# jyfang6/kirag

Measured on NVIDIA B200. Metric: QPS, exact IP top-100 over 21000000x1024, higher is better.
Workload: dtype bf16 filter + f32 rescoring

## Files before the change

### include/kirag_b200.h

```cpp
#ifndef KIRAG_B200_H
#define KIRAG_B200_H

#include <stdint.h>

#ifdef __cplusplus
extern "C" {
#endif

#define KIRAG_ABI_VERSION 7

#define KIRAG_METRIC_INNER_PRODUCT 0
#define KIRAG_METRIC_L2 1

#define KIRAG_PATH_AUTO 0
#define KIRAG_PATH_EXACT 1
#define KIRAG_PATH_FAST 2

#define KIRAG_DTYPE_F32 0
#define KIRAG_DTYPE_BF16 1
#define KIRAG_DTYPE_F16 2

#define KIRAG_MASK_I64 0
#define KIRAG_MASK_I32 1
#define KIRAG_MASK_U8 2

#define KIRAG_POOL_MEAN 0
#define KIRAG_POOL_CLS 1

typedef struct kirag_index kirag_index_t;

typedef struct kirag_search_stats {
    int64_t nq;
    int64_t n_fast;
    int64_t n_exact;
    int64_t n_cert_fail;
    int64_t n_overflow;
    int32_t levels;
    int32_t path;
    int64_t kernel_launches;
    int64_t n_rescan;
    int64_t n_retry;
} kirag_search_stats_t;


int kirag_abi_version(void);

const char* kirag_last_error(void);

int kirag_device_count(void);

int kirag_profile_enable(int on);
int kirag_profile_read(double* scan_ms, int64_t* scan_launches, double* scan_rows);
int kirag_profile_read_launches(double* ms_out, double* rows_out, int64_t max_n);
int kirag_profile_read_timeline(int* tags_out, double* ms_since_first, int64_t max_n);


int kirag_index_create(int d, int metric, int device, kirag_index_t** out);

int kirag_index_destroy(kirag_index_t* h);

int kirag_index_reserve(kirag_index_t* h, int64_t n_total);

int kirag_index_add(kirag_index_t* h, const float* x, int64_t n, int x_is_device, void* stream);

int64_t kirag_index_ntotal(const kirag_index_t* h);

int kirag_index_dim(const kirag_index_t* h);

int kirag_index_search(kirag_index_t* h, const float* q, int64_t nq, int k,
                       float* D, int64_t* I, int ptrs_are_device, int64_t id_offset, void* stream);

int kirag_index_search_ex(kirag_index_t* h, const float* q, int64_t nq, int k,
                          float* D, int64_t* I, int ptrs_are_device, int64_t id_offset,
                          int path, kirag_search_stats_t* stats, void* stream);

int kirag_index_range_search(kirag_index_t* h, const float* q, int64_t nq, float radius, int q_is_device,
                             int64_t id_offset, int path, int64_t* lims_out, kirag_search_stats_t* stats,
                             void* stream);
int kirag_index_range_fetch(kirag_index_t* h, float* D, int64_t* I, int ptrs_are_device, void* stream);

int kirag_index_search_async(kirag_index_t* h, const float* q, int64_t nq, int k,
                             float* D, int64_t* I, int64_t id_offset, void* stream);

int kirag_index_search_finish(kirag_index_t* h, kirag_search_stats_t* stats, int64_t* n_changed);

int kirag_index_search_flags(const kirag_index_t* h, const int** flags_dev);

int kirag_index_search_rearm(kirag_index_t* h, void* stream);

int kirag_index_state_token(const kirag_index_t* h, uint64_t* token);

int kirag_index_reconstruct(const kirag_index_t* h, int64_t i0, int64_t n, float* out,
                            int out_is_device, void* stream);

int kirag_index_save(const kirag_index_t* h, const char* path);

int kirag_index_load(const char* path, int device, kirag_index_t** out);

int kirag_index_device_ptrs(const kirag_index_t* h, const float** master_f32, const void** shadow_bf16);

int kirag_debug_level_schedule(int64_t n_rows, int64_t nq, int k, int d, int64_t* rows_hi_out, int max_levels,
                               int* cap_out, int* kprime_out);

int kirag_index_debug_scores(kirag_index_t* h, const float* q_host, int64_t nq, float* out_host);

int kirag_merge_topk(const float* D_all, const int64_t* I_all, int G, int64_t nq, int k,
                     float* D_out, int64_t* I_out, int ptrs_are_device, int device, void* stream);

typedef struct kirag_exchange kirag_exchange_t;

int kirag_exchange_create(int device, int rank, int world, int64_t max_nq, int max_k, kirag_exchange_t** out);
int kirag_exchange_destroy(kirag_exchange_t* x);
int kirag_exchange_handle_bytes(void);
int kirag_exchange_export(kirag_exchange_t* x, void* handle_out);
int kirag_exchange_connect(kirag_exchange_t* x, const void* handles_all);
int kirag_exchange_connect_ptrs(kirag_exchange_t* x, void* const* peer_buffers);
void* kirag_exchange_buffer(kirag_exchange_t* x);
int kirag_exchange_merge_topk(kirag_exchange_t* x, const float* D_loc, const int64_t* I_loc, int64_t nq, int k,
                              float* D_out, int64_t* I_out, void* stream);

int kirag_exchange_merge_topk_flags(kirag_exchange_t* x, const float* D_loc, const int64_t* I_loc, const int* flags_loc,
                                    int64_t nq, int k, float* D_out, int64_t* I_out, void* stream);
int kirag_exchange_last_any_flag(kirag_exchange_t* x);

// ... 31 lines not shown
```

### kirag_b200/_lib.py

```python
from __future__ import annotations

import ctypes
import os
from ctypes import POINTER, c_char_p, c_float, c_int, c_int32, c_int64, c_void_p

HERE = os.path.dirname(os.path.abspath(__file__))
LIB_PATH = os.environ.get("KIRAG_B200_LIB") or os.path.join(HERE, "libkirag_b200.so")

ABI_VERSION = 7
METRIC_INNER_PRODUCT = 0
METRIC_L2 = 1
PATH_AUTO, PATH_EXACT, PATH_FAST = 0, 1, 2
DTYPE_F32, DTYPE_BF16, DTYPE_F16 = 0, 1, 2
MASK_I64, MASK_I32, MASK_U8 = 0, 1, 2
POOL_MEAN, POOL_CLS = 0, 1


class SearchStats(ctypes.Structure):
    _fields_ = [
        ("nq", c_int64),
        ("n_fast", c_int64),
        ("n_exact", c_int64),
        ("n_cert_fail", c_int64),
        ("n_overflow", c_int64),
        ("levels", c_int32),
        ("path", c_int32),
        ("kernel_launches", c_int64),
        ("n_rescan", c_int64),
        ("n_retry", c_int64),
    ]

    def as_dict(self):
        return {name: int(getattr(self, name)) for name, _ in self._fields_}


class KiragError(RuntimeError):
    """A C-ABI call returned a non-zero status (CUDA failure, bad handle...)."""


SIGNATURES = {
    "kirag_abi_version": (c_int, []),
    "kirag_last_error": (c_char_p, []),
    "kirag_device_count": (c_int, []),
    "kirag_profile_enable": (c_int, [c_int]),
    "kirag_profile_read": (c_int, [POINTER(ctypes.c_double), POINTER(c_int64), POINTER(ctypes.c_double)]),
    "kirag_profile_read_launches": (c_int, [POINTER(ctypes.c_double), POINTER(ctypes.c_double), c_int64]),
    "kirag_profile_read_timeline": (c_int, [POINTER(c_int), POINTER(ctypes.c_double), c_int64]),
    "kirag_index_create": (c_int, [c_int, c_int, c_int, POINTER(c_void_p)]),
    "kirag_index_destroy": (c_int, [c_void_p]),
    "kirag_index_reserve": (c_int, [c_void_p, c_int64]),
    "kirag_index_add": (c_int, [c_void_p, c_void_p, c_int64, c_int, c_void_p]),
    "kirag_index_ntotal": (c_int64, [c_void_p]),
    "kirag_index_dim": (c_int, [c_void_p]),
    "kirag_index_search": (c_int, [c_void_p, c_void_p, c_int64, c_int, c_void_p, c_void_p, c_int, c_int64, c_void_p]),
    "kirag_index_search_ex": (c_int, [c_void_p, c_void_p, c_int64, c_int, c_void_p, c_void_p, c_int, c_int64, c_int,
                                      POINTER(SearchStats), c_void_p]),
    "kirag_index_range_search": (c_int, [c_void_p, c_void_p, c_int64, c_float, c_int, c_int64, c_int, c_void_p,
                                         POINTER(SearchStats), c_void_p]),
    "kirag_index_range_fetch": (c_int, [c_void_p, c_void_p, c_void_p, c_int, c_void_p]),
    "kirag_index_search_async": (c_int, [c_void_p, c_void_p, c_int64, c_int, c_void_p, c_void_p, c_int64, c_void_p]),
    "kirag_index_search_finish": (c_int, [c_void_p, POINTER(SearchStats), POINTER(c_int64)]),
    "kirag_index_search_flags": (c_int, [c_void_p, POINTER(c_void_p)]),
    "kirag_index_search_rearm": (c_int, [c_void_p, c_void_p]),
    "kirag_index_state_token": (c_int, [c_void_p, POINTER(ctypes.c_uint64)]),
    "kirag_index_reconstruct": (c_int, [c_void_p, c_int64, c_int64, c_void_p, c_int, c_void_p]),
    "kirag_index_save": (c_int, [c_void_p, c_char_p]),
    "kirag_index_load": (c_int, [c_char_p, c_int, POINTER(c_void_p)]),
    "kirag_index_device_ptrs": (c_int, [c_void_p, POINTER(c_void_p), POINTER(c_void_p)]),
    "kirag_debug_level_schedule": (c_int, [c_int64, c_int64, c_int, c_int, POINTER(c_int64), c_int, POINTER(c_int),
                                           POINTER(c_int)]),
    "kirag_index_debug_scores": (c_int, [c_void_p, c_void_p, c_int64, c_void_p]),
    "kirag_merge_topk": (c_int, [c_void_p, c_void_p, c_int, c_int64, c_int, c_void_p, c_void_p, c_int, c_int, c_void_p]),
    "kirag_exchange_create": (c_int, [c_int, c_int, c_int, c_int64, c_int, POINTER(c_void_p)]),
    "kirag_exchange_destroy": (c_int, [c_void_p]),
    "kirag_exchange_handle_bytes": (c_int, []),
    "kirag_exchange_export": (c_int, [c_void_p, c_void_p]),
    "kirag_exchange_connect": (c_int, [c_void_p, c_void_p]),
    "kirag_exchange_connect_ptrs": (c_int, [c_void_p, POINTER(c_void_p)]),
    "kirag_exchange_buffer": (c_void_p, [c_void_p]),
    "kirag_exchange_merge_topk": (c_int, [c_void_p, c_void_p, c_void_p, c_int64, c_int, c_void_p, c_void_p, c_void_p]),
    "kirag_exchange_merge_topk_flags": (c_int, [c_void_p, c_void_p, c_void_p, c_void_p, c_int64, c_int, c_void_p, c_void_p,
                                                c_void_p]),
    "kirag_exchange_last_any_flag": (c_int, [c_void_p]),
    "kirag_topk_ip": (c_int, [c_void_p, c_int64, c_void_p, c_int64, c_int, c_int, c_void_p, c_void_p, c_int, c_int,
                              c_void_p]),
    "kirag_topk_ip_release": (c_int, []),
    "kirag_pool_normalize": (c_int, [c_void_p, c_void_p, c_void_p, c_int64, c_int64, c_int64, c_int64, c_int64, c_int64,
                                     c_int, c_int, c_int, c_int, c_int, c_void_p]),
    "kirag_pool_normalize_fwd_saved": (c_int, [c_void_p, c_void_p, c_void_p, c_void_p, c_int64, c_int64, c_int64,
                                               c_int64, c_int64, c_int64, c_int, c_int, c_int, c_int, c_int, c_void_p]),
    "kirag_pool_normalize_typed": (c_int, [c_void_p, c_void_p, c_void_p, c_void_p, c_void_p, c_int64, c_int64, c_int64,
                                           c_int64, c_int64, c_int64, c_int, c_int, c_int, c_int, c_int, c_void_p]),
    "kirag_pool_normalize_backward": (c_int, [c_void_p, c_void_p, c_void_p, c_void_p, c_void_p, c_int64, c_int64,
                                              c_int64, c_int64, c_int, c_int, c_int, c_int, c_int, c_void_p]),
}

_lib = None


def load() -> ctypes.CDLL:
    global _lib
    if _lib is not None:
        return _lib
    if not os.path.exists(LIB_PATH):
        raise ImportError(
            f"{LIB_PATH} is missing: build it with `python -m kirag_b200._build` "
            "(or `python -c 'import __graft_entry__ as g; g.build()'`). "
            "kirag_b200 has no CPU or pure-Python fallback."
        )
    lib = ctypes.CDLL(LIB_PATH)
    for name, (restype, argtypes) in SIGNATURES.items():
        fn = getattr(lib, name)
# ... 34 lines not shown
```

### kirag_b200/csrc/api.cu

```cuda
#include "common.cuh"
#include "../../include/kirag_b200.h"

#include <cuda.h>

#include <algorithm>
#include <atomic>
#include <cstdarg>
#include <cstdio>
#include <cstdlib>
#include <cstring>
#include <cmath>
#include <mutex>
#include <new>
#include <vector>

namespace kirag {

static thread_local char g_err[768] = "";
static std::atomic<long long> g_launches{0};

void set_error(const char* fmt, ...) {
    va_list ap;
    va_start(ap, fmt);
    vsnprintf(g_err, sizeof(g_err), fmt, ap);
// ... 140 lines not shown
            return cudaGetDriverEntryPoint(name, fn, cudaEnableDefault, &qr) == cudaSuccess &&
                   qr == cudaDriverEntryPointSuccess && *fn != nullptr;
        };
        a.ok = get("cuMemAddressReserve", (void**)&a.AddressReserve) && get("cuMemAddressFree", (void**)&a.AddressFree) &&
               get("cuMemCreate", (void**)&a.Create) && get("cuMemRelease", (void**)&a.Release) &&
               get("cuMemMap", (void**)&a.Map) && get("cuMemUnmap", (void**)&a.Unmap) &&
               get("cuMemSetAccess", (void**)&a.SetAccess) &&
               get("cuMemGetAllocationGranularity", (void**)&a.GetGranularity);
        cudaGetLastError();
        return a;
    }();
    return api;
}

struct VmBuffer {
    CUdeviceptr base = 0;
    size_t reserved = 0, mapped = 0, gran = 0;
    int device = 0;
    struct Chunk { CUmemGenericAllocationHandle h; size_t off, size; };
    std::vector<Chunk> chunks;

    bool active() const { return base != 0; }
    void* ptr() const { return reinterpret_cast<void*>(base); }

    CUmemAllocationProp prop() const {
        CUmemAllocationProp p = {};
        p.type = CU_MEM_ALLOCATION_TYPE_PINNED;
        p.location.type = CU_MEM_LOCATION_TYPE_DEVICE;
        p.location.id = device;
        return p;
    }
    int reserve(int dev, size_t bytes) {
        const VmmApi& a = vmm_api();
        if (!a.ok) return 1;
        device = dev;
        const CUmemAllocationProp p = prop();
        if (a.GetGranularity(&gran, &p, CU_MEM_ALLOC_GRANULARITY_RECOMMENDED) != CUDA_SUCCESS || gran == 0) return 1;
        reserved = (bytes + gran - 1) / gran * gran;
        if (a.AddressReserve(&base, reserved, 0, 0, 0) != CUDA_SUCCESS) { base = 0; reserved = 0; return 1; }
        return 0;
    }
    int ensure(size_t bytes) {
        if (bytes <= mapped) return 0;
        const VmmApi& a = vmm_api();
        const size_t want = (bytes + gran - 1) / gran * gran;
        if (want > reserved) return 1;
        Chunk c;
        c.off = mapped;
        c.size = want - mapped;
        const CUmemAllocationProp p = prop();
        if (a.Create(&c.h, c.size, &p, 0) != CUDA_SUCCESS) return 1;
        if (a.Map(base + c.off, c.size, 0, c.h, 0) != CUDA_SUCCESS) { a.Release(c.h); return 1; }
        CUmemAccessDesc acc = {};
        acc.location = p.location;
        acc.flags = CU_MEM_ACCESS_FLAGS_PROT_READWRITE;
        if (a.SetAccess(base + c.off, c.size, &acc, 1) != CUDA_SUCCESS) {
            a.Unmap(base + c.off, c.size);
            a.Release(c.h);
            return 1;
        }
        chunks.push_back(c);
        mapped = want;
        return 0;
    }
    void release() {
        const VmmApi& a = vmm_api();
        for (auto& c : chunks) { a.Unmap(base + c.off, c.size); a.Release(c.h); }
        chunks.clear();
        if (base) a.AddressFree(base, reserved);
        base = 0;
        reserved = mapped = 0;
    }
};

struct FastParams {
    int kprime;
    int growth_override;
    int cap_override;
    int first_growth_override;
    int few_queries;
};

struct SearchCounters {
    int64_t n_fast = 0, n_exact = 0, n_cert_fail = 0, n_overflow = 0, n_rescan = 0, n_retry = 0, n_changed = 0;
    int levels = 0;
};

struct PendingSearch {
    bool active = false;
    bool ev_recorded = false;
    bool fast_ok = false;
    int mode = 0, path = 0, k = 0;
    int64_t nq = 0, id_offset = 0;
    const float* qd = nullptr;
    float* Dd = nullptr;
    int64_t* Id = nullptr;
    cudaStream_t st = nullptr;
    long long launches0 = 0;
    SearchCounters counters;
    FastParams fp{};
};

struct kirag_index {
    int d = 0;
    int metric = 0;
    int device = 0;
    int num_sms = 148;
    int64_t ntotal = 0;
    int64_t capacity = 0;
    float* master = nullptr;
    uint8_t* shadow = nullptr;
    VmBuffer vm_master, vm_shadow;
    bool use_vmm = false;
    unsigned* maxnorm2_bits = nullptr;
    float maxnorm = 0.f;
    float maxerr = 0.f;
    float maxnorm_x = 0.f;
    float* center = nullptr;
    float center_norm = 0.f;
    bool center_decided = false;
    DevBuf q_dev, D_dev, I_dev, qshadow, qnorm, cand, cnt, tau, tauk, overflow, flags, rescored;
    DevBuf dense, stage_a, stage_b, qmap, qsel, qnorm2, D_tmp, I_tmp, t_dev, center_sums;
    int* host_flags = nullptr;
    size_t host_flags_n = 0;
    PendingSearch pending;
    PendingSearch captured;
    bool has_captured = false;
    cudaEvent_t pending_ev = nullptr;
    DevBuf ritems, ritems2, rcount, rcursor, roff, rtab, rD, rI;
    int64_t range_n = 0;
    bool range_valid = false;
};

static int64_t round_up(int64_t v, int64_t m) { return (v + m - 1) / m * m; }

static int env_int(const char* name, int dflt) {
    const char* v = getenv(name);
    if (!v || !*v) return dflt;
    return atoi(v);
}

constexpr int64_t kCenterMinRows = 4096;
constexpr int64_t kCenterSampleRows = 8192;
static int decide_center(kirag_index* h, int64_t rows_available, cudaStream_t st) {
    if (env_int("KIRAG_NO_CENTER", 0)) return 0;
    const int d = h->d;
    const int64_t rows = rows_available < kCenterSampleRows ? rows_available : kCenterSampleRows;
    DevBuf& sums = h->center_sums;
    if (sums.ensure((size_t)(d + 1) * 4)) return 1;
    std::vector<float> host((size_t)d + 1);
    int rc = 1;
    do {
        if (cudaMemsetAsync(sums.p, 0, (size_t)(d + 1) * 4, st) != cudaSuccess) break;
        if (launch_column_sums(h->master, rows, d, sums.as<float>(), st)) break;
        if (cudaMemcpyAsync(host.data(), sums.p, (size_t)(d + 1) * 4, cudaMemcpyDeviceToHost, st) != cudaSuccess ||
            cudaStreamSynchronize(st) != cudaSuccess) {
            set_error("decide_center: reading the column sums failed: %s", cudaGetErrorString(cudaGetLastError()));
            break;
        }
        double c2 = 0.0;
        for (int c = 0; c < d; ++c) {
            host[(size_t)c] = (float)((double)host[(size_t)c] / (double)rows);
            c2 += (double)host[(size_t)c] * (double)host[(size_t)c];
        }
        const double mean_sq = (double)host[(size_t)d] / (double)rows;
        rc = 0;
        if (!(c2 >= mean_sq / 16.0) || !(mean_sq > 0.0) || !(c2 == c2)) break;
        rc = 1;
        if (cudaMalloc((void**)&h->center, (size_t)d * 4) != cudaSuccess) {
            h->center = nullptr;
            set_error("decide_center: cudaMalloc failed: %s", cudaGetErrorString(cudaGetLastError()));
            break;
        }
        if (cudaMemcpyAsync(h->center, host.data(), (size_t)d * 4, cudaMemcpyHostToDevice, st) != cudaSuccess ||
            cudaStreamSynchronize(st) != cudaSuccess) {
            set_error("decide_center: uploading the centre failed");
            break;
        }
        h->center_norm = (float)sqrt(c2);
        rc = 0;
    } while (0);
    return rc;
}

static int index_grow(kirag_index* h, int64_t need_rows, cudaStream_t st) {
    if (need_rows <= h->capacity) return 0;
    const bool want_shadow = scan_tc_supported(h->d) != 0;
    const size_t row_m = (size_t)h->d * sizeof(float), row_s = (size_t)h->d * 2;
    if (h->capacity == 0 && !h->master && vmm_api().ok) {
        size_t free_b = 0, total_b = 0;
        if (cudaMemGetInfo(&free_b, &total_b) == cudaSuccess && total_b > 0) {
            const size_t max_rows = (size_t)round_up((int64_t)(total_b / row_m) + kTileRows, kTileRows);
            if (h->vm_master.reserve(h->device, max_rows * row_m) == 0 &&
                (!want_shadow || h->vm_shadow.reserve(h->device, max_rows * row_s) == 0)) {
                h->use_vmm = true;
                h->master = static_cast<float*>(h->vm_master.ptr());
                h->shadow = want_shadow ? static_cast<uint8_t*>(h->vm_shadow.ptr()) : nullptr;
            } else {
                h->vm_master.release();
                h->vm_shadow.release();
            }
        }
        cudaGetLastError();
    }
    int64_t cap = round_up(need_rows > h->capacity + h->capacity / 4 ? need_rows : h->capacity + h->capacity / 4, kTileRows);
    const int64_t exact = round_up(need_rows, kTileRows);
    if (h->use_vmm) {
        for (int attempt = 0; attempt < 2; ++attempt) {
            const int64_t c = attempt == 0 ? cap : exact;
            if (h->vm_master.ensure((size_t)c * row_m) == 0 && (!want_shadow || h->vm_shadow.ensure((size_t)c * row_s) == 0)) {
                h->capacity = c;
                return 0;
            }
            if (cap == exact) break;
        }
        size_t free_b = 0, total_b = 0;
        cudaMemGetInfo(&free_b, &total_b);
        set_error("index storage for %lld rows x %d (fp32 master%s) does not fit: %zu MiB free of %zu MiB",
                  (long long)exact, h->d, want_shadow ? " + bf16 shadow" : "", free_b >> 20, total_b >> 20);
        cudaGetLastError();
        return 1;
    }
    auto regrow = [&](void** buf, size_t row_bytes, size_t live_rows, const char* what) -> int {
        void* nb = nullptr;
        int64_t c = cap;
        cudaError_t e = cudaMalloc(&nb, (size_t)c * row_bytes);
        if (e != cudaSuccess && cap != exact) { cudaGetLastError(); c = exact; e = cudaMalloc(&nb, (size_t)c * row_bytes); }
        if (e != cudaSuccess) {
            set_error("cudaMalloc of the %s (%zu bytes for %lld rows) failed: %s", what, (size_t)c * row_bytes, (long long)c,
                      cudaGetErrorString(e));
            cudaGetLastError();
            return 1;
        }
        if (*buf && live_rows > 0) {
            if (cudaMemcpyAsync(nb, *buf, live_rows * row_bytes, cudaMemcpyDeviceToDevice, st) != cudaSuccess ||
                cudaStreamSynchronize(st) != cudaSuccess) {
                cudaFree(nb);
                set_error("device copy while growing the %s failed: %s", what, cudaGetErrorString(cudaGetLastError()));
                return 1;
            }
        }
        if (*buf) cudaFree(*buf);
        *buf = nb;
        cap = c;
        return 0;
    };
    if (regrow((void**)&h->master, row_m, (size_t)h->ntotal, "fp32 master")) return 1;
    if (want_shadow && regrow((void**)&h->shadow, row_s, (size_t)round_up(h->ntotal, kTileRows), "bf16 shadow")) return 1;
    h->capacity = cap;
    return 0;
}

static int exact_search(kirag_index* h, const float* qsub, int64_t nsub, int k, float* D, int64_t* I,
                        int64_t out_row0, const int* qmap_dev, int64_t id_offset, cudaStream_t st) {
    const int64_t n = h->ntotal;
    const int d = h->d;
    const int m = (int)((k < n) ? k : n);
    const int64_t ld = round_up(n, 32);
    if (h->dense.ensure((size_t)kExactNQ * ld * sizeof(float))) return 1;
    const int64_t n_seg = (n + kSelectSeg - 1) / kSelectSeg;
    if (h->stage_a.ensure((size_t)kExactNQ * n_seg * m * sizeof(Cand))) return 1;
    for (int64_t g0 = 0; g0 < nsub; g0 += kExactNQ) {
        const int gq = (int)((nsub - g0 < kExactNQ) ? (nsub - g0) : kExactNQ);
        if (launch_scan_exact(h->master, n, d, qsub + g0 * d, gq, h->dense.as<float>(), ld, h->num_sms, st)) return 1;
        int nseg_i = 0;
        if (launch_select_dense(h->dense.as<float>(), ld, n, gq, m, h->stage_a.as<Cand>(), &nseg_i, st)) return 1;
        Cand* cur = h->stage_a.as<Cand>();
        int64_t cur_stride = (int64_t)nseg_i * m;
        int cur_count = (int)cur_stride;
        bool use_b = true;
        while (cur_count > kSelectSeg) {
            const int ns2 = (cur_count + kSelectSeg - 1) / kSelectSeg;
            DevBuf& dstb = use_b ? h->stage_b : h->stage_a;
            if (dstb.ensure((size_t)kExactNQ * ns2 * m * sizeof(Cand))) return 1;
            Cand* dst = dstb.as<Cand>();
            if (launch_select_pairs(cur, cur_stride, nullptr, cur_count, 0x7fffffff, gq, m, dst,
                                    (int64_t)ns2 * m, ns2, nullptr, nullptr, nullptr, st)) return 1;
            cur = dst;
            cur_stride = (int64_t)ns2 * m;
            cur_count = (int)cur_stride;
// ... 7 lines not shown
    return 0;
}

constexpr int64_t kWideCapMaxQueries = 128;
constexpr int64_t kQChunk = 16384;
constexpr int64_t kFewQueries = 8;
constexpr int kMaxGrowth = 32;


static bool fast_eligible(const kirag_index* h, int k, FastParams* fp) {
    if (!h->shadow || !scan_tc_supported(h->d)) return false;
    if (h->ntotal > 0x7fffff00LL) return false;
    int64_t kp = (int64_t)4 * k;
    if (kp < 32) kp = 32;
    if (kp > 2048) kp = 2048;
    if (kp < k) return false;
    fp->kprime = (int)kp;
    fp->growth_override = env_int("KIRAG_LEVEL_GROWTH", 0);
    fp->cap_override = env_int("KIRAG_CAND_CAP", 0);
    fp->first_growth_override = env_int("KIRAG_LEVEL1_GROWTH", 0);
    if (fp->cap_override > 0 && fp->cap_override < 4 * kp) return false;
    return true;
}

static int pick_cap(const FastParams& fp, int64_t nq) {
    int cap = (nq <= kWideCapMaxQueries) ? kWideCap : kSelectSeg;
    if (fp.cap_override > 0) cap = fp.cap_override;
    if (cap > kWideCap) cap = kWideCap;
    return cap;
}

static std::vector<int64_t> level_bounds(int64_t n_tiles, int cap, const FastParams& fp) {
    std::vector<int64_t> hi;
    int64_t t = (cap / 2) / kTileRows;
    if (t < 1) t = 1;
    if (t > n_tiles) t = n_tiles;
    hi.push_back(t);
    if (t >= n_tiles) return hi;
    int gmax = cap / (4 * fp.kprime);
    if (gmax > kMaxGrowth) gmax = kMaxGrowth;
    if (fp.growth_override > 0) gmax = fp.growth_override;
    if (gmax < 2) gmax = 2;
    int g1 = (cap >= kWideCap && fp.few_queries) ? 16 : 4;
    if (fp.first_growth_override > 0) g1 = fp.first_growth_override;
    if (g1 > gmax) g1 = gmax;
    t = t * g1;
    if (t > n_tiles) t = n_tiles;
    hi.push_back(t);
    if (t >= n_tiles) return hi;
    const double ratio = (double)n_tiles / (double)t;
    int L = (int)ceil(log(ratio) / log((double)gmax) - 1e-9);
    if (L < 1) L = 1;
    const double g = pow(ratio, 1.0 / L);
    const int64_t base = t;
    for (int i = 1; i <= L; ++i) {
        int64_t b = (i == L) ? n_tiles : (int64_t)ceil((double)base * pow(g, (double)i));
        if (b <= hi.back()) b = hi.back() + 1;
        if (b > n_tiles) b = n_tiles;
        hi.push_back(b);
        if (b >= n_tiles) break;
    }
    return hi;
}

static int64_t pick_tile_mult(int64_t n_tiles) {
    if (n_tiles <= 2) return 1;
    int64_t m = (int64_t)(0.6180339887498949 * (double)n_tiles);
    if (m < 1) m = 1;
    auto gcd = [](int64_t a, int64_t b) { while (b) { int64_t t = a % b; a = b; b = t; } return a; };
    while (gcd(m, n_tiles) != 1) ++m;
    return m % n_tiles;
}

struct CertEps { float a, b; };
static CertEps cert_eps(const kirag_index* h) {
    const double yn = (double)h->maxnorm, ey = (double)h->maxerr, xn = (double)h->maxnorm_x, cn = (double)h->center_norm;
    const double acc = (double)h->d * ldexp(1.0, -22);
    CertEps e;
    e.a = (float)((ey + acc * (yn + xn) + ldexp(1.0, -24) * yn + 64.0 * ldexp(1.0, -24) * cn) * 1.002);
    e.b = (float)((yn + 2.0 * ey) * 1.002);
    return e;
}

static int fast_search(kirag_index* h, const float* qd, int64_t nq, int k, float* D, int64_t* I,
                       int64_t id_offset, const FastParams& fp, int check_cert, int* levels_out,
                       cudaStream_t st) {
    const int d = h->d;
    const int64_t n = h->ntotal;
    struct PdlScope {
        explicit PdlScope(bool on) { g_pdl_this_call = on; }
        ~PdlScope() { g_pdl_this_call = true; }
    } pdl_scope(nq <= kPdlMaxQueries);
    ScanTcPlan plan;
    if (scan_tc_pick(nq, d, &plan)) return 1;
    const size_t qs_bytes = scan_tc_qshadow_bytes(nq, d, plan);
    if (h->qshadow.ensure(qs_bytes)) return 1;
    if (h->qnorm.ensure((size_t)nq * 12)) return 1;
    const int cap = pick_cap(fp, nq);
    if (h->cand.ensure((size_t)nq * cap * sizeof(Cand))) return 1;
    if (h->cnt.ensure((size_t)nq * 4)) return 1;
    const int64_t nq_pad = round_up(nq, 256);
    if (h->tau.ensure((size_t)nq_pad * 4)) return 1;
    if (h->overflow.ensure((size_t)nq * 4)) return 1;
    if (h->flags.ensure((size_t)nq * 4)) return 1;
    if (h->rescored.ensure((size_t)nq * fp.kprime * 4)) return 1;
    if (h->tauk.ensure((size_t)nq * 4)) return 1;
    const bool fuse_tail = cap == kWideCap && fp.kprime <= 2048;
    if ((nq % plan.bq) != 0)
        KIRAG_CUDA_OK(cudaMemsetAsync(h->qshadow.p, 0, qs_bytes, st));
    KIRAG_CUDA_OK(launch_chained(init_search_state_kernel, dim3((unsigned)((nq_pad + 255) / 256)), dim3(256), 0, st,
                                 h->tau.as<float>(), h->cnt.as<int>(), h->overflow.as<int>(), nq, nq_pad));
    KIRAG_LAUNCH_OK("init_search_state_kernel");
    prof_mark(0, st);
    float* const qcdot = h->qnorm.as<float>() + 2 * nq;
    if (launch_convert_rows(qd, nq, d, 0, h->qshadow.p, plan.bq / 2, nullptr, h->qnorm.as<float>(),
                            h->qnorm.as<float>() + nq, h->center, qcdot, st)) return 1;
    prof_mark(1, st);

    const int64_t n_tiles = (n + kTileRows - 1) / kTileRows;
    const int64_t mult = pick_tile_mult(n_tiles);
    FastParams fpl = fp;
    fpl.few_queries = nq <= kFewQueries ? 1 : 0;
    const std::vector<int64_t> bounds = level_bounds(n_tiles, cap, fpl);
    int64_t lo = 0;
    int levels = 0;
    for (const int64_t hi : bounds) {
        cudaEvent_t e0 = nullptr, e1 = nullptr;
        if (g_prof.on) {
            KIRAG_CUDA_OK(cudaEventCreate(&e0));
            KIRAG_CUDA_OK(cudaEventCreate(&e1));
            KIRAG_CUDA_OK(cudaEventRecord(e0, st));
        }
        if (launch_scan_tc(h->shadow, n, d, h->qshadow.p, nq, plan, lo, hi, n_tiles, mult,
                           h->tau.as<float>(), h->cand.as<Cand>(), h->cnt.as<int>(), cap, h->num_sms,
                           levels == 0 ? 1 : 0, st)) return 1;
        if (g_prof.on) {
            KIRAG_CUDA_OK(cudaEventRecord(e1, st));
            g_prof.ev.emplace_back(e0, e1);
            int64_t r1 = hi * kTileRows; if (r1 > n) r1 = n;
            g_prof.rows += (double)(r1 - lo * kTileRows);
            g_prof.launch_rows.push_back((double)(r1 - lo * kTileRows));
            g_prof.queries = (double)nq;
        }
        prof_mark(10 + levels, st);
        const bool last = (hi == bounds.back());
        if (last && fuse_tail) break;
        if (launch_compact_topm(h->cand.as<Cand>(), cap, h->cnt.as<int>(), cap, (int)nq, fp.kprime,
                                h->tau.as<float>(), h->overflow.as<int>(), last ? h->tauk.as<float>() : nullptr,
                                k, st)) return 1;
        prof_mark(30 + levels, st);
        ++levels;
        lo = hi;
    }
    const CertEps ce = cert_eps(h);
    if (fuse_tail) {
        ++levels;
        if (launch_tail_fused(h->cand.as<Cand>(), cap, h->cnt.as<int>(), cap, (int)nq, fp.kprime, h->tau.as<float>(),
                              h->overflow.as<int>(), h->master, d, qd, h->rescored.as<float>(), k, D, I, id_offset,
                              h->qnorm.as<float>(), h->qnorm.as<float>() + nq, qcdot, ce.a, ce.b, h->flags.as<int>(),
                              h->num_sms, st)) return 1;
        prof_mark(51, st);
        if (levels_out) *levels_out = levels;
        return 0;
    }
    if (launch_rescore(h->master, d, qd, h->cand.as<Cand>(), h->cnt.as<int>(), cap, fp.kprime,
                       h->rescored.as<float>(), nq, h->tauk.as<float>(), h->qnorm.as<float>(),
                       h->qnorm.as<float>() + nq, ce.a, ce.b, st)) return 1;
    prof_mark(50, st);
    if (launch_final(h->cand.as<Cand>(), cap, h->rescored.as<float>(), h->cnt.as<int>(), 0, fp.kprime,
                     (int)nq, k, D, I, id_offset, h->tau.as<float>(), h->qnorm.as<float>(), h->qnorm.as<float>() + nq,
                     qcdot, ce.a, ce.b, check_cert, h->overflow.as<int>(), h->flags.as<int>(), nullptr, st)) return 1;
    prof_mark(51, st);
    if (levels_out) *levels_out = levels;
    return 0;
}

__global__ void rescan_threshold_kernel(const float* __restrict__ D, const int* __restrict__ qmap,
                                        const float* __restrict__ qnorm, const float* __restrict__ qerr,
                                        const float* __restrict__ qcdot, int k,
                                        float eps_a, float eps_b, int64_t nb,
                                        int64_t nb_pad, float* __restrict__ tau2, int* __restrict__ cnt,
                                        int* __restrict__ overflow) {
    const int64_t i = (int64_t)blockIdx.x * blockDim.x + threadIdx.x;
    if (i >= nb_pad) return;
    if (i >= nb) { tau2[i] = INFINITY; return; }
    const int q = qmap[i];
    const float kth = D[(int64_t)q * k + (k - 1)];
    tau2[i] = (kth > -FLT_MAX) ? kth - (eps_a * qnorm[q] + eps_b * qerr[q]) - qcdot[q] : -INFINITY;
    cnt[i] = 0;
    overflow[i] = 0;
}

static int rescan_search(kirag_index* h, const float* qsel, const float* qnorm_all, const float* qerr_all,
                         const float* qcdot_all, int64_t nb,
                         int k, float* D,
                         int64_t* I, const int* qmap_dev, int64_t id_offset, int cap, std::vector<int>* still_bad,
                         cudaStream_t st) {
    const int d = h->d;
    const int64_t n = h->ntotal;
    ScanTcPlan plan;
    if (scan_tc_pick(nb, d, &plan)) return 1;
    const size_t qs_bytes = scan_tc_qshadow_bytes(nb, d, plan);
    const int64_t nb_pad = round_up(nb, 256);
    if (h->qshadow.ensure(qs_bytes)) return 1;
    if (h->cand.ensure((size_t)nb * cap * sizeof(Cand))) return 1;
    if (h->cnt.ensure((size_t)nb_pad * 4) || h->tau.ensure((size_t)nb_pad * 4) || h->overflow.ensure((size_t)nb_pad * 4)) return 1;
    if (h->flags.ensure((size_t)nb_pad * 4)) return 1;
    if (h->rescored.ensure((size_t)nb * cap * 4)) return 1;
    const CertEps ce = cert_eps(h);
    rescan_threshold_kernel<<<(unsigned)((nb_pad + 255) / 256), 256, 0, st>>>(
        D, qmap_dev, qnorm_all, qerr_all, qcdot_all, k, ce.a, ce.b, nb, nb_pad, h->tau.as<float>(), h->cnt.as<int>(),
        h->overflow.as<int>());
    KIRAG_LAUNCH_OK("rescan_threshold_kernel");
    if ((nb % plan.bq) != 0) KIRAG_CUDA_OK(cudaMemsetAsync(h->qshadow.p, 0, qs_bytes, st));
    if (launch_convert_rows(qsel, nb, d, 0, h->qshadow.p, plan.bq / 2, nullptr, nullptr, nullptr, nullptr, nullptr,
                            st)) return 1;
    const int64_t n_tiles = (n + kTileRows - 1) / kTileRows;
    if (launch_scan_tc(h->shadow, n, d, h->qshadow.p, nb, plan, 0, n_tiles, n_tiles, 1, h->tau.as<float>(),
                       h->cand.as<Cand>(), h->cnt.as<int>(), cap, h->num_sms, 1, st)) return 1;
    if (launch_rescore(h->master, d, qsel, h->cand.as<Cand>(), h->cnt.as<int>(), cap, cap, h->rescored.as<float>(), nb,
                       nullptr, nullptr, nullptr, 0.f, 0.f, st)) return 1;
    std::vector<int> counts((size_t)nb);
    KIRAG_CUDA_OK(cudaMemcpyAsync(counts.data(), h->cnt.p, (size_t)nb * 4, cudaMemcpyDeviceToHost, st));
    if (launch_final(h->cand.as<Cand>(), cap, h->rescored.as<float>(), h->cnt.as<int>(), 0, cap, (int)nb, k, D, I,
                     id_offset, nullptr, nullptr, nullptr, nullptr, 0.f, 0.f, 0, nullptr, nullptr, qmap_dev, st)) return 1;
    KIRAG_CUDA_OK(cudaStreamSynchronize(st));
    for (int64_t i = 0; i < nb; ++i)
        if (counts[(size_t)i] > cap) still_bad->push_back((int)i);
    return 0;
}


static int ensure_host_flags(kirag_index* h, int64_t cq) {
    if (h->host_flags_n >= (size_t)cq) return 0;
    if (h->host_flags) cudaFreeHost(h->host_flags);
    h->host_flags = nullptr;
    h->host_flags_n = 0;
    const size_t want = (size_t)round_up(cq, 4096);
    KIRAG_CUDA_OK(cudaHostAlloc((void**)&h->host_flags, want * sizeof(int), cudaHostAllocDefault));
    h->host_flags_n = want;
    return 0;
}

static int enqueue_chunk(kirag_index* h, const float* qd, int64_t cq, int k, float* Dd, int64_t* Id, int64_t id_offset,
                         bool fast_ok, const FastParams& fp, SearchCounters* c, int* mode, cudaStream_t st) {
    *mode = 0;
    if (h->ntotal == 0) return launch_fill_pad(Dd, Id, cq * k, st);
    if (!fast_ok) {
        if (exact_search(h, qd, cq, k, Dd, Id, 0, nullptr, id_offset, st)) return 1;
        c->n_exact += cq;
        return 0;
    }
    if (ensure_host_flags(h, cq)) return 1;
    if (fast_search(h, qd, cq, k, Dd, Id, id_offset, fp, 1, &c->levels, st)) return 1;
    KIRAG_CUDA_OK(cudaMemcpyAsync(h->host_flags, h->flags.p, (size_t)cq * 4, cudaMemcpyDeviceToHost, st));
    *mode = 1;
    return 0;
}

__global__ void scatter_rows_kernel(const float* __restrict__ Ds, const int64_t* __restrict__ Is, const int* __restrict__ qmap,
                                    int k, float* __restrict__ D, int64_t* __restrict__ I) {
    const int64_t src = blockIdx.x, dst = qmap[src];
    for (int j = threadIdx.x; j < k; j += blockDim.x) {
        D[dst * k + j] = Ds[src * k + j];
        I[dst * k + j] = Is[src * k + j];
    }
}

static int resolve_chunk(kirag_index* h, const float* qd, int64_t cq, int k, float* Dd, int64_t* Id, int64_t id_offset,
                         int path, const FastParams& fp, SearchCounters* c, cudaStream_t st) {
    const int d = h->d;
    const int* flags = h->host_flags;
    std::vector<int> cert, ovf;
    for (int64_t i = 0; i < cq; ++i) {
        if (flags[(size_t)i] == 2) { ovf.push_back((int)i); ++c->n_overflow; }
        else if (flags[(size_t)i]) { cert.push_back((int)i); ++c->n_cert_fail; }
    }
    const int64_t n_bad = (int64_t)(cert.size() + ovf.size());
    if (n_bad == 0 || path != KIRAG_PATH_AUTO) {
        c->n_fast += cq;
        return 0;
    }
    if (h->qnorm2.ensure((size_t)cq * 12)) return 1;
    KIRAG_CUDA_OK(cudaMemcpyAsync(h->qnorm2.p, h->qnorm.p, (size_t)cq * 12, cudaMemcpyDeviceToDevice, st));
    std::vector<int> exact;
    const bool no_rescan = env_int("KIRAG_NO_RESCAN", 0) != 0;
    const bool gentle_already = fp.growth_override > 0 && fp.growth_override <= 4 && fp.first_growth_override > 0;
    if (!ovf.empty() && !gentle_already) {
        const int64_t nb = (int64_t)ovf.size();
        if (h->qmap.ensure((size_t)nb * 4) || h->qsel.ensure((size_t)nb * d * 4)) return 1;
        if (h->D_tmp.ensure((size_t)nb * k * 4) || h->I_tmp.ensure((size_t)nb * k * 8)) return 1;
        KIRAG_CUDA_OK(cudaMemcpyAsync(h->qmap.p, ovf.data(), (size_t)nb * 4, cudaMemcpyHostToDevice, st));
        gather_rows_kernel<<<(unsigned)nb, 256, 0, st>>>(qd, h->qmap.as<int>(), d, h->qsel.as<float>());
        KIRAG_LAUNCH_OK("gather_rows_kernel");
        FastParams gentle = fp;
        gentle.growth_override = 4;
        gentle.first_growth_override = 2;
        if (fast_search(h, h->qsel.as<float>(), nb, k, h->D_tmp.as<float>(), h->I_tmp.as<int64_t>(), id_offset, gentle, 1,
                        nullptr, st)) return 1;
        std::vector<int> f2((size_t)nb);
        KIRAG_CUDA_OK(cudaMemcpyAsync(f2.data(), h->flags.p, (size_t)nb * 4, cudaMemcpyDeviceToHost, st));
        scatter_rows_kernel<<<(unsigned)nb, 128, 0, st>>>(h->D_tmp.as<float>(), h->I_tmp.as<int64_t>(), h->qmap.as<int>(), k,
                                                          Dd, Id);
        KIRAG_LAUNCH_OK("scatter_rows_kernel");
        KIRAG_CUDA_OK(cudaStreamSynchronize(st));
        for (int64_t i = 0; i < nb; ++i) {
            if (f2[(size_t)i] == 0) ++c->n_retry;
            else if (f2[(size_t)i] == 2) exact.push_back(ovf[(size_t)i]);
            else cert.push_back(ovf[(size_t)i]);
        }
    } else {
        exact = ovf;
    }
    if (!cert.empty() && no_rescan) {
        exact.insert(exact.end(), cert.begin(), cert.end());
        cert.clear();
    }
    if (!cert.empty()) {
        const int64_t nb = (int64_t)cert.size();
        if (h->qmap.ensure((size_t)nb * 4)) return 1;
        if (h->qsel.ensure((size_t)nb * d * 4)) return 1;
        KIRAG_CUDA_OK(cudaMemcpyAsync(h->qmap.p, cert.data(), (size_t)nb * 4, cudaMemcpyHostToDevice, st));
        gather_rows_kernel<<<(unsigned)nb, 256, 0, st>>>(qd, h->qmap.as<int>(), d, h->qsel.as<float>());
        KIRAG_LAUNCH_OK("gather_rows_kernel");
        std::vector<int> still_bad;
        if (rescan_search(h, h->qsel.as<float>(), h->qnorm2.as<float>(), h->qnorm2.as<float>() + cq,
                          h->qnorm2.as<float>() + 2 * cq, nb, k, Dd, Id, h->qmap.as<int>(), id_offset, kSelectSeg, &still_bad,
                          st)) return 1;
        for (int i : still_bad) exact.push_back(cert[(size_t)i]);
        c->n_rescan += nb - (int64_t)still_bad.size();
    }
    if (!exact.empty()) {
        const int64_t nb = (int64_t)exact.size();
        if (h->qmap.ensure((size_t)nb * 4)) return 1;
        if (h->qsel.ensure((size_t)nb * d * 4)) return 1;
        KIRAG_CUDA_OK(cudaMemcpyAsync(h->qmap.p, exact.data(), (size_t)nb * 4, cudaMemcpyHostToDevice, st));
        gather_rows_kernel<<<(unsigned)nb, 256, 0, st>>>(qd, h->qmap.as<int>(), d, h->qsel.as<float>());
        KIRAG_LAUNCH_OK("gather_rows_kernel");
        if (exact_search(h, h->qsel.as<float>(), nb, k, Dd, Id, 0, h->qmap.as<int>(), id_offset, st)) return 1;
        c->n_exact += nb;
    }
    KIRAG_CUDA_OK(cudaStreamSynchronize(st));
    c->n_fast += cq - n_bad;
    c->n_changed += n_bad;
    return 0;
}

static void fill_stats(kirag_search_stats_t* stats, int64_t nq, const SearchCounters& c, bool fast_ok, int path,
                       long long launches0) {
    if (!stats) return;
    stats->nq = nq;
    stats->n_fast = c.n_fast;
    stats->n_exact = c.n_exact;
    stats->n_cert_fail = c.n_cert_fail;
    stats->n_overflow = c.n_overflow;
    stats->n_rescan = c.n_rescan;
    stats->n_retry = c.n_retry;
    stats->levels = c.levels;
    stats->path = fast_ok ? path : KIRAG_PATH_EXACT;
    stats->kernel_launches = g_launches.load() - launches0;
}

static void drop_range_result(kirag_index* h) {
    h->range_n = 0;
    h->range_valid = false;
}

static int finish_pending(kirag_index* h, kirag_search_stats_t* stats, int64_t* n_changed) {
    drop_range_result(h);
    if (n_changed) *n_changed = 0;
    PendingSearch& p = h->pending;
    if (!p.active) {
        if (stats) memset(stats, 0, sizeof(*stats));
        return 0;
    }
    p.active = false;
    DeviceGuard guard(h->device);
    if (!guard.ok) return 1;
    if (p.ev_recorded) KIRAG_CUDA_OK(cudaEventSynchronize(h->pending_ev));
    else KIRAG_CUDA_OK(cudaStreamSynchronize(p.st));
    SearchCounters c = p.counters;
    if (p.mode == 1 && resolve_chunk(h, p.qd, p.nq, p.k, p.Dd, p.Id, p.id_offset, p.path, p.fp, &c, p.st)) return 1;
    fill_stats(stats, p.nq, c, p.fast_ok, p.path, p.launches0);
    if (n_changed) *n_changed = c.n_changed;
    return 0;
}

static int search_impl(kirag_index* h, const float* q, int64_t nq, int k, float* D, int64_t* I,
                       int ptrs_are_device, int64_t id_offset, int path, kirag_search_stats_t* stats,
                       cudaStream_t st) {
    KIRAG_CHECK(h != nullptr, "search: null index");
    KIRAG_CHECK(k > 0, "search: k must be positive (got %d)", k);
    KIRAG_CHECK(k <= 2048, "search: k=%d exceeds the supported maximum of 2048", k);
    KIRAG_CHECK(nq >= 0, "search: negative nq");
    KIRAG_CHECK(path >= 0 && path <= 2, "search: unknown path %d", path);
    if (finish_pending(h, nullptr, nullptr)) return 1;
    if (stats) memset(stats, 0, sizeof(*stats));
    if (nq == 0) return 0;
    KIRAG_CHECK(q && D && I, "search: null buffer");
    DeviceGuard guard(h->device);
    if (!guard.ok) return 1;
    const long long launches0 = g_launches.load();
    const int d = h->d;
    SearchCounters c;
    FastParams fp{};
    const bool fast_ok = (path != KIRAG_PATH_EXACT) && h->ntotal > 0 && fast_eligible(h, k, &fp);

    for (int64_t q0 = 0; q0 < nq; q0 += kQChunk) {
        const int64_t cq = (nq - q0 < kQChunk) ? (nq - q0) : kQChunk;
        const float* qd;
        float* Dd;
        int64_t* Id;
        if (ptrs_are_device) {
            qd = q + q0 * d; Dd = D + q0 * k; Id = I + q0 * k;
        } else {
            if (h->q_dev.ensure((size_t)cq * d * 4)) return 1;
            if (h->D_dev.ensure((size_t)cq * k * 4)) return 1;
            if (h->I_dev.ensure((size_t)cq * k * 8)) return 1;
            KIRAG_CUDA_OK(cudaMemcpyAsync(h->q_dev.p, q + q0 * d, (size_t)cq * d * 4, cudaMemcpyHostToDevice, st));
            qd = h->q_dev.as<float>(); Dd = h->D_dev.as<float>(); Id = h->I_dev.as<int64_t>();
        }
        int mode = 0;
        if (enqueue_chunk(h, qd, cq, k, Dd, Id, id_offset, fast_ok, fp, &c, &mode, st)) return 1;
        if (!ptrs_are_device) {
            KIRAG_CUDA_OK(cudaMemcpyAsync(D + q0 * k, Dd, (size_t)cq * k * 4, cudaMemcpyDeviceToHost, st));
            KIRAG_CUDA_OK(cudaMemcpyAsync(I + q0 * k, Id, (size_t)cq * k * 8, cudaMemcpyDeviceToHost, st));
        }
        if (mode == 1 || !ptrs_are_device) KIRAG_CUDA_OK(cudaStreamSynchronize(st));
        if (mode == 1) {
            const int64_t changed0 = c.n_changed;
            if (resolve_chunk(h, qd, cq, k, Dd, Id, id_offset, path, fp, &c, st)) return 1;
            if (!ptrs_are_device && c.n_changed != changed0) {
                KIRAG_CUDA_OK(cudaMemcpyAsync(D + q0 * k, Dd, (size_t)cq * k * 4, cudaMemcpyDeviceToHost, st));
                KIRAG_CUDA_OK(cudaMemcpyAsync(I + q0 * k, Id, (size_t)cq * k * 8, cudaMemcpyDeviceToHost, st));
                KIRAG_CUDA_OK(cudaStreamSynchronize(st));
            }
        }
    }
    fill_stats(stats, nq, c, fast_ok, path, launches0);
    return 0;
}

constexpr size_t kRangeGroupBytes = (size_t)1 << 30;

struct RangeChunk {
    std::vector<int64_t> src_off, count;
    int64_t used = 0;
};

static int grow_keep(DevBuf& b, size_t used, size_t need, cudaStream_t st) {
    if (need <= b.bytes) return 0;
    size_t want = b.bytes + b.bytes / 2;
    if (want < need) want = need;
    want = (want + ((size_t)1 << 20) - 1) & ~(((size_t)1 << 20) - 1);
    void* p = nullptr;
    cudaError_t e = cudaMalloc(&p, want);
    if (e != cudaSuccess) {
        cudaGetLastError();
        set_error("range_search: cudaMalloc(%zu) for the collected entries failed: %s", want, cudaGetErrorString(e));
        return 1;
    }
    if (used) KIRAG_CUDA_OK(cudaMemcpyAsync(p, b.p, used, cudaMemcpyDeviceToDevice, st));
    KIRAG_CUDA_OK(cudaStreamSynchronize(st));
    b.release();
    b.p = p;
    b.bytes = want;
    return 0;
}

static int range_reserve(kirag_index* h, RangeChunk& rc, const std::vector<int>& counts, const std::vector<int>& chunk_q,
                         cudaStream_t st) {
    const size_t nsrc = counts.size();
    std::vector<int64_t> cursor(nsrc, 0);
    int64_t add = 0;
    for (size_t i = 0; i < nsrc; ++i) {
        if (chunk_q[i] < 0) continue;
        cursor[i] = rc.used + add;
        rc.src_off[(size_t)chunk_q[i]] = cursor[i];
        rc.count[(size_t)chunk_q[i]] = counts[i];
        add += counts[i];
    }
    if (grow_keep(h->ritems, (size_t)rc.used * 8, (size_t)(rc.used + add) * 8, st)) return 1;
    rc.used += add;
    if (h->rcursor.ensure(nsrc * 8)) return 1;
    KIRAG_CUDA_OK(cudaMemcpyAsync(h->rcursor.p, cursor.data(), nsrc * 8, cudaMemcpyHostToDevice, st));
    KIRAG_CUDA_OK(cudaStreamSynchronize(st));
    return 0;
}

static int range_scan(kirag_index* h, const ScanTcPlan& plan, int64_t nq, int cap, cudaStream_t st) {
    const int64_t n = h->ntotal;
    const int64_t n_tiles = (n + kTileRows - 1) / kTileRows;
    cudaEvent_t e0 = nullptr, e1 = nullptr;
    if (g_prof.on) {
        KIRAG_CUDA_OK(cudaEventCreate(&e0));
        KIRAG_CUDA_OK(cudaEventCreate(&e1));
        KIRAG_CUDA_OK(cudaEventRecord(e0, st));
    }
    if (launch_scan_tc(h->shadow, n, h->d, h->qshadow.p, nq, plan, 0, n_tiles, n_tiles, 1, h->tau.as<float>(),
                       h->cand.as<Cand>(), h->cnt.as<int>(), cap, h->num_sms, 1, st)) return 1;
    if (g_prof.on) {
        KIRAG_CUDA_OK(cudaEventRecord(e1, st));
        g_prof.ev.emplace_back(e0, e1);
        g_prof.rows += (double)n;
        g_prof.launch_rows.push_back((double)n);
        g_prof.queries = (double)nq;
    }
    return 0;
}

static int range_filter_pass(kirag_index* h, const float* qs, int64_t nb, const int* qmap_dev,
                             const std::vector<int>& chunk_q_of_row, int64_t cq, float radius, int cap, bool first,
                             RangeChunk& rc, std::vector<int>* cnt_out, cudaStream_t st) {
    const int d = h->d;
// ... 133 lines not shown
    }
    if (n_seg) {
        tab[(size_t)4 * n_seg] = total_long;
        if (h->ritems2.ensure((size_t)rc.used * 8) || h->rtab.ensure(tab.size() * 8)) return 1;
        KIRAG_CUDA_OK(cudaMemcpyAsync(h->rtab.p, tab.data(), tab.size() * 8, cudaMemcpyHostToDevice, st));
    }
    if (h->roff.ensure(((size_t)cq * 2 + 1) * 8)) return 1;
    KIRAG_CUDA_OK(cudaMemcpyAsync(h->roff.p, rc.src_off.data(), (size_t)cq * 8, cudaMemcpyHostToDevice, st));
    KIRAG_CUDA_OK(cudaMemcpyAsync(h->roff.as<int64_t>() + cq, lims.data(), ((size_t)cq + 1) * 8, cudaMemcpyHostToDevice, st));
    if (launch_range_emit(h->ritems.as<uint64_t>(), h->ritems2.as<uint64_t>(), cq, h->roff.as<int64_t>(),
                          h->roff.as<int64_t>() + cq, n_seg, longest, total_long, h->rtab.as<int64_t>(), id_offset,
                          h->rD.as<float>() + base, h->rI.as<int64_t>() + base, st)) return 1;
    KIRAG_CUDA_OK(cudaStreamSynchronize(st));
    return 0;
}

static int range_search_impl(kirag_index* h, const float* q, int64_t nq, float radius, int q_is_device,
                             int64_t id_offset, int path, int64_t* lims_out, kirag_search_stats_t* stats,
                             cudaStream_t st) {
    KIRAG_CHECK(nq >= 0, "range_search: negative nq");
    KIRAG_CHECK(h != nullptr, "range_search: null index");
    KIRAG_CHECK(lims_out != nullptr, "range_search: null lims");
    KIRAG_CHECK(path >= 0 && path <= 2, "range_search: unknown path %d", path);
    if (finish_pending(h, nullptr, nullptr)) return 1;
    if (stats) memset(stats, 0, sizeof(*stats));
    for (int64_t i = 0; i <= nq; ++i) lims_out[i] = 0;
    const bool fast_ok = path != KIRAG_PATH_EXACT && h->shadow && scan_tc_supported(h->d) && h->ntotal <= 0x7fffff00LL;
    if (nq == 0 || h->ntotal == 0 || !(radius < INFINITY)) {
        h->range_valid = true;
        if (stats) { stats->nq = nq; stats->path = fast_ok ? path : KIRAG_PATH_EXACT; }
        return 0;
    }
    KIRAG_CHECK(q != nullptr, "range_search: null queries");
    DeviceGuard guard(h->device);
    if (!guard.ok) return 1;
    const long long launches0 = g_launches.load();
    const int d = h->d;
    FastParams fp{};
    fp.cap_override = env_int("KIRAG_CAND_CAP", 0);
    SearchCounters c;
    int64_t base = 0;
    for (int64_t q0 = 0; q0 < nq; q0 += kQChunk) {
        const int64_t cq = (nq - q0 < kQChunk) ? (nq - q0) : kQChunk;
        const float* qd = q + q0 * d;
        if (!q_is_device) {
            if (h->q_dev.ensure((size_t)cq * d * 4)) return 1;
            KIRAG_CUDA_OK(cudaMemcpyAsync(h->q_dev.p, qd, (size_t)cq * d * 4, cudaMemcpyHostToDevice, st));
            qd = h->q_dev.as<float>();
        }
        RangeChunk rc;
        rc.src_off.assign((size_t)cq, 0);
        rc.count.assign((size_t)cq, 0);
        if (fast_ok ? range_filter_chunk(h, qd, cq, radius, pick_cap(fp, cq), rc, &c, st)
                    : range_exact_chunk(h, qd, cq, radius, rc, &c, st)) return 1;
        int64_t chunk_total = 0;
        if (range_emit_chunk(h, rc, cq, id_offset, base, lims_out + q0, &chunk_total, st)) return 1;
        base += chunk_total;
    }
    lims_out[nq] = base;
    h->range_n = base;
    h->range_valid = true;
    fill_stats(stats, nq, c, fast_ok, path, launches0);
    return 0;
}

static int range_fetch_impl(kirag_index* h, float* D, int64_t* I, int ptrs_are_device, cudaStream_t st) {
    KIRAG_CHECK(h != nullptr, "range_fetch: null index");
    KIRAG_CHECK(h->range_valid, "range_fetch: no range-search result is held (the last call on this index was not "
                                "kirag_index_range_search, or its result was fetched already)");
    const int64_t total = h->range_n;
    if (total > 0) {
        KIRAG_CHECK(D && I, "range_fetch: null buffer");
        DeviceGuard guard(h->device);
        if (!guard.ok) return 1;
        const cudaMemcpyKind kind = ptrs_are_device ? cudaMemcpyDeviceToDevice : cudaMemcpyDeviceToHost;
        KIRAG_CUDA_OK(cudaMemcpyAsync(D, h->rD.p, (size_t)total * 4, kind, st));
        KIRAG_CUDA_OK(cudaMemcpyAsync(I, h->rI.p, (size_t)total * 8, kind, st));
        KIRAG_CUDA_OK(cudaStreamSynchronize(st));
    }
    drop_range_result(h);
    return 0;
}

static int finalize_rows(kirag_index* h, int64_t r0, int64_t n, cudaStream_t st) {
    if (h->shadow && !h->center_decided && r0 + n >= kCenterMinRows) {
        if (decide_center(h, r0 + n, st)) return 1;
        h->center_decided = true;
        if (h->center && r0 > 0) {
            KIRAG_CUDA_OK(cudaMemsetAsync(h->maxnorm2_bits, 0, 8, st));
            if (launch_convert_rows(h->master, r0, h->d, 0, h->shadow, kTileRows, h->maxnorm2_bits, nullptr, nullptr, h->center,
                                    nullptr, st)) return 1;
        }
    }
    if (launch_convert_rows(h->master + r0 * (int64_t)h->d, n, h->d, r0, h->shadow, kTileRows, h->maxnorm2_bits, nullptr,
                            nullptr, h->center, nullptr, st)) return 1;
    if (h->shadow && ((r0 + n) % kTileRows) != 0) {
        const int64_t end = r0 + n;
        const int64_t tile = end / kTileRows;
        const int rr = (int)(end - tile * kTileRows);
        uint8_t* tile_base = h->shadow + (size_t)tile * ((size_t)h->d * kTileRows * 2);
        KIRAG_CUDA_OK(cudaMemset2DAsync(tile_base + (size_t)rr * 128, (size_t)kTileRows * 128, 0, (size_t)(kTileRows - rr) * 128,
                                        (size_t)(h->d / kKChunk), st));
    }
    unsigned bits[3] = {0, 0, 0};
    KIRAG_CUDA_OK(cudaMemcpyAsync(bits, h->maxnorm2_bits, 12, cudaMemcpyDeviceToHost, st));
    KIRAG_CUDA_OK(cudaStreamSynchronize(st));
    float m2[3];
    memcpy(m2, bits, 12);
    h->maxnorm = sqrtf(m2[0]);
    h->maxerr = h->shadow ? sqrtf(m2[1]) : 0.f;
    h->maxnorm_x = h->shadow ? sqrtf(m2[2]) : h->maxnorm;
    h->ntotal = r0 + n;
    return 0;
}

extern "C" {

int kirag_abi_version(void) { return KIRAG_ABI_VERSION; }

const char* kirag_last_error(void) { return g_err; }

int kirag_device_count(void) {
    int n = 0;
    if (cudaGetDeviceCount(&n) != cudaSuccess) { cudaGetLastError(); return 0; }
    return n;
}

int kirag_profile_enable(int on) {
    for (auto& pr : g_prof.ev) { cudaEventDestroy(pr.first); cudaEventDestroy(pr.second); }
    g_prof.ev.clear();
    g_prof.launch_rows.clear();
    for (auto& mk : g_prof.marks) cudaEventDestroy(mk.second);
    g_prof.marks.clear();
    g_prof.rows = 0.0;
    g_prof.on = on != 0;
    return 0;
}

int kirag_profile_read_timeline(int* tags_out, double* ms_since_first, int64_t max_n) {
    int64_t i = 0;
    for (auto& mk : g_prof.marks) {
        if (i >= max_n) break;
        KIRAG_CUDA_OK(cudaEventSynchronize(mk.second));
        float t = 0.f;
        KIRAG_CUDA_OK(cudaEventElapsedTime(&t, g_prof.marks[0].second, mk.second));
        if (tags_out) tags_out[i] = mk.first;
        if (ms_since_first) ms_since_first[i] = t;
        ++i;
    }
    return (int)i;
}

int kirag_profile_read_launches(double* ms_out, double* rows_out, int64_t max_n) {
    int64_t i = 0;
    for (auto& pr : g_prof.ev) {
        if (i >= max_n) break;
        KIRAG_CUDA_OK(cudaEventSynchronize(pr.second));
        float t = 0.f;
        KIRAG_CUDA_OK(cudaEventElapsedTime(&t, pr.first, pr.second));
        if (ms_out) ms_out[i] = t;
        if (rows_out) rows_out[i] = g_prof.launch_rows[(size_t)i];
        ++i;
    }
    return 0;
}

int kirag_profile_read(double* scan_ms, int64_t* scan_launches, double* scan_rows) {
    double ms = 0.0;
    for (auto& pr : g_prof.ev) {
        KIRAG_CUDA_OK(cudaEventSynchronize(pr.second));
        float t = 0.f;
        KIRAG_CUDA_OK(cudaEventElapsedTime(&t, pr.first, pr.second));
        ms += t;
    }
    if (scan_ms) *scan_ms = ms;
    if (scan_launches) *scan_launches = (int64_t)g_prof.ev.size();
    if (scan_rows) *scan_rows = g_prof.rows;
    for (auto& pr : g_prof.ev) { cudaEventDestroy(pr.first); cudaEventDestroy(pr.second); }
    g_prof.ev.clear();
    g_prof.launch_rows.clear();
    for (auto& mk : g_prof.marks) cudaEventDestroy(mk.second);
    g_prof.marks.clear();
    g_prof.rows = 0.0;
    return 0;
}

int kirag_index_create(int d, int metric, int device, kirag_index_t** out) {
    KIRAG_CHECK(out != nullptr, "index_create: null out pointer");
    *out = nullptr;
    KIRAG_CHECK(d > 0 && d <= 16384, "index_create: unsupported dimension %d", d);
    KIRAG_CHECK(metric == KIRAG_METRIC_INNER_PRODUCT,
                "index_create: only the inner-product metric is implemented (got %d)", metric);
    int ndev = 0;
    cudaError_t e = cudaGetDeviceCount(&ndev);
    if (e != cudaSuccess || ndev == 0) {
        set_error("index_create: no CUDA device available (%s); this library has no CPU path",
                  e == cudaSuccess ? "device count is 0" : cudaGetErrorString(e));
        cudaGetLastError();
        return 1;
    }
    KIRAG_CHECK(device >= 0 && device < ndev, "index_create: device %d out of range [0,%d)", device, ndev);
    cudaDeviceProp prop;
    KIRAG_CUDA_OK(cudaGetDeviceProperties(&prop, device));
    KIRAG_CHECK(prop.major == 10, "index_create: device %d is sm_%d%d; this library is built for sm_100a only",
                device, prop.major, prop.minor);
    DeviceGuard guard(device);
    if (!guard.ok) return 1;
    kirag_index* h = new (std::nothrow) kirag_index();
    KIRAG_CHECK(h != nullptr, "index_create: out of host memory");
    h->d = d;
    h->metric = metric;
    h->device = device;
    h->num_sms = prop.multiProcessorCount;
    if (cudaMalloc((void**)&h->maxnorm2_bits, 12) != cudaSuccess || cudaMemset(h->maxnorm2_bits, 0, 12) != cudaSuccess) {
        set_error("index_create: cudaMalloc failed: %s", cudaGetErrorString(cudaGetLastError()));
        delete h;
        return 1;
    }
    *out = h;
    return 0;
}

int kirag_index_destroy(kirag_index_t* h) {
    if (!h) return 0;
    DeviceGuard guard(h->device);
    cudaDeviceSynchronize();
    if (h->use_vmm) {
        h->vm_master.release();
        h->vm_shadow.release();
    } else {
        if (h->master) cudaFree(h->master);
        if (h->shadow) cudaFree(h->shadow);
    }
    if (h->maxnorm2_bits) cudaFree(h->maxnorm2_bits);
    if (h->center) cudaFree(h->center);
    DevBuf* bufs[] = {&h->q_dev, &h->D_dev, &h->I_dev, &h->qshadow, &h->qnorm, &h->cand, &h->cnt, &h->tau, &h->tauk,
                      &h->overflow, &h->flags, &h->rescored, &h->dense, &h->stage_a, &h->stage_b, &h->qmap, &h->qsel, &h->qnorm2, &h->t_dev, &h->center_sums,
                      &h->D_tmp, &h->I_tmp, &h->ritems, &h->ritems2, &h->rcount, &h->rcursor, &h->roff, &h->rtab,
                      &h->rD, &h->rI};
    for (DevBuf* b : bufs) b->release();
    if (h->host_flags) cudaFreeHost(h->host_flags);
    if (h->pending_ev) cudaEventDestroy(h->pending_ev);
    delete h;
    return 0;
}

int kirag_index_reserve(kirag_index_t* h, int64_t n_total) {
    KIRAG_CHECK(h != nullptr, "index_reserve: null index");
    KIRAG_CHECK(n_total >= 0, "index_reserve: negative size");
    DeviceGuard guard(h->device);
    if (!guard.ok) return 1;
    return index_grow(h, n_total, 0);
}

int kirag_index_add(kirag_index_t* h, const float* x, int64_t n, int x_is_device, void* stream) {
    KIRAG_CHECK(h != nullptr, "index_add: null index");
    KIRAG_CHECK(n >= 0, "index_add: negative n");
    if (n == 0) return 0;
    KIRAG_CHECK(x != nullptr, "index_add: null data");
    DeviceGuard guard(h->device);
    if (!guard.ok) return 1;
    cudaStream_t st = (cudaStream_t)stream;
    if (finish_pending(h, nullptr, nullptr)) return 1;
    KIRAG_CHECK(h->ntotal + n <= 0x7fffff00LL, "index_add: more than 2^31 rows per device are not supported");
    if (index_grow(h, h->ntotal + n, st)) return 1;
    float* dst = h->master + h->ntotal * (int64_t)h->d;
    KIRAG_CUDA_OK(cudaMemcpyAsync(dst, x, (size_t)n * h->d * sizeof(float),
                                  x_is_device ? cudaMemcpyDeviceToDevice : cudaMemcpyHostToDevice, st));
    return finalize_rows(h, h->ntotal, n, st);
}

int64_t kirag_index_ntotal(const kirag_index_t* h) { return h ? h->ntotal : -1; }
int kirag_index_dim(const kirag_index_t* h) { return h ? h->d : -1; }

int kirag_index_search(kirag_index_t* h, const float* q, int64_t nq, int k, float* D, int64_t* I,
                       int ptrs_are_device, int64_t id_offset, void* stream) {
    int path = env_int("KIRAG_PATH", KIRAG_PATH_AUTO);
    return search_impl(h, q, nq, k, D, I, ptrs_are_device, id_offset, path, nullptr, (cudaStream_t)stream);
}

int kirag_index_search_ex(kirag_index_t* h, const float* q, int64_t nq, int k, float* D, int64_t* I,
                          int ptrs_are_device, int64_t id_offset, int path, kirag_search_stats_t* stats,
                          void* stream) {
    return search_impl(h, q, nq, k, D, I, ptrs_are_device, id_offset, path, stats, (cudaStream_t)stream);
}

int kirag_index_range_search(kirag_index_t* h, const float* q, int64_t nq, float radius, int q_is_device,
                             int64_t id_offset, int path, int64_t* lims_out, kirag_search_stats_t* stats,
                             void* stream) {
    const int rc = range_search_impl(h, q, nq, radius, q_is_device, id_offset, path, lims_out, stats,
                                     (cudaStream_t)stream);
    if (rc && h) drop_range_result(h);
    return rc;
}

int kirag_index_range_fetch(kirag_index_t* h, float* D, int64_t* I, int ptrs_are_device, void* stream) {
    return range_fetch_impl(h, D, I, ptrs_are_device, (cudaStream_t)stream);
}

int kirag_index_search_async(kirag_index_t* h, const float* q, int64_t nq, int k, float* D, int64_t* I,
                             int64_t id_offset, void* stream) {
    KIRAG_CHECK(h != nullptr, "search_async: null index");
    KIRAG_CHECK(k > 0 && k <= 2048, "search_async: k=%d not in [1, 2048]", k);
    KIRAG_CHECK(nq >= 0 && nq <= kQChunk, "search_async: nq=%lld not in [0, %lld] (split larger batches)", (long long)nq,
                (long long)kQChunk);
    if (finish_pending(h, nullptr, nullptr)) return 1;
    if (nq == 0) return 0;
    KIRAG_CHECK(q && D && I, "search_async: null buffer");
    DeviceGuard guard(h->device);
    if (!guard.ok) return 1;
    cudaStream_t st = (cudaStream_t)stream;
    PendingSearch& p = h->pending;
    p = PendingSearch();
    p.launches0 = g_launches.load();
    p.fast_ok = h->ntotal > 0 && fast_eligible(h, k, &p.fp);
    p.path = KIRAG_PATH_AUTO;
    if (enqueue_chunk(h, q, nq, k, D, I, id_offset, p.fast_ok, p.fp, &p.counters, &p.mode, st)) return 1;
    cudaStreamCaptureStatus cap = cudaStreamCaptureStatusNone;
    cudaStreamIsCapturing(st, &cap);
    if (cap == cudaStreamCaptureStatusNone) {
        if (!h->pending_ev) KIRAG_CUDA_OK(cudaEventCreateWithFlags(&h->pending_ev, cudaEventDisableTiming));
        KIRAG_CUDA_OK(cudaEventRecord(h->pending_ev, st));
        p.ev_recorded = true;
    }
    p.nq = nq; p.k = k; p.id_offset = id_offset;
    p.qd = q; p.Dd = D; p.Id = I; p.st = st;
    p.active = true;
    if (cap != cudaStreamCaptureStatusNone) {
        h->captured = p;
        h->has_captured = true;
    }
    return 0;
}

int kirag_index_search_rearm(kirag_index_t* h, void* stream) {
    KIRAG_CHECK(h != nullptr, "search_rearm: null index");
    KIRAG_CHECK(h->has_captured, "search_rearm: no asynchronous search has been captured on this index");
    if (finish_pending(h, nullptr, nullptr)) return 1;
    h->pending = h->captured;
    h->pending.st = (cudaStream_t)stream;
    h->pending.ev_recorded = false;
    h->pending.launches0 = g_launches.load();
    h->pending.active = true;
    return 0;
}

int kirag_index_state_token(const kirag_index_t* h, uint64_t* token) {
    KIRAG_CHECK(h != nullptr && token != nullptr, "state_token: null argument");
    uint64_t x = 1469598103934665603ULL;
    auto mix = [&x](uint64_t v) {
        for (int i = 0; i < 8; ++i) { x ^= (v >> (8 * i)) & 0xffu; x *= 1099511628211ULL; }
    };
    mix((uint64_t)h->ntotal);
    mix((uint64_t)(uintptr_t)h->master);
    mix((uint64_t)(uintptr_t)h->shadow);
    mix((uint64_t)(uintptr_t)h->center);
    uint32_t f[4];
    memcpy(&f[0], &h->maxnorm, 4); memcpy(&f[1], &h->maxerr, 4); memcpy(&f[2], &h->maxnorm_x, 4); memcpy(&f[3], &h->center_norm, 4);
    mix(((uint64_t)f[0] << 32) | f[1]);
    mix(((uint64_t)f[2] << 32) | f[3]);
    const DevBuf* bufs[] = {&h->qshadow, &h->qnorm, &h->cand, &h->cnt, &h->tau, &h->tauk, &h->overflow, &h->flags, &h->rescored};
    for (const DevBuf* b : bufs) { mix((uint64_t)(uintptr_t)b->p); mix((uint64_t)b->bytes); }
    mix((uint64_t)(uintptr_t)h->host_flags);
    *token = x;
    return 0;
}

int kirag_index_search_finish(kirag_index_t* h, kirag_search_stats_t* stats, int64_t* n_changed) {
    KIRAG_CHECK(h != nullptr, "search_finish: null index");
    return finish_pending(h, stats, n_changed);
}

int kirag_index_search_flags(const kirag_index_t* h, const int** flags_dev) {
    KIRAG_CHECK(h != nullptr && flags_dev != nullptr, "search_flags: null argument");
    *flags_dev = (h->pending.active && h->pending.mode == 1) ? h->flags.as<int>() : nullptr;
    return 0;
}

int kirag_index_reconstruct(const kirag_index_t* h, int64_t i0, int64_t n, float* out, int out_is_device,
                            void* stream) {
    KIRAG_CHECK(h != nullptr && out != nullptr, "index_reconstruct: null argument");
    KIRAG_CHECK(i0 >= 0 && n >= 0 && i0 + n <= h->ntotal, "index_reconstruct: rows [%lld,%lld) out of range (ntotal=%lld)",
                (long long)i0, (long long)(i0 + n), (long long)h->ntotal);
    if (n == 0) return 0;
    DeviceGuard guard(h->device);
    if (!guard.ok) return 1;
    cudaStream_t st = (cudaStream_t)stream;
    KIRAG_CUDA_OK(cudaMemcpyAsync(out, h->master + i0 * (int64_t)h->d, (size_t)n * h->d * 4,
                                  out_is_device ? cudaMemcpyDeviceToDevice : cudaMemcpyDeviceToHost, st));
    if (!out_is_device) KIRAG_CUDA_OK(cudaStreamSynchronize(st));
    return 0;
}

int kirag_index_debug_scores(kirag_index_t* h, const float* q_host, int64_t nq, float* out_host) {
    KIRAG_CHECK(h && q_host && out_host, "debug_scores: null argument");
    KIRAG_CHECK(h->shadow && scan_tc_supported(h->d), "debug_scores: index has no bf16 shadow (d=%d)", h->d);
    KIRAG_CHECK(nq > 0 && h->ntotal > 0, "debug_scores: empty input");
    DeviceGuard guard(h->device);
    if (!guard.ok) return 1;
    cudaStream_t st = 0;
    const int d = h->d;
    ScanTcPlan plan;
    if (scan_tc_pick(nq, d, &plan)) return 1;
    const char* force = getenv("KIRAG_DEBUG_BQ");
    if (force && *force) {
        static const struct { const char* name; int bq, resident; } kVariants[] = {
            {"64r", 64, 1}, {"64s", 64, 0}, {"128r", 128, 1}, {"128s", 128, 0}, {"256s", 256, 0}};
        bool found = false;
        for (const auto& v : kVariants)
            if (strcmp(force, v.name) == 0) { plan.bq = v.bq; plan.resident = v.resident; found = true; }
        KIRAG_CHECK(found, "debug_scores: KIRAG_DEBUG_BQ=%s is not one of 64r, 64s, 128r, 128s, 256s", force);
    }
    const size_t qs_bytes = scan_tc_qshadow_bytes(nq, d, plan);
    const int64_t nq_pad = round_up(nq, 256);
    DevBuf qd, qs, tau, cnt, dump, cdot;
    std::vector<float> cdot_host;
    int rc = 1;
    do {
        if (cdot.ensure((size_t)nq_pad * 4)) break;
        if (qd.ensure((size_t)nq * d * 4) || qs.ensure(qs_bytes) || tau.ensure((size_t)nq_pad * 4) ||
            cnt.ensure((size_t)nq_pad * 4) || dump.ensure((size_t)h->ntotal * nq * 4)) break;
        if (cudaMemcpyAsync(qd.p, q_host, (size_t)nq * d * 4, cudaMemcpyHostToDevice, st) != cudaSuccess) break;
        if (cudaMemsetAsync(qs.p, 0, qs_bytes, st) != cudaSuccess) break;
        if (cudaMemsetAsync(cnt.p, 0, (size_t)nq_pad * 4, st) != cudaSuccess) break;
        if (cudaMemsetAsync(dump.p, 0, (size_t)h->ntotal * nq * 4, st) != cudaSuccess) break;
        if (fill_f32(tau.as<float>(), INFINITY, nq_pad, st)) break;
        if (launch_convert_rows(qd.as<float>(), nq, d, 0, qs.p, plan.bq / 2, nullptr, nullptr, nullptr, h->center,
                                h->center ? cdot.as<float>() : nullptr, st)) break;
        if (launch_scan_tc_dump(h->shadow, h->ntotal, d, qs.p, nq, plan, tau.as<float>(), cnt.as<int>(),
                                dump.as<float>(), nq, h->num_sms, st)) break;
        if (h->center) {
            cdot_host.resize((size_t)nq);
            if (cudaMemcpyAsync(cdot_host.data(), cdot.p, (size_t)nq * 4, cudaMemcpyDeviceToHost, st) != cudaSuccess) break;
        }
        if (cudaMemcpyAsync(out_host, dump.p, (size_t)h->ntotal * nq * 4, cudaMemcpyDeviceToHost, st) != cudaSuccess ||
            cudaStreamSynchronize(st) != cudaSuccess) {
            set_error("debug_scores: copy/sync failed: %s", cudaGetErrorString(cudaGetLastError()));
            break;
        }
        if (h->center)
            for (int64_t r = 0; r < h->ntotal; ++r)
                for (int64_t qi = 0; qi < nq; ++qi) out_host[r * nq + qi] += cdot_host[(size_t)qi];
        rc = 0;
    } while (0);
    qd.release(); qs.release(); tau.release(); cnt.release(); dump.release(); cdot.release();
    return rc;
}

int kirag_debug_level_schedule(int64_t n_rows, int64_t nq, int k, int d, int64_t* rows_hi_out, int max_levels,
                               int* cap_out, int* kprime_out) {
    if (!(n_rows > 0 && nq > 0 && k > 0 && rows_hi_out && max_levels > 0)) {
        set_error("debug_level_schedule: bad argument");
        return -2;
    }
    int64_t kp = (int64_t)4 * k;
    if (kp < 32) kp = 32;
    if (kp > 2048) kp = 2048;
    if (kp < k || !scan_tc_supported(d) || n_rows > 0x7fffff00LL) return -1;
    FastParams fp{};
    fp.kprime = (int)kp;
    fp.growth_override = env_int("KIRAG_LEVEL_GROWTH", 0);
    fp.cap_override = env_int("KIRAG_CAND_CAP", 0);
    fp.first_growth_override = env_int("KIRAG_LEVEL1_GROWTH", 0);
    if (fp.cap_override > 0 && fp.cap_override < 4 * kp) return -1;
    const int cap = pick_cap(fp, nq);
    fp.few_queries = nq <= kFewQueries ? 1 : 0;
    const int64_t n_tiles = (n_rows + kTileRows - 1) / kTileRows;
    const std::vector<int64_t> b = level_bounds(n_tiles, cap, fp);
    if ((int)b.size() > max_levels) {
        set_error("debug_level_schedule: %zu levels do not fit in %d slots", b.size(), max_levels);
        return -2;
    }
    for (size_t i = 0; i < b.size(); ++i) {
        const int64_t r = b[i] * kTileRows;
        rows_hi_out[i] = r < n_rows ? r : n_rows;
    }
    if (cap_out) *cap_out = cap;
    if (kprime_out) *kprime_out = (int)kp;
    return (int)b.size();
}

int kirag_index_device_ptrs(const kirag_index_t* h, const float** master_f32, const void** shadow_bf16) {
    KIRAG_CHECK(h != nullptr, "index_device_ptrs: null index");
    if (master_f32) *master_f32 = h->master;
    if (shadow_bf16) *shadow_bf16 = h->shadow;
    return 0;
}

static const size_t kIoChunkRows = 65536;

int kirag_index_save(const kirag_index_t* h, const char* path) {
    KIRAG_CHECK(h != nullptr && path != nullptr, "index_save: null argument");
    DeviceGuard guard(h->device);
    if (!guard.ok) return 1;
    FILE* f = fopen(path, "wb");
    KIRAG_CHECK(f != nullptr, "index_save: cannot open %s for writing", path);
    bool ok = true;
    const uint32_t fourcc = (uint32_t)'I' | ((uint32_t)'x' << 8) | ((uint32_t)'F' << 16) | ((uint32_t)'I' << 24);
    const int32_t d = h->d;
    const int64_t ntotal = h->ntotal;
    const int64_t dummy = (int64_t)1 << 20;
    const uint8_t trained = 1;
    const int32_t metric = 0;
    const uint64_t words = (uint64_t)ntotal * (uint64_t)d;
    ok = ok && fwrite(&fourcc, 4, 1, f) == 1 && fwrite(&d, 4, 1, f) == 1 && fwrite(&ntotal, 8, 1, f) == 1 &&
         fwrite(&dummy, 8, 1, f) == 1 && fwrite(&dummy, 8, 1, f) == 1 && fwrite(&trained, 1, 1, f) == 1 &&
         fwrite(&metric, 4, 1, f) == 1 && fwrite(&words, 8, 1, f) == 1;
    float* stage[2] = {nullptr, nullptr};
    cudaEvent_t copied[2] = {nullptr, nullptr};
    cudaStream_t st = nullptr;
    const size_t chunk_bytes = kIoChunkRows * (size_t)d * 4;
    if (ok && ntotal > 0) {
        bool alloc_ok = cudaStreamCreateWithFlags(&st, cudaStreamNonBlocking) == cudaSuccess;
        for (int i = 0; i < 2; ++i)
            alloc_ok = alloc_ok && cudaMallocHost((void**)&stage[i], chunk_bytes) == cudaSuccess &&
                       cudaEventCreateWithFlags(&copied[i], cudaEventDisableTiming) == cudaSuccess;
        if (!alloc_ok) {
            set_error("index_save: pinned staging buffers: %s", cudaGetErrorString(cudaGetLastError()));
            ok = false;
        }
    }
    const int64_t n_pieces = (ntotal + (int64_t)kIoChunkRows - 1) / (int64_t)kIoChunkRows;
    auto piece_rows = [&](int64_t i) {
        const int64_t r = i * (int64_t)kIoChunkRows;
        return (ntotal - r < (int64_t)kIoChunkRows) ? (ntotal - r) : (int64_t)kIoChunkRows;
    };
    auto enqueue = [&](int64_t i) {
        const int b = (int)(i & 1);
// ... 102 lines not shown
    KIRAG_CHECK(G > 0 && k > 0 && nq >= 0, "merge_topk: bad shape G=%d nq=%lld k=%d", G, (long long)nq, k);
    if (nq == 0) return 0;
    KIRAG_CHECK(D_all && I_all && D_out && I_out, "merge_topk: null buffer");
    DeviceGuard guard(device);
    if (!guard.ok) return 1;
    cudaStream_t st = (cudaStream_t)stream;
    if (ptrs_are_device) return launch_merge(D_all, I_all, G, nq, k, D_out, I_out, st);
    const size_t nin = (size_t)G * nq * k, nout = (size_t)nq * k;
    float* dD = nullptr; int64_t* dI = nullptr; float* oD = nullptr; int64_t* oI = nullptr;
    int rc = 1;
    do {
        if (cudaMalloc((void**)&dD, nin * 4) != cudaSuccess || cudaMalloc((void**)&dI, nin * 8) != cudaSuccess ||
            cudaMalloc((void**)&oD, nout * 4) != cudaSuccess || cudaMalloc((void**)&oI, nout * 8) != cudaSuccess) {
            set_error("merge_topk: cudaMalloc failed: %s", cudaGetErrorString(cudaGetLastError()));
            break;
        }
        if (cudaMemcpyAsync(dD, D_all, nin * 4, cudaMemcpyHostToDevice, st) != cudaSuccess ||
            cudaMemcpyAsync(dI, I_all, nin * 8, cudaMemcpyHostToDevice, st) != cudaSuccess) {
            set_error("merge_topk: H2D copy failed");
            break;
        }
        if (launch_merge(dD, dI, G, nq, k, oD, oI, st)) break;
        if (cudaMemcpyAsync(D_out, oD, nout * 4, cudaMemcpyDeviceToHost, st) != cudaSuccess ||
            cudaMemcpyAsync(I_out, oI, nout * 8, cudaMemcpyDeviceToHost, st) != cudaSuccess ||
            cudaStreamSynchronize(st) != cudaSuccess) {
            set_error("merge_topk: D2H copy failed: %s", cudaGetErrorString(cudaGetLastError()));
            break;
        }
        rc = 0;
    } while (0);
    if (dD) cudaFree(dD); if (dI) cudaFree(dI); if (oD) cudaFree(oD); if (oI) cudaFree(oI);
    return rc;
}

struct ScratchIndex { int device; int d; kirag_index_t* h; };
static std::vector<ScratchIndex> g_scratch;
static std::mutex g_scratch_mu;

int kirag_topk_ip(const float* q, int64_t nq, const float* t, int64_t nt, int d, int k, float* D, int64_t* I,
                  int ptrs_are_device, int device, void* stream) {
    KIRAG_CHECK(nt >= 0 && nq >= 0, "topk_ip: negative size");
    std::lock_guard<std::mutex> lock(g_scratch_mu);
    kirag_index_t* h = nullptr;
    for (auto& e : g_scratch)
        if (e.device == device && e.d == d) h = e.h;
    if (!h) {
        if (kirag_index_create(d, KIRAG_METRIC_INNER_PRODUCT, device, &h)) return 1;
        g_scratch.push_back({device, d, h});
    }
    DeviceGuard guard(device);
    if (!guard.ok) return 1;
    cudaStream_t st = (cudaStream_t)stream;
    if (finish_pending(h, nullptr, nullptr)) return 1;
    if (nq > 0 && nq <= 2 * kExactNQ && nt > 0 && nt <= kSelectSeg) {
        KIRAG_CHECK(q && t && D && I, "topk_ip: null buffer");
        KIRAG_CHECK(k > 0 && k <= 2048, "topk_ip: k=%d not in [1, 2048]", k);
        const float* qd = q;
        const float* td = t;
        float* Dd = D;
        int64_t* Id = I;
        if (!ptrs_are_device) {
            if (h->t_dev.ensure((size_t)nt * d * 4) || h->q_dev.ensure((size_t)nq * d * 4) ||
                h->D_dev.ensure((size_t)nq * k * 4) || h->I_dev.ensure((size_t)nq * k * 8)) return 1;
            KIRAG_CUDA_OK(cudaMemcpyAsync(h->t_dev.p, t, (size_t)nt * d * 4, cudaMemcpyHostToDevice, st));
            KIRAG_CUDA_OK(cudaMemcpyAsync(h->q_dev.p, q, (size_t)nq * d * 4, cudaMemcpyHostToDevice, st));
            qd = h->q_dev.as<float>(); td = h->t_dev.as<float>(); Dd = h->D_dev.as<float>(); Id = h->I_dev.as<int64_t>();
        }
        float* const own_master = h->master;
        const int64_t own_n = h->ntotal;
        h->master = const_cast<float*>(td);
        h->ntotal = nt;
        const int rc_small = exact_search(h, qd, nq, k, Dd, Id, 0, nullptr, 0, st);
        h->master = own_master;
        h->ntotal = own_n;
        if (rc_small) return 1;
        if (!ptrs_are_device) {
            KIRAG_CUDA_OK(cudaMemcpyAsync(D, Dd, (size_t)nq * k * 4, cudaMemcpyDeviceToHost, st));
            KIRAG_CUDA_OK(cudaMemcpyAsync(I, Id, (size_t)nq * k * 8, cudaMemcpyDeviceToHost, st));
            KIRAG_CUDA_OK(cudaStreamSynchronize(st));
        }
        return 0;
    }
    h->ntotal = 0;
    h->maxnorm = h->maxerr = h->maxnorm_x = h->center_norm = 0.f;
    h->center_decided = false;
    if (h->center) { cudaFree(h->center); h->center = nullptr; }
    KIRAG_CUDA_OK(cudaMemsetAsync(h->maxnorm2_bits, 0, 12, st));
    int rc = 0;
    if (nt > 0 && ptrs_are_device && (reinterpret_cast<uintptr_t>(t) & 15) == 0) {
        if (index_grow(h, nt, st)) return 1;
        float* const own_master = h->master;
        h->master = const_cast<float*>(t);
        rc = finalize_rows(h, 0, nt, st);
        if (!rc) rc = kirag_index_search(h, q, nq, k, D, I, ptrs_are_device, 0, stream);
        h->master = own_master;
        return rc;
    }
    if (nt > 0) rc = kirag_index_add(h, t, nt, ptrs_are_device, stream);
    if (!rc) rc = kirag_index_search(h, q, nq, k, D, I, ptrs_are_device, 0, stream);
    return rc;
}

int kirag_topk_ip_release(void) {
    std::lock_guard<std::mutex> lock(g_scratch_mu);
    for (auto& e : g_scratch) kirag_index_destroy(e.h);
    g_scratch.clear();
    return 0;
}

int kirag_pool_normalize(const void* hidden, const void* mask, float* out, int64_t B, int64_t S, int64_t H,
                         int64_t sb, int64_t ss, int64_t mb, int hidden_dtype, int mask_dtype, int mode,
                         int normalize, int device, void* stream) {
    KIRAG_CHECK(hidden && out, "pool_normalize: null buffer");
    DeviceGuard guard(device);
    if (!guard.ok) return 1;
    return launch_pool_normalize(hidden, mask, out, nullptr, nullptr, B, S, H, sb, ss, mb, hidden_dtype, mask_dtype, mode,
                                 normalize, (cudaStream_t)stream);
}

int kirag_pool_normalize_fwd_saved(const void* hidden, const void* mask, float* out, float* pooled_norm,
                                   int64_t B, int64_t S, int64_t H, int64_t sb, int64_t ss, int64_t mb,
                                   int hidden_dtype, int mask_dtype, int mode, int normalize, int device,
                                   void* stream) {
    KIRAG_CHECK(hidden && out && pooled_norm, "pool_normalize_fwd_saved: null buffer");
    DeviceGuard guard(device);
    if (!guard.ok) return 1;
    return launch_pool_normalize(hidden, mask, out, nullptr, pooled_norm, B, S, H, sb, ss, mb, hidden_dtype, mask_dtype,
                                 mode, normalize, (cudaStream_t)stream);
}

int kirag_pool_normalize_typed(const void* hidden, const void* mask, float* out, void* out_typed, float* pooled_norm,
                               int64_t B, int64_t S, int64_t H, int64_t sb, int64_t ss, int64_t mb,
                               int hidden_dtype, int mask_dtype, int mode, int normalize, int device,
                               void* stream) {
    KIRAG_CHECK(hidden && out && out_typed, "pool_normalize_typed: null buffer");
    DeviceGuard guard(device);
    if (!guard.ok) return 1;
    return launch_pool_normalize(hidden, mask, out, out_typed, pooled_norm, B, S, H, sb, ss, mb, hidden_dtype, mask_dtype,
                                 mode, normalize, (cudaStream_t)stream);
}

int kirag_pool_normalize_backward(const float* grad_out, const float* out, const float* pooled_norm,
                                  const void* mask, void* grad_hidden, int64_t B, int64_t S, int64_t H,
                                  int64_t mb, int hidden_dtype, int mask_dtype, int mode, int normalize,
                                  int device, void* stream) {
    KIRAG_CHECK(grad_out && out && pooled_norm && grad_hidden, "pool_normalize_backward: null buffer");
    DeviceGuard guard(device);
    if (!guard.ok) return 1;
    return launch_pool_normalize_backward(grad_out, out, pooled_norm, mask, grad_hidden, B, S, H, mb, hidden_dtype,
                                          mask_dtype, mode, normalize, (cudaStream_t)stream);
}

}
```

### kirag_b200/csrc/common.cuh

```cuda
#pragma once

#include <cuda_runtime.h>
#include <cuda_bf16.h>
#include <cuda_fp16.h>
#include <stdint.h>
#include <float.h>

namespace kirag {

void set_error(const char* fmt, ...);
void count_launch(int n = 1);

#define KIRAG_CUDA_OK(expr)                                                              \
    do {                                                                                  \
        cudaError_t _e = (expr);                                                          \
        if (_e != cudaSuccess) {                                                          \
            kirag::set_error("%s failed: %s (%s:%d)", #expr, cudaGetErrorString(_e),      \
                             __FILE__, __LINE__);                                         \
            return 1;                                                                     \
        }                                                                                 \
    } while (0)

#define KIRAG_CHECK(cond, ...)                                                            \
    do {                                                                                  \
        if (!(cond)) {                                                                    \
            kirag::set_error(__VA_ARGS__);                                                \
            return 1;                                                                     \
        }                                                                                 \
    } while (0)

#define KIRAG_LAUNCH_OK(name)                                                             \
    do {                                                                                  \
        cudaError_t _e = cudaGetLastError();                                              \
        if (_e != cudaSuccess) {                                                          \
            kirag::set_error("launch of %s failed: %s (%s:%d)", name,                     \
                             cudaGetErrorString(_e), __FILE__, __LINE__);                 \
            return 1;                                                                     \
        }                                                                                 \
        kirag::count_launch();                                                            \
    } while (0)

int ensure_dynamic_smem_impl(const void* kernel, size_t bytes);
template <typename K>
inline int ensure_dynamic_smem(K kernel, size_t bytes) {
    return ensure_dynamic_smem_impl(reinterpret_cast<const void*>(kernel), bytes);
}

#ifdef __CUDACC__
__device__ __forceinline__ void pdl_launch_dependents() { asm volatile("griddepcontrol.launch_dependents;" ::: "memory"); }
__device__ __forceinline__ void pdl_wait() { asm volatile("griddepcontrol.wait;" ::: "memory"); }
#endif
bool pdl_enabled();

template <typename... KArgs, typename... Args>
inline cudaError_t launch_chained(void (*kernel)(KArgs...), dim3 grid, dim3 block, size_t smem, cudaStream_t st,
                                  Args... args) {
    cudaLaunchConfig_t cfg = {};
    cfg.gridDim = grid;
    cfg.blockDim = block;
    cfg.dynamicSmemBytes = smem;
    cfg.stream = st;
    cudaLaunchAttribute attr[1];
    attr[0].id = cudaLaunchAttributeProgrammaticStreamSerialization;
    attr[0].val.programmaticStreamSerializationAllowed = 1;
    cfg.attrs = attr;
    cfg.numAttrs = pdl_enabled() ? 1 : 0;
    return cudaLaunchKernelEx(&cfg, kernel, static_cast<KArgs>(args)...);
}

constexpr int kTileRows = 128;
constexpr int kKChunk = 64;
constexpr int kChunkBytes = 16;

__host__ __device__ __forceinline__ size_t shadow_offset(int64_t r, int c, int d, int rows_per_tile) {
    const int64_t tile = r / rows_per_tile;
    const int rr = (int)(r - tile * rows_per_tile);
    const int kc = c >> 6;
    const int cc = c & 63;
    const int g = cc >> 3;
    const size_t tile_bytes = (size_t)rows_per_tile * d * 2;
    const size_t block_bytes = (size_t)rows_per_tile * 128;
    return (size_t)tile * tile_bytes + (size_t)kc * block_bytes + (size_t)rr * 128 +
           (size_t)((g ^ (rr & 7)) << 4) + (size_t)(cc & 7) * 2;
}

__host__ __device__ __forceinline__ uint32_t score_key(float f) {
    if (!(f == f)) return 0u;
    f += 0.0f;
#ifdef __CUDA_ARCH__
    uint32_t u = __float_as_uint(f);
#else
    union { float f; uint32_t u; } cv; cv.f = f; uint32_t u = cv.u;
#endif
    return (u & 0x80000000u) ? ~u : (u | 0x80000000u);
}
__host__ __device__ __forceinline__ float key_score(uint32_t k) {
    uint32_t u = (k & 0x80000000u) ? (k & 0x7fffffffu) : ~k;
#ifdef __CUDA_ARCH__
    return __uint_as_float(u);
#else
    union { float f; uint32_t u; } cv; cv.u = u; return cv.f;
#endif
}
__host__ __device__ __forceinline__ uint64_t pack_item(float score, int32_t id) {
    return ((uint64_t)score_key(score) << 32) | (uint64_t)(0xffffffffu - (uint32_t)id);
}
__host__ __device__ __forceinline__ int32_t item_id(uint64_t it) {
    return (int32_t)(0xffffffffu - (uint32_t)(it & 0xffffffffu));
}
__host__ __device__ __forceinline__ uint32_t item_key(uint64_t it) { return (uint32_t)(it >> 32); }

struct __align__(8) Cand {
    float s;
    int32_t id;
};

#ifdef __CUDACC__
__device__ __forceinline__ float canonical_partial(const float* __restrict__ x,
                                                   const float* __restrict__ q, int d, int lane,
                                                   bool vec4) {
    float acc = 0.0f;
    if (vec4) {
#pragma unroll 8
        for (int c = lane * 4; c < d; c += 128) {
            const float4 xv = *reinterpret_cast<const float4*>(x + c);
            const float4 qv = *reinterpret_cast<const float4*>(q + c);
            acc = __fmaf_rn(xv.x, qv.x, acc);
            acc = __fmaf_rn(xv.y, qv.y, acc);
            acc = __fmaf_rn(xv.z, qv.z, acc);
            acc = __fmaf_rn(xv.w, qv.w, acc);
        }
    } else {
        for (int c = lane * 4; c < d; c += 128) {
#pragma unroll
            for (int j = 0; j < 4; ++j)
                if (c + j < d) acc = __fmaf_rn(x[c + j], q[c + j], acc);
        }
    }
    return acc;
}
__device__ __forceinline__ float warp_butterfly_sum(float v) {
    v = __fadd_rn(v, __shfl_xor_sync(0xffffffffu, v, 16));
    v = __fadd_rn(v, __shfl_xor_sync(0xffffffffu, v, 8));
    v = __fadd_rn(v, __shfl_xor_sync(0xffffffffu, v, 4));
    v = __fadd_rn(v, __shfl_xor_sync(0xffffffffu, v, 2));
    v = __fadd_rn(v, __shfl_xor_sync(0xffffffffu, v, 1));
    return v;
}

__device__ __forceinline__ void bitonic_sort_desc(uint64_t* s, int P) {
    for (int size = 2; size <= P; size <<= 1) {
        for (int stride = size >> 1; stride > 0; stride >>= 1) {
            for (int t = threadIdx.x; t < (P >> 1); t += blockDim.x) {
                const int pos = 2 * t - (t & (stride - 1));
                const int par = pos + stride;
                const bool desc = ((pos & size) == 0);
                const uint64_t a = s[pos], b = s[par];
                if ((a < b) == desc) { s[pos] = b; s[par] = a; }
            }
            __syncthreads();
        }
    }
}
#endif

int launch_convert_rows(const float* src, int64_t n_rows, int d, int64_t dst_row0, void* shadow,
                        int rows_per_tile, unsigned* maxnorm2_bits, float* row_norms, float* row_errs,
                        const float* center, float* row_cdot, cudaStream_t st);
int launch_column_sums(const float* src, int64_t n_rows, int d, float* sums, cudaStream_t st);
constexpr int kExactNQ = 8;
int launch_scan_exact(const float* master, int64_t n, int d, const float* q, int nq_valid,
                      float* scores, int64_t ld, int num_sms, cudaStream_t st);
int launch_rescore(const float* master, int d, const float* q, const Cand* cand, const int* cnt,
                   int cand_stride, int m, float* out_scores, int64_t nq, const float* tauk, const float* qnorm,
                   const float* qerr, float eps_a, float eps_b, cudaStream_t st);
constexpr int kSelectSeg = 8192;
constexpr int kWideCap = 32768;
int launch_select_dense(const float* scores, int64_t ld, int64_t n, int nq, int m, Cand* out,
                        int* n_seg_out, cudaStream_t st);
int launch_select_pairs(const Cand* in, int64_t in_stride, const int* cnt, int fixed_count, int cap,
                        int nq, int m, Cand* out, int64_t out_stride, int n_seg, float* tau,
                        int* cnt_out, int* overflow, cudaStream_t st);
int launch_compact_topm(Cand* buf, int64_t stride, int* cnt, int cap, int nq, int m, float* tau, int* overflow,
                        float* tauk, int kth_k, cudaStream_t st);
int launch_tail_fused(Cand* buf, int64_t stride, int* cnt, int cap, int nq, int m, float* tau, int* overflow,
                      const float* master, int d, const float* q, float* rescored, int k, float* D, int64_t* I,
                      int64_t id_offset, const float* qnorm, const float* qerr, const float* qcdot, float eps_a, float eps_b,
                      int* flags, int num_sms, cudaStream_t st);
int launch_final(const Cand* cand, int64_t cand_stride, const float* rescored, const int* cnt,
                 int fixed_count, int m_in, int nq, int k, float* D, int64_t* I, int64_t id_offset,
                 const float* tau, const float* qnorm, const float* qerr, const float* qcdot, float eps_a, float eps_b,
                 int check_cert, const int* overflow, int* flags, const int* qmap, cudaStream_t st);
int launch_merge(const float* D_all, const int64_t* I_all, int G, int64_t nq, int k, float* D_out,
                 int64_t* I_out, cudaStream_t st);
int launch_fill_pad(float* D, int64_t* I, int64_t n, cudaStream_t st);
struct ScanTcPlan {
    int bq;
    int resident;
};
int scan_tc_supported(int d);
int scan_tc_pick(int64_t nq, int d, ScanTcPlan* plan);
size_t scan_tc_qshadow_bytes(int64_t nq, int d, const ScanTcPlan& plan);
int launch_scan_tc(const void* shadow, int64_t n_rows, int d, const void* qshadow, int64_t nq,
                   const ScanTcPlan& plan, int64_t tile_lo, int64_t tile_hi, int64_t n_tiles,
                   int64_t tile_mult, const float* tau, Cand* cand, int* cnt, int cap, int num_sms,
                   int q_dep, cudaStream_t st);
int launch_scan_tc_dump(const void* shadow, int64_t n_rows, int d, const void* qshadow, int64_t nq,
                        const ScanTcPlan& plan, const float* tau_inf, int* cnt_scratch, float* dump,
                        int64_t dump_ld, int num_sms, cudaStream_t st);
constexpr int kRangeRun = 8192;
int launch_range_threshold(const int* qmap, const float* qnorm, const float* qerr, const float* qcdot, float radius,
                           float eps_a, float eps_b, int64_t nb, int64_t nb_pad, float* tau, int* cnt, cudaStream_t st);
int launch_range_count_cand(const Cand* cand, int cap, const float* rescored, int m, const int* cnt, int64_t nq,
                            float radius, int* counts, cudaStream_t st);
int launch_range_collect_cand(const Cand* cand, int cap, const float* rescored, int m, const int* cnt, int64_t nq,
                              float radius, unsigned long long* cursor, uint64_t* items, cudaStream_t st);
int launch_range_count_dense(const float* scores, int64_t ld, int64_t n, int nq, float radius, int* counts,
                             cudaStream_t st);
int launch_range_collect_dense(const float* scores, int64_t ld, int64_t n, int nq, float radius,
                               unsigned long long* cursor, uint64_t* items, cudaStream_t st);
int launch_range_emit(uint64_t* items, uint64_t* items2, int64_t nq, const int64_t* src_off, const int64_t* lims,
                      int n_seg, int64_t longest, int64_t total_long, const int64_t* tab, int64_t id_offset, float* D,
                      int64_t* I, cudaStream_t st);
int launch_pool_normalize(const void* hidden, const void* mask, float* out, void* out_lp, float* pooled_norm,
                          int64_t B, int64_t S, int64_t H, int64_t sb, int64_t ss, int64_t mb,
                          int hidden_dtype, int mask_dtype, int mode, int normalize,
                          cudaStream_t st);
int launch_pool_normalize_backward(const float* grad_out, const float* out, const float* pooled_norm,
                                   const void* mask, void* grad_hidden, int64_t B, int64_t S,
                                   int64_t H, int64_t mb, int hidden_dtype, int mask_dtype, int mode,
                                   int normalize, cudaStream_t st);

}
```

### kirag_b200/csrc/convert.cu

```cuda
#include "common.cuh"

namespace kirag {

__global__ void __launch_bounds__(256)
convert_rows_kernel(const float* __restrict__ src, int64_t n_rows, int d, int64_t dst_row0,
                    uint8_t* __restrict__ shadow, int rows_per_tile,
                    unsigned* __restrict__ maxnorm2_bits, float* __restrict__ row_norms,
                    float* __restrict__ row_errs, const float* __restrict__ center, float* __restrict__ row_cdot) {
    pdl_wait();
    pdl_launch_dependents();
    const int lane = threadIdx.x & 31;
    const int64_t warp = ((int64_t)blockIdx.x * blockDim.x + threadIdx.x) >> 5;
    const int64_t n_warps = ((int64_t)gridDim.x * blockDim.x) >> 5;
    const int n_gran = d >> 3;
    for (int64_t r = warp; r < n_rows; r += n_warps) {
        const float* row = src + r * (int64_t)d;
        float ss = 0.0f;
        float xs = 0.0f;
        float es = 0.0f;
        float cd = 0.0f;
        for (int g = lane; g < n_gran; g += 32) {
            float4 a = *reinterpret_cast<const float4*>(row + g * 8);
            float4 b = *reinterpret_cast<const float4*>(row + g * 8 + 4);
            if (center) {
                const float4 ca = __ldg(reinterpret_cast<const float4*>(center + g * 8));
                const float4 cb = __ldg(reinterpret_cast<const float4*>(center + g * 8 + 4));
                if (row_cdot) {
                    cd = fmaf(a.x, ca.x, cd); cd = fmaf(a.y, ca.y, cd); cd = fmaf(a.z, ca.z, cd); cd = fmaf(a.w, ca.w, cd);
                    cd = fmaf(b.x, cb.x, cd); cd = fmaf(b.y, cb.y, cd); cd = fmaf(b.z, cb.z, cd); cd = fmaf(b.w, cb.w, cd);
                } else {
                    xs = fmaf(a.x, a.x, xs); xs = fmaf(a.y, a.y, xs); xs = fmaf(a.z, a.z, xs); xs = fmaf(a.w, a.w, xs);
                    xs = fmaf(b.x, b.x, xs); xs = fmaf(b.y, b.y, xs); xs = fmaf(b.z, b.z, xs); xs = fmaf(b.w, b.w, xs);
                    a.x = __fsub_rn(a.x, ca.x); a.y = __fsub_rn(a.y, ca.y); a.z = __fsub_rn(a.z, ca.z); a.w = __fsub_rn(a.w, ca.w);
                    b.x = __fsub_rn(b.x, cb.x); b.y = __fsub_rn(b.y, cb.y); b.z = __fsub_rn(b.z, cb.z); b.w = __fsub_rn(b.w, cb.w);
                }
            }
            ss = fmaf(a.x, a.x, ss); ss = fmaf(a.y, a.y, ss);
            ss = fmaf(a.z, a.z, ss); ss = fmaf(a.w, a.w, ss);
            ss = fmaf(b.x, b.x, ss); ss = fmaf(b.y, b.y, ss);
            ss = fmaf(b.z, b.z, ss); ss = fmaf(b.w, b.w, ss);
            __nv_bfloat162 p0 = __floats2bfloat162_rn(a.x, a.y);
            __nv_bfloat162 p1 = __floats2bfloat162_rn(a.z, a.w);
            __nv_bfloat162 p2 = __floats2bfloat162_rn(b.x, b.y);
            __nv_bfloat162 p3 = __floats2bfloat162_rn(b.z, b.w);
            {
                const float2 r0 = __bfloat1622float2(p0), r1 = __bfloat1622float2(p1);
                const float2 r2 = __bfloat1622float2(p2), r3 = __bfloat1622float2(p3);
                float e;
                e = a.x - r0.x; es = fmaf(e, e, es); e = a.y - r0.y; es = fmaf(e, e, es);
                e = a.z - r1.x; es = fmaf(e, e, es); e = a.w - r1.y; es = fmaf(e, e, es);
                e = b.x - r2.x; es = fmaf(e, e, es); e = b.y - r2.y; es = fmaf(e, e, es);
                e = b.z - r3.x; es = fmaf(e, e, es); e = b.w - r3.y; es = fmaf(e, e, es);
            }
            uint4 o;
            o.x = *reinterpret_cast<uint32_t*>(&p0);
            o.y = *reinterpret_cast<uint32_t*>(&p1);
            o.z = *reinterpret_cast<uint32_t*>(&p2);
            o.w = *reinterpret_cast<uint32_t*>(&p3);
            const size_t off = shadow_offset(dst_row0 + r, g * 8, d, rows_per_tile);
            *reinterpret_cast<uint4*>(shadow + off) = o;
        }
        ss = warp_butterfly_sum(ss);
        es = warp_butterfly_sum(es);
        if (center && !row_cdot) xs = warp_butterfly_sum(xs); else xs = ss;
        if (row_cdot) cd = warp_butterfly_sum(cd);
        if (lane == 0) {
            if (row_norms) row_norms[r] = sqrtf(ss);
            if (row_errs) row_errs[r] = (es == es) ? sqrtf(es) : INFINITY;
            if (row_cdot) row_cdot[r] = center ? cd : 0.0f;
            if (maxnorm2_bits) {
                unsigned bits = (ss == ss) ? __float_as_uint(ss) : 0x7f800000u;
                atomicMax(maxnorm2_bits, bits);
                unsigned ebits = (es == es) ? __float_as_uint(es) : 0x7f800000u;
                atomicMax(maxnorm2_bits + 1, ebits);
                unsigned xbits = (xs == xs) ? __float_as_uint(xs) : 0x7f800000u;
                atomicMax(maxnorm2_bits + 2, xbits);
            }
        }
    }
}

__global__ void __launch_bounds__(256)
column_sums_kernel(const float* __restrict__ src, int64_t n_rows, int d, int rows_per_block, float* __restrict__ sums) {
    const int64_t r0 = (int64_t)blockIdx.x * rows_per_block;
    int64_t r1 = r0 + rows_per_block;
    if (r1 > n_rows) r1 = n_rows;
    float sq = 0.0f;
    for (int c = threadIdx.x; c < d; c += blockDim.x) {
        float acc = 0.0f;
        int64_t r = r0;
        for (; r + 4 <= r1; r += 4) {
            const float v0 = src[r * (int64_t)d + c], v1 = src[(r + 1) * (int64_t)d + c];
            const float v2 = src[(r + 2) * (int64_t)d + c], v3 = src[(r + 3) * (int64_t)d + c];
            acc += (v0 + v1) + (v2 + v3);
            sq = fmaf(v0, v0, fmaf(v1, v1, fmaf(v2, v2, fmaf(v3, v3, sq))));
        }
        for (; r < r1; ++r) {
            const float v = src[r * (int64_t)d + c];
            acc += v;
            sq = fmaf(v, v, sq);
        }
        atomicAdd(sums + c, acc);
    }
    sq = warp_butterfly_sum(sq);
    if ((threadIdx.x & 31) == 0) atomicAdd(sums + d, sq);
}

__global__ void __launch_bounds__(256)
row_norms_kernel(const float* __restrict__ src, int64_t n_rows, int d,
                 unsigned* __restrict__ maxnorm2_bits, float* __restrict__ row_norms) {
    const int lane = threadIdx.x & 31;
    const int64_t warp = ((int64_t)blockIdx.x * blockDim.x + threadIdx.x) >> 5;
    const int64_t n_warps = ((int64_t)gridDim.x * blockDim.x) >> 5;
    for (int64_t r = warp; r < n_rows; r += n_warps) {
        const float* row = src + r * (int64_t)d;
        float ss = 0.0f;
        for (int c = lane; c < d; c += 32) ss = fmaf(row[c], row[c], ss);
        ss = warp_butterfly_sum(ss);
        if (lane == 0) {
            if (row_norms) row_norms[r] = sqrtf(ss);
            if (maxnorm2_bits) {
                unsigned bits = (ss == ss) ? __float_as_uint(ss) : 0x7f800000u;
                atomicMax(maxnorm2_bits, bits);
            }
        }
    }
}

int launch_column_sums(const float* src, int64_t n_rows, int d, float* sums, cudaStream_t st) {
    if (n_rows <= 0) return 0;
    const int rows_per_block = 16;
    column_sums_kernel<<<(unsigned)((n_rows + rows_per_block - 1) / rows_per_block), 256, 0, st>>>(src, n_rows, d,
                                                                                                    rows_per_block, sums);
    KIRAG_LAUNCH_OK("column_sums_kernel");
    return 0;
}

int launch_convert_rows(const float* src, int64_t n_rows, int d, int64_t dst_row0, void* shadow,
                        int rows_per_tile, unsigned* maxnorm2_bits, float* row_norms, float* row_errs,
                        const float* center, float* row_cdot, cudaStream_t st) {
    if (n_rows <= 0) return 0;
    const int threads = 256;
    const int64_t warps_needed = n_rows;
    int64_t blocks = (warps_needed * 32 + threads - 1) / threads;
    if (blocks > 148 * 16) blocks = 148 * 16;
    if (shadow) {
        KIRAG_CHECK(d % 64 == 0, "convert: d=%d is not a multiple of 64", d);
        KIRAG_CUDA_OK(launch_chained(convert_rows_kernel, dim3((unsigned)blocks), dim3(threads), 0, st, src, n_rows, d,
                                     dst_row0, (uint8_t*)shadow, rows_per_tile, maxnorm2_bits, row_norms, row_errs, center,
                                     row_cdot));
        KIRAG_LAUNCH_OK("convert_rows_kernel");
    } else {
        row_norms_kernel<<<(unsigned)blocks, threads, 0, st>>>(src, n_rows, d, maxnorm2_bits,
                                                              row_norms);
        KIRAG_LAUNCH_OK("row_norms_kernel");
    }
    return 0;
}

}
```

### kirag_b200/csrc/rescore.cu

```cuda
#include "common.cuh"

namespace kirag {

__global__ void __launch_bounds__(256)
rescore_kernel(const float* __restrict__ master, int d, const float* __restrict__ q,
               const Cand* __restrict__ cand, const int* __restrict__ cnt, int cand_stride, int m,
               float* __restrict__ out, int64_t nq, bool vec4, const float* __restrict__ tauk,
               const float* __restrict__ qnorm, const float* __restrict__ qerr, float eps_a, float eps_b) {
    pdl_wait();
    pdl_launch_dependents();
    const int lane = threadIdx.x & 31;
    const int64_t warp = ((int64_t)blockIdx.x * blockDim.x + threadIdx.x) >> 5;
    if (warp >= nq * m) return;
    const int64_t qi = warp / m;
    const int j = (int)(warp - qi * m);
    int count = cnt ? cnt[qi] : m;
    if (count > m) count = m;
    float result = __int_as_float(0x7fc00000);
    if (j < count) {
        const Cand cd = cand[qi * (int64_t)cand_stride + j];
        const int32_t row = cd.id;
        bool needed = true;
        if (tauk) needed = cd.s >= __ldcg(tauk + qi) - 2.0f * (eps_a * __ldcg(qnorm + qi) + eps_b * __ldcg(qerr + qi));
        if (row >= 0 && needed) {
            const float* x = master + (int64_t)row * d;
            const float part = canonical_partial(x, q + qi * (int64_t)d, d, lane, vec4);
            result = warp_butterfly_sum(part);
        }
    }
    if (lane == 0) out[qi * (int64_t)m + j] = result;
}

int launch_rescore(const float* master, int d, const float* q, const Cand* cand, const int* cnt,
                   int cand_stride, int m, float* out_scores, int64_t nq, const float* tauk, const float* qnorm,
                   const float* qerr, float eps_a, float eps_b, cudaStream_t st) {
    if (nq <= 0 || m <= 0) return 0;
    const int threads = 256;
    const int64_t warps = nq * m;
    const int64_t blocks = (warps + (threads / 32) - 1) / (threads / 32);
    KIRAG_CHECK(blocks < 0x7fffffffLL, "rescore: too many candidates (%lld warps)", (long long)warps);
    const bool vec4 = (d % 4 == 0) && ((reinterpret_cast<uintptr_t>(master) & 15) == 0) &&
                      ((reinterpret_cast<uintptr_t>(q) & 15) == 0);
    KIRAG_CUDA_OK(launch_chained(rescore_kernel, dim3((unsigned)blocks), dim3(threads), 0, st, master, d, q, cand, cnt,
                                 cand_stride, m, out_scores, nq, vec4, tauk, qnorm, qerr, eps_a, eps_b));
    KIRAG_LAUNCH_OK("rescore_kernel");
    return 0;
}

}
```

### kirag_b200/csrc/scan_tc.cu

```cuda
#include "common.cuh"
#include <cstdio>

namespace kirag {

constexpr int kMaxStages = 12;
constexpr int kBlockBytes = kTileRows * 128;
constexpr int kSmemLimit = 227 * 1024;

__device__ __forceinline__ uint32_t smem_u32(const void* p) {
    return (uint32_t)__cvta_generic_to_shared(p);
}
__device__ __forceinline__ void mbar_init(uint64_t* bar, uint32_t count) {
    asm volatile("mbarrier.init.shared::cta.b64 [%0], %1;" ::"r"(smem_u32(bar)), "r"(count));
}
__device__ __forceinline__ void mbar_expect_tx(uint64_t* bar, uint32_t bytes) {
    asm volatile("mbarrier.arrive.expect_tx.shared::cta.b64 _, [%0], %1;" ::"r"(smem_u32(bar)), "r"(bytes)
                 : "memory");
}
__device__ __forceinline__ bool mbar_try_wait(uint64_t* bar, uint32_t parity) {
    uint32_t ok;
    asm volatile(
        "{\n\t.reg .pred p;\n\t"
        "mbarrier.try_wait.parity.shared::cta.b64 p, [%1], %2;\n\t"
        "selp.u32 %0, 1, 0, p;\n\t}"
        : "=r"(ok)
        : "r"(smem_u32(bar)), "r"(parity)
        : "memory");
    return ok != 0;
}
__device__ __forceinline__ void mbar_wait(uint64_t* bar, uint32_t parity, int tag) {
    if (mbar_try_wait(bar, parity)) return;
    const long long t0 = clock64();
    while (!mbar_try_wait(bar, parity)) {
        if (clock64() - t0 > 8000000000LL) {
            printf("kirag scan_tc: mbarrier wait timed out (tag %d, block %d, thread %d, parity %u)\n", tag,
                   blockIdx.x, threadIdx.x, parity);
            __trap();
        }
    }
}
__device__ __forceinline__ void mbar_wait_warp(uint64_t* bar, uint32_t parity, int tag, int lane) {
    if (lane == 0) mbar_wait(bar, parity, tag);
    __syncwarp();
}
__device__ __forceinline__ bool elect_one() {
    uint32_t pred;
    asm volatile(
        "{\n\t.reg .pred P;\n\t"
        "elect.sync _|P, 0xffffffff;\n\t"
        "selp.u32 %0, 1, 0, P;\n\t}"
        : "=r"(pred));
    return pred != 0;
}
__device__ __forceinline__ void fence_barrier_init() {
    asm volatile("fence.mbarrier_init.release.cluster;" ::: "memory");
}
__device__ __forceinline__ uint64_t policy_evict_first() {
    uint64_t p;
    asm volatile("createpolicy.fractional.L2::evict_first.b64 %0, 1.0;" : "=l"(p));
    return p;
}
__device__ __forceinline__ uint64_t policy_evict_last() {
    uint64_t p;
    asm volatile("createpolicy.fractional.L2::evict_last.b64 %0, 1.0;" : "=l"(p));
    return p;
}
__device__ __forceinline__ void bulk_g2s(void* dst_smem, const void* src_gmem, uint32_t bytes, uint64_t* bar,
                                         uint64_t policy) {
    asm volatile(
        "cp.async.bulk.shared::cluster.global.mbarrier::complete_tx::bytes.L2::cache_hint [%0], [%1], %2, [%3], %4;"
        ::"r"(smem_u32(dst_smem)), "l"(src_gmem), "r"(bytes), "r"(smem_u32(bar)), "l"(policy)
        : "memory");
}
__device__ __forceinline__ void tc_fence_before() { asm volatile("tcgen05.fence::before_thread_sync;" ::: "memory"); }
__device__ __forceinline__ void tc_fence_after() { asm volatile("tcgen05.fence::after_thread_sync;" ::: "memory"); }
__device__ __forceinline__ uint32_t cluster_ctarank() {
    uint32_t r;
    asm volatile("mov.u32 %0, %%cluster_ctarank;" : "=r"(r));
    return r;
}
__device__ __forceinline__ void cluster_sync_all() {
    asm volatile("barrier.cluster.arrive.release.aligned;" ::: "memory");
    asm volatile("barrier.cluster.wait.acquire.aligned;" ::: "memory");
}
__device__ __forceinline__ uint32_t map_to_rank(const void* p, uint32_t rank) {
    uint32_t r;
    asm volatile("mapa.shared::cluster.u32 %0, %1, %2;" : "=r"(r) : "r"(smem_u32(p)), "r"(rank));
    return r;
}
__device__ __forceinline__ void mbar_arrive_cluster(uint32_t cluster_addr) {
    asm volatile("mbarrier.arrive.shared::cluster.b64 _, [%0];" ::"r"(cluster_addr) : "memory");
}
__device__ __forceinline__ void tmem_alloc2(uint32_t* holder_smem, uint32_t ncols) {
    asm volatile("tcgen05.alloc.cta_group::2.sync.aligned.shared::cta.b32 [%0], %1;" ::"r"(smem_u32(holder_smem)),
                 "r"(ncols)
                 : "memory");
    asm volatile("tcgen05.relinquish_alloc_permit.cta_group::2.sync.aligned;" ::: "memory");
}
__device__ __forceinline__ void tmem_dealloc2(uint32_t taddr, uint32_t ncols) {
    asm volatile("tcgen05.dealloc.cta_group::2.sync.aligned.b32 %0, %1;" ::"r"(taddr), "r"(ncols) : "memory");
}
__device__ __forceinline__ void umma_bf16_2cta(uint32_t tmem_d, uint64_t desc_a, uint64_t desc_b, uint32_t idesc,
                                               uint32_t accumulate) {
    asm volatile(
        "{\n\t.reg .pred p;\n\t"
        "setp.ne.b32 p, %4, 0;\n\t"
        "tcgen05.mma.cta_group::2.kind::f16 [%0], %1, %2, %3, p;\n\t}"
        ::"r"(tmem_d), "l"(desc_a), "l"(desc_b), "r"(idesc), "r"(accumulate)
        : "memory");
}
__device__ __forceinline__ void umma_commit_2cta(uint64_t* bar, uint16_t mask) {
    asm volatile(
        "tcgen05.commit.cta_group::2.mbarrier::arrive::one.shared::cluster.multicast::cluster.b64 [%0], %1;"
        ::"r"(smem_u32(bar)), "h"(mask)
        : "memory");
}
__device__ __forceinline__ void tmem_ld32(uint32_t taddr, uint32_t (&v)[32]) {
    asm volatile(
        "tcgen05.ld.sync.aligned.32x32b.x32.b32 "
        "{%0, %1, %2, %3, %4, %5, %6, %7, %8, %9, %10, %11, %12, %13, %14, %15, "
        "%16, %17, %18, %19, %20, %21, %22, %23, %24, %25, %26, %27, %28, %29, %30, %31}, [%32];"
        : "=r"(v[0]), "=r"(v[1]), "=r"(v[2]), "=r"(v[3]), "=r"(v[4]), "=r"(v[5]), "=r"(v[6]), "=r"(v[7]),
          "=r"(v[8]), "=r"(v[9]), "=r"(v[10]), "=r"(v[11]), "=r"(v[12]), "=r"(v[13]), "=r"(v[14]), "=r"(v[15]),
          "=r"(v[16]), "=r"(v[17]), "=r"(v[18]), "=r"(v[19]), "=r"(v[20]), "=r"(v[21]), "=r"(v[22]), "=r"(v[23]),
          "=r"(v[24]), "=r"(v[25]), "=r"(v[26]), "=r"(v[27]), "=r"(v[28]), "=r"(v[29]), "=r"(v[30]), "=r"(v[31])
        : "r"(taddr)
        : "memory");
}
__device__ __forceinline__ uint32_t tmem_ld1(uint32_t taddr) {
    uint32_t r;
    asm volatile("tcgen05.ld.sync.aligned.32x32b.x1.b32 {%0}, [%1];" : "=r"(r) : "r"(taddr) : "memory");
    return r;
}
__device__ __forceinline__ void tmem_ld_wait() { asm volatile("tcgen05.wait::ld.sync.aligned;" ::: "memory"); }

__device__ __forceinline__ uint64_t make_sw128_desc(uint32_t smem_addr) {
    uint64_t d = 0;
    d |= (uint64_t)((smem_addr & 0x3ffffu) >> 4);
    d |= (uint64_t)1 << 16;
    d |= (uint64_t)(1024 >> 4) << 32;
    d |= (uint64_t)1 << 46;
    d |= (uint64_t)2 << 61;
    return d;
}
__host__ __device__ constexpr uint32_t make_idesc_bf16(int M, int N) {
    return (1u << 4) | (1u << 7) | (1u << 10) | ((uint32_t)(N >> 3) << 17) | ((uint32_t)(M >> 4) << 24);
}

struct ScanArgs {
    const uint8_t* shadow;
    const uint8_t* qshadow;
    int64_t n_rows;
    int d;
    int64_t nq;
    int64_t tile_lo, tile_hi, n_tiles, tile_mult;
    const float* tau;
    Cand* cand;
    int* cnt;
    int cap;
    int n_stages;
    int q_dep;
    float* dump;
    int64_t dump_ld;
};

__device__ __forceinline__ uint32_t pass_mask(const ScanArgs& a, const uint32_t (&v)[32], int64_t q0, int64_t row,
                                              bool row_ok, float mytau) {
    uint32_t pass = 0;
#pragma unroll
    for (int c = 0; c < 32; ++c) {
        const float t = __shfl_sync(0xffffffffu, mytau, c);
        pass |= (__uint_as_float(v[c]) >= t ? 1u : 0u) << c;
    }
    if (!row_ok) pass = 0;
    if (a.dump && row_ok) {
#pragma unroll
        for (int c = 0; c < 32; ++c)
            if (q0 + c < a.nq) a.dump[row * a.dump_ld + q0 + c] = __uint_as_float(v[c]);
    }
    return pass;
}

constexpr int kStash = 4;
struct Stash {
    uint32_t sv[kStash];
    int sc[kStash];
    int slot[kStash];
    int n;
    int64_t q0;
    int32_t row;
};
__device__ __forceinline__ void stash_clear(Stash& st) {
    st.n = 0;
    st.q0 = 0;
    st.row = 0;
#pragma unroll
    for (int j = 0; j < kStash; ++j) { st.sv[j] = 0; st.sc[j] = 0; st.slot[j] = -1; }
}
__device__ __forceinline__ void stash_reserve(const ScanArgs& a, Stash& st) {
#pragma unroll
    for (int j = 0; j < kStash; ++j) {
        st.slot[j] = -1;
        if (st.n > j && st.q0 + st.sc[j] < a.nq) st.slot[j] = atomicAdd(a.cnt + st.q0 + st.sc[j], 1);
    }
}
__device__ __forceinline__ void stash_store(const ScanArgs& a, const Stash& st) {
#pragma unroll
    for (int j = 0; j < kStash; ++j) {
        if (st.n > j && st.slot[j] >= 0 && st.slot[j] < a.cap) {
            Cand cd;
            cd.s = __uint_as_float(st.sv[j]);
            cd.id = st.row;
            a.cand[(st.q0 + st.sc[j]) * (int64_t)a.cap + st.slot[j]] = cd;
        }
    }
}

__device__ __forceinline__ uint32_t warp_transpose_bits(uint32_t x, int lane) {
#pragma unroll
    for (int s = 0; s < 5; ++s) {
        const int j = 16 >> s;
        const uint32_t m = (s == 0) ? 0x0000ffffu : (s == 1) ? 0x00ff00ffu : (s == 2) ? 0x0f0f0f0fu
                         : (s == 3) ? 0x33333333u : 0x55555555u;
        const uint32_t t = __shfl_xor_sync(0xffffffffu, x, j);
        x = (lane & j) ? ((x & ~m) | ((t & ~m) >> j)) : ((x & m) | ((t & m) << j));
    }
    return x;
}

__device__ __forceinline__ uint32_t select32(const uint32_t (&v)[32], int c) {
    uint32_t a[16];
#pragma unroll
    for (int i = 0; i < 16; ++i) a[i] = (c & 16) ? v[16 + i] : v[i];
#pragma unroll
    for (int i = 0; i < 8; ++i) a[i] = (c & 8) ? a[8 + i] : a[i];
#pragma unroll
    for (int i = 0; i < 4; ++i) a[i] = (c & 4) ? a[4 + i] : a[i];
#pragma unroll
    for (int i = 0; i < 2; ++i) a[i] = (c & 2) ? a[2 + i] : a[i];
    return (c & 1) ? a[1] : a[0];
}

__device__ __forceinline__ void handle_survivors(const ScanArgs& a, const uint32_t (&v)[32], uint32_t pass,
                                                 int64_t q0g, int col_g, int32_t row, int lane, Stash& st) {
    if (__all_sync(0xffffffffu, pass == 0xffffffffu)) {
        int mybase = a.cap;
        if (q0g + lane < a.nq) mybase = atomicAdd(a.cnt + q0g + lane, 32);
#pragma unroll
        for (int c = 0; c < 32; ++c) {
            const int slot = __shfl_sync(0xffffffffu, mybase, c) + lane;
            if (slot < a.cap) {
                Cand cd;
                cd.s = __uint_as_float(v[c]);
                cd.id = row;
                a.cand[(q0g + c) * (int64_t)a.cap + slot] = cd;
            }
        }
        return;
    }
    const bool dense = __any_sync(0xffffffffu, st.n + __popc(pass) > kStash);
    if (!dense) {
        for (uint32_t u = pass; u; u &= u - 1) {
            const int c = __ffs(u) - 1;
            const uint32_t val = select32(v, c);
#pragma unroll
            for (int j = 0; j < kStash; ++j)
                if (st.n == j) { st.sv[j] = val; st.sc[j] = col_g + c; }
            ++st.n;
        }
        return;
    }
    uint32_t loc[32];
#pragma unroll
    for (int c = 0; c < 32; ++c) loc[c] = v[c];
    uint32_t mybal = warp_transpose_bits(pass, lane);
    if (q0g + lane >= a.nq) mybal = 0;
    int mybase = 0;
    if (mybal != 0) mybase = atomicAdd(a.cnt + q0g + lane, __popc(mybal));
    const unsigned lt = (1u << lane) - 1u;
    const int iters = __reduce_max_sync(0xffffffffu, __popc(pass));
    uint32_t u = pass;
    for (int i = 0; i < iters; ++i) {
        const bool has = u != 0;
        const int c = has ? (__ffs(u) - 1) : 0;
        u &= u - 1;
        const unsigned bal = __shfl_sync(0xffffffffu, mybal, c);
        const int base = __shfl_sync(0xffffffffu, mybase, c);
        if (has) {
            const int slot = base + __popc(bal & lt);
            if (slot < a.cap && ((bal >> lane) & 1u)) {
                Cand cd;
                cd.s = __uint_as_float(loc[c]);
                cd.id = row;
                a.cand[(q0g + c) * (int64_t)a.cap + slot] = cd;
            }
        }
    }
}

template <int NG, typename Release>
__device__ __forceinline__ void filter_item(const ScanArgs& a, uint32_t taddr, int64_t q0, int64_t row, bool row_ok,
                                            int lane, Stash& st, const float (&mytau)[NG], Release release) {
    stash_clear(st);
    st.q0 = q0;
    st.row = (int32_t)row;
#pragma unroll 1
    for (int g = 0; g < NG; ++g) {
        uint32_t v[32];
        tmem_ld32(taddr + g * 32, v);
        tmem_ld_wait();
        const uint32_t pass = pass_mask(a, v, q0 + g * 32, row, row_ok, mytau[g]);
        if (__any_sync(0xffffffffu, pass != 0))
            handle_survivors(a, v, pass, q0 + g * 32, g * 32, (int32_t)row, lane, st);
    }
    release();
}

template <int BQ> struct EpiCfg {
    static constexpr int kWarps = (BQ >= 128) ? 8 : 4;
    static constexpr int kThreads = 64 + 32 * kWarps;
    static constexpr int kGroups = BQ / 32 / (kWarps / 4);
};

template <int PQ, bool RES> struct PairCfg {
    static constexpr int kHalfQ = PQ / 2;
    static constexpr int kQHalfBytes = kHalfQ * 128;
    static constexpr int kStageBytes = kBlockBytes + (RES ? 0 : kQHalfBytes);
};

template <int PQ, bool RES>
__global__ void __cluster_dims__(2, 1, 1) __launch_bounds__(EpiCfg<PQ>::kThreads, 1)
scan_tc_pair_kernel(const ScanArgs a) {
    constexpr int kHalfQ = PairCfg<PQ, RES>::kHalfQ;
    constexpr int kQHalfBytes = PairCfg<PQ, RES>::kQHalfBytes;
    constexpr int kStageBytes = PairCfg<PQ, RES>::kStageBytes;
    constexpr uint16_t kPairMask = 0x3;
    extern __shared__ uint8_t smem_raw[];
    uint8_t* smem = reinterpret_cast<uint8_t*>((reinterpret_cast<uintptr_t>(smem_raw) + 1023) & ~(uintptr_t)1023);
    const int KC = a.d >> 6;
    const int NS = a.n_stages;
    uint8_t* stage_base = smem;
    uint8_t* q_res = smem + (size_t)NS * kStageBytes;
    uint8_t* tail = q_res + (RES ? (size_t)KC * kQHalfBytes : 0);
    uint64_t* full_bar = reinterpret_cast<uint64_t*>(tail);
    uint64_t* empty_bar = full_bar + kMaxStages;
    uint64_t* tmem_full = empty_bar + kMaxStages;
    uint64_t* tmem_empty = tmem_full + 2;
    uint64_t* q_bar = tmem_empty + 2;
    uint32_t* tmem_holder = reinterpret_cast<uint32_t*>(q_bar + 1);

    const int warp = threadIdx.x >> 5;
    const int lane = threadIdx.x & 31;
    const uint32_t rank = cluster_ctarank();
    const int64_t pair = blockIdx.x / 2;
    const int64_t n_pairs = gridDim.x / 2;
    constexpr uint32_t kTmemCols = 2 * PQ;
    const int n_qt = (int)((a.nq + PQ - 1) / PQ);
    const int64_t W = ((a.tile_hi - a.tile_lo + 1) / 2) * n_qt;
    const int64_t w_lo = W * pair / n_pairs;
    const int64_t w_hi = W * (pair + 1) / n_pairs;

    if (threadIdx.x == 0) {
        for (int s = 0; s < NS; ++s) { mbar_init(&full_bar[s], rank == 0 ? 2 : 1); mbar_init(&empty_bar[s], 1); }
        for (int s = 0; s < 2; ++s) { mbar_init(&tmem_full[s], 1); mbar_init(&tmem_empty[s], 2 * EpiCfg<PQ>::kWarps); }
        mbar_init(q_bar, rank == 0 ? 2 : 1);
        fence_barrier_init();
    }
    if (warp == 1) tmem_alloc2(tmem_holder, kTmemCols);
    tc_fence_before();
    cluster_sync_all();
    tc_fence_after();
    const uint32_t tmem_base = *tmem_holder;

    if (warp == 0) {
        {
            const uint64_t pol_x = (n_qt == 1) ? policy_evict_first() : policy_evict_last();
            const uint64_t pol_x_last = policy_evict_first();
            const uint64_t pol_q = policy_evict_last();
            if (a.q_dep) pdl_wait();
            if (RES && elect_one()) {
                mbar_expect_tx(q_bar, (uint32_t)(KC * kQHalfBytes));
                bulk_g2s(q_res, a.qshadow + (size_t)rank * ((size_t)a.d * kHalfQ * 2), (uint32_t)(KC * kQHalfBytes),
                         q_bar, pol_q);
            }
            __syncwarp();
            int s = 0;
            uint32_t ph = 0;
            for (int64_t w = w_lo; w < w_hi; ++w) {
                const int64_t p = w / n_qt;
                const int qt = (int)(w - p * n_qt);
                int64_t ti = a.tile_lo + 2 * p + rank;
                if (ti >= a.tile_hi) ti = a.tile_hi - 1;
                const int64_t tile = (ti * a.tile_mult) % a.n_tiles;
                const uint8_t* xsrc = a.shadow + (size_t)tile * ((size_t)a.d * kTileRows * 2);
                const uint8_t* qsrc = a.qshadow + (size_t)(2 * qt + rank) * ((size_t)a.d * kHalfQ * 2);
                const uint64_t pol_xw = (n_qt > 1 && qt == n_qt - 1) ? pol_x_last : pol_x;
                for (int kc = 0; kc < KC; ++kc) {
                    mbar_wait_warp(&empty_bar[s], ph ^ 1u, 100 + s, lane);
                    uint8_t* dst = stage_base + (size_t)s * kStageBytes;
                    if (elect_one()) {
                        mbar_expect_tx(&full_bar[s], (uint32_t)kStageBytes);
                        bulk_g2s(dst, xsrc + (size_t)kc * kBlockBytes, kBlockBytes, &full_bar[s], pol_xw);
                        if (!RES)
                            bulk_g2s(dst + kBlockBytes, qsrc + (size_t)kc * kQHalfBytes, kQHalfBytes, &full_bar[s], pol_q);
                    }
                    __syncwarp();
                    if (++s == NS) { s = 0; ph ^= 1u; }
                }
            }
        }
    } else if (warp == 1) {
        {
            int s = 0;
            uint32_t ph = 0;
            if (rank == 1) {
                if (RES) {
                    mbar_wait_warp(q_bar, 0, 650, lane);
                    if (elect_one()) mbar_arrive_cluster(map_to_rank(q_bar, 0));
                    __syncwarp();
                }
                for (int64_t w = w_lo; w < w_hi; ++w) {
                    for (int kc = 0; kc < KC; ++kc) {
                        mbar_wait_warp(&full_bar[s], ph, 600 + s, lane);
                        if (elect_one()) mbar_arrive_cluster(map_to_rank(&full_bar[s], 0));
                        __syncwarp();
                        if (++s == NS) { s = 0; ph ^= 1u; }
                    }
                }
            } else {
                constexpr uint32_t idesc = make_idesc_bf16(2 * kTileRows, PQ);
                if (RES) mbar_wait_warp(q_bar, 0, 200, lane);
                uint32_t it = 0;
                for (int64_t w = w_lo; w < w_hi; ++w, ++it) {
                    const uint32_t as = it & 1u;
                    const uint32_t aph = (it >> 1) & 1u;
                    mbar_wait_warp(&tmem_empty[as], aph ^ 1u, 300 + as, lane);
                    tc_fence_after();
                    const uint32_t d_tmem = tmem_base + as * PQ;
                    for (int kc = 0; kc < KC; ++kc) {
                        mbar_wait_warp(&full_bar[s], ph, 400 + s, lane);
                        tc_fence_after();
                        const uint32_t xa = smem_u32(stage_base + (size_t)s * kStageBytes);
                        const uint64_t da = make_sw128_desc(xa);
                        const uint64_t db = make_sw128_desc(RES ? smem_u32(q_res + (size_t)kc * kQHalfBytes) : xa + kBlockBytes);
                        if (elect_one()) {
#pragma unroll
                            for (int k4 = 0; k4 < 4; ++k4)
                                umma_bf16_2cta(d_tmem, da + (uint64_t)(k4 * 2), db + (uint64_t)(k4 * 2), idesc,
                                               (kc | k4) ? 1u : 0u);
                            umma_commit_2cta(&empty_bar[s], kPairMask);
                            if (kc == KC - 1) umma_commit_2cta(&tmem_full[as], kPairMask);
                        }
                        __syncwarp();
                        if (++s == NS) { s = 0; ph ^= 1u; }
                    }
                }
            }
        }
    } else {
        const int quad = warp & 3;
        const uint32_t lane_base = (uint32_t)(quad * 32) << 16;
        uint32_t leader_empty[2];
        leader_empty[0] = map_to_rank(&tmem_empty[0], 0);
        leader_empty[1] = map_to_rank(&tmem_empty[1], 0);
        constexpr int NG = EpiCfg<PQ>::kGroups;
        const int col0 = ((warp - 2) >> 2) * (NG * 32);
        uint32_t it = 0;
        Stash pend, cur;
        stash_clear(pend);
        pdl_wait();
        float mytau[NG], nxtau[NG];
        {
            const int qt0 = RES ? 0 : (int)(w_lo % n_qt);
#pragma unroll
            for (int g = 0; g < NG; ++g)
                mytau[g] = (w_lo < w_hi) ? __ldcg(a.tau + (int64_t)qt0 * PQ + col0 + g * 32 + lane) : 0.f;
        }
        for (int64_t w = w_lo; w < w_hi; ++w, ++it) {
            const int64_t p = w / n_qt;
            const int qt = (int)(w - p * n_qt);
            const int64_t ti = a.tile_lo + 2 * p + rank;
            const bool tile_ok = ti < a.tile_hi;
            const int64_t tile = ((tile_ok ? ti : a.tile_hi - 1) * a.tile_mult) % a.n_tiles;
            const int64_t row = tile * kTileRows + quad * 32 + lane;
            const bool row_ok = tile_ok && row < a.n_rows;
            const uint32_t as = it & 1u;
            const uint32_t aph = (it >> 1) & 1u;
            const int qt_next = (qt + 1 == n_qt) ? 0 : qt + 1;
            const bool fetch = !RES && n_qt > 1 && w + 1 < w_hi;
#pragma unroll
            for (int g = 0; g < NG; ++g)
                nxtau[g] = fetch ? __ldcg(a.tau + (int64_t)qt_next * PQ + col0 + g * 32 + lane) : mytau[g];
            mbar_wait(&tmem_full[as], aph, 500 + as);
            tc_fence_after();
            const uint32_t ebar = leader_empty[as];
            filter_item<NG>(a, tmem_base + lane_base + as * PQ + col0, (int64_t)qt * PQ + col0, row, row_ok,
                            lane, cur, mytau, [=]() {
                                tc_fence_before();
                                __syncwarp();
                                if (lane == 0) mbar_arrive_cluster(ebar);
                            });
#pragma unroll
            for (int g = 0; g < NG; ++g) mytau[g] = nxtau[g];
            stash_store(a, pend);
            stash_reserve(a, cur);
            pend = cur;
        }
        stash_store(a, pend);
    }
    pdl_launch_dependents();
    tc_fence_before();
    cluster_sync_all();
    if (warp == 1) {
        tc_fence_after();
        tmem_dealloc2(tmem_base, kTmemCols);
    }
}

int scan_tc_supported(int d) { return (d % 64 == 0 && d >= 64 && d <= 4096) ? 1 : 0; }

template <int PQ, bool RES>
static size_t pair_fixed_bytes(int d) {
    return 1024 + (2 * kMaxStages + 5) * 8 + 16 + (RES ? (size_t)(d / 64) * PairCfg<PQ, RES>::kQHalfBytes : 0);
}
template <int PQ, bool RES>
static int pair_stages(int d) {
    int ns = kMaxStages;
    while (ns > 0 && pair_fixed_bytes<PQ, RES>(d) + (size_t)ns * PairCfg<PQ, RES>::kStageBytes > (size_t)kSmemLimit) --ns;
    return ns;
}

int scan_tc_pick(int64_t nq, int d, ScanTcPlan* plan) {
    KIRAG_CHECK(scan_tc_supported(d), "scan_tc: dimension %d is not supported (need a multiple of 64, <= 4096)", d);
    if (nq <= 64) { plan->bq = 64; plan->resident = pair_stages<64, true>(d) >= 6; }
    else if (nq <= 128) { plan->bq = 128; plan->resident = pair_stages<128, true>(d) >= 4; }
    else { plan->bq = 256; plan->resident = 0; }
    return 0;
}

size_t scan_tc_qshadow_bytes(int64_t nq, int d, const ScanTcPlan& plan) {
    const int64_t tiles = (nq + plan.bq - 1) / plan.bq;
    return (size_t)tiles * plan.bq * d * 2;
}

template <int PQ, bool RES>
static int launch_scan_pair(const ScanArgs& args_in, int num_sms, cudaStream_t st) {
    ScanArgs args = args_in;
    const int ns = pair_stages<PQ, RES>(args.d);
    KIRAG_CHECK(ns >= 2, "scan_tc pair: no room for a shared-memory pipeline");
    KIRAG_CHECK(!RES || args.nq <= PQ, "scan_tc pair: the resident variant takes a single query tile");
    args.n_stages = ns;
    const size_t smem = pair_fixed_bytes<PQ, RES>(args.d) + (size_t)ns * PairCfg<PQ, RES>::kStageBytes;
    if (ensure_dynamic_smem(scan_tc_pair_kernel<PQ, RES>, kSmemLimit)) return 1;
    int64_t pairs = ((args.tile_hi - args.tile_lo + 1) / 2) * ((args.nq + PQ - 1) / PQ);
    if (pairs > num_sms / 2) pairs = num_sms / 2;
    if (pairs <= 0) return 0;
    KIRAG_CUDA_OK(launch_chained(scan_tc_pair_kernel<PQ, RES>, dim3((unsigned)(2 * pairs)), dim3(EpiCfg<PQ>::kThreads), smem, st, args));
    KIRAG_LAUNCH_OK("scan_tc_pair_kernel");
    return 0;
}

static int launch_scan_args(const ScanArgs& args, const ScanTcPlan& plan, int num_sms, cudaStream_t st) {
    if (plan.bq == 64 && plan.resident) return launch_scan_pair<64, true>(args, num_sms, st);
    if (plan.bq == 64 && !plan.resident) return launch_scan_pair<64, false>(args, num_sms, st);
    if (plan.bq == 128 && plan.resident) return launch_scan_pair<128, true>(args, num_sms, st);
    if (plan.bq == 128 && !plan.resident) return launch_scan_pair<128, false>(args, num_sms, st);
    if (plan.bq == 256 && !plan.resident) return launch_scan_pair<256, false>(args, num_sms, st);
    set_error("scan_tc: no kernel for plan (bq=%d resident=%d)", plan.bq, plan.resident);
    return 1;
}

int launch_scan_tc(const void* shadow, int64_t n_rows, int d, const void* qshadow, int64_t nq,
                   const ScanTcPlan& plan, int64_t tile_lo, int64_t tile_hi, int64_t n_tiles,
                   int64_t tile_mult, const float* tau, Cand* cand, int* cnt, int cap, int num_sms,
                   int q_dep, cudaStream_t st) {
    ScanArgs args{};
    args.q_dep = q_dep;
    args.shadow = (const uint8_t*)shadow;
    args.qshadow = (const uint8_t*)qshadow;
    args.n_rows = n_rows;
    args.d = d;
    args.nq = nq;
    args.tile_lo = tile_lo;
    args.tile_hi = tile_hi;
    args.n_tiles = n_tiles;
    args.tile_mult = tile_mult;
    args.tau = tau;
    args.cand = cand;
    args.cnt = cnt;
    args.cap = cap;
    args.dump = nullptr;
    args.dump_ld = 0;
    return launch_scan_args(args, plan, num_sms, st);
}

int launch_scan_tc_dump(const void* shadow, int64_t n_rows, int d, const void* qshadow, int64_t nq,
                        const ScanTcPlan& plan, const float* tau_inf, int* cnt_scratch, float* dump,
                        int64_t dump_ld, int num_sms, cudaStream_t st) {
    ScanArgs args{};
    args.shadow = (const uint8_t*)shadow;
    args.qshadow = (const uint8_t*)qshadow;
    args.n_rows = n_rows;
    args.d = d;
    args.nq = nq;
    args.n_tiles = (n_rows + kTileRows - 1) / kTileRows;
    args.tile_lo = 0;
    args.tile_hi = args.n_tiles;
    args.tile_mult = 1;
    args.tau = tau_inf;
    args.cand = nullptr;
    args.cnt = cnt_scratch;
    args.cap = 0;
    args.dump = dump;
    args.dump_ld = dump_ld;
    args.q_dep = 1;
    return launch_scan_args(args, plan, num_sms, st);
}

}
```

Before: 31620.

## Add int8 tensor-core prefilter tier with bf16 rescore before f32 certification

Adds an int8 shadow copy of the database with per-row metadata, plus int8 query quantization. Large batches scan with an int8 UMMA kernel using a rigorous error-bound slack, then rescore the top-2048 candidates in bf16 before the existing compaction and certification. Queries that fail certification fall back to the full bf16 fast path. This halves the bytes streamed per row and raises tensor-core throughput, in exchange for extra memory, an extra rescore stage and possible fallback work when the bounds are loose.

```diff
diff --git a/include/kirag_b200.h b/include/kirag_b200.h
--- a/include/kirag_b200.h
+++ b/include/kirag_b200.h
@@ -7,7 +7,7 @@
 extern "C" {
 #endif
 
-#define KIRAG_ABI_VERSION 7
+#define KIRAG_ABI_VERSION 8
 
 #define KIRAG_METRIC_INNER_PRODUCT 0
 #define KIRAG_METRIC_L2 1
@@ -40,6 +40,7 @@
     int64_t kernel_launches;
     int64_t n_rescan;
     int64_t n_retry;
+    int64_t n_i8;
 } kirag_search_stats_t;
 
 
diff --git a/kirag_b200/_lib.py b/kirag_b200/_lib.py
--- a/kirag_b200/_lib.py
+++ b/kirag_b200/_lib.py
@@ -7,7 +7,7 @@
 HERE = os.path.dirname(os.path.abspath(__file__))
 LIB_PATH = os.environ.get("KIRAG_B200_LIB") or os.path.join(HERE, "libkirag_b200.so")
 
-ABI_VERSION = 7
+ABI_VERSION = 8
 METRIC_INNER_PRODUCT = 0
 METRIC_L2 = 1
 PATH_AUTO, PATH_EXACT, PATH_FAST = 0, 1, 2
@@ -28,6 +28,7 @@
         ("kernel_launches", c_int64),
         ("n_rescan", c_int64),
         ("n_retry", c_int64),
+        ("n_i8", c_int64),
     ]
 
     def as_dict(self):
diff --git a/kirag_b200/csrc/api.cu b/kirag_b200/csrc/api.cu
--- a/kirag_b200/csrc/api.cu
+++ b/kirag_b200/csrc/api.cu
@@ -246,7 +246,7 @@
 };
 
 struct SearchCounters {
-    int64_t n_fast = 0, n_exact = 0, n_cert_fail = 0, n_overflow = 0, n_rescan = 0, n_retry = 0, n_changed = 0;
+    int64_t n_i8 = 0, n_fast = 0, n_exact = 0, n_cert_fail = 0, n_overflow = 0, n_rescan = 0, n_retry = 0, n_changed = 0;
     int levels = 0;
 };
 
@@ -254,6 +254,7 @@
     bool active = false;
     bool ev_recorded = false;
     bool fast_ok = false;
+    bool i8 = false;
     int mode = 0, path = 0, k = 0;
     int64_t nq = 0, id_offset = 0;
     const float* qd = nullptr;
@@ -274,7 +275,12 @@
     int64_t capacity = 0;
     float* master = nullptr;
     uint8_t* shadow = nullptr;
-    VmBuffer vm_master, vm_shadow;
+    uint8_t* shadow8 = nullptr;
+    float* meta8 = nullptr;
+    int64_t s8_cap = 0, s8_rows = 0;
+    unsigned* min8_bits = nullptr;
+    float emin8 = 0.f, ymin8 = 0.f;
+    VmBuffer vm_master, vm_shadow, vm_shadow8, vm_meta8;
     bool use_vmm = false;
     unsigned* maxnorm2_bits = nullptr;
     float maxnorm = 0.f;
@@ -285,6 +291,7 @@
     bool center_decided = false;
     DevBuf q_dev, D_dev, I_dev, qshadow, qnorm, cand, cnt, tau, tauk, overflow, flags, rescored;
     DevBuf dense, stage_a, stage_b, qmap, qsel, qnorm2, D_tmp, I_tmp, t_dev, center_sums;
+    DevBuf qshadow8, qmeta8, tau8, qfb, qmapfb, Dfb, Ifb;
     int* host_flags = nullptr;
     size_t host_flags_n = 0;
     PendingSearch pending;
@@ -360,6 +367,14 @@
                 h->use_vmm = true;
                 h->master = static_cast<float*>(h->vm_master.ptr());
                 h->shadow = want_shadow ? static_cast<uint8_t*>(h->vm_shadow.ptr()) : nullptr;
+                if (scan_tc_i8_supported(h->d) && h->vm_shadow8.reserve(h->device, max_rows * (size_t)h->d) == 0 &&
+                    h->vm_meta8.reserve(h->device, max_rows * 12) == 0) {
+                    h->shadow8 = static_cast<uint8_t*>(h->vm_shadow8.ptr());
+                    h->meta8 = static_cast<float*>(h->vm_meta8.ptr());
+                } else {
+                    h->vm_shadow8.release();
+                    h->vm_meta8.release();
+                }
             } else {
                 h->vm_master.release();
                 h->vm_shadow.release();
@@ -533,8 +548,26 @@
     return e;
 }
 
+constexpr int kI8KPrime = 2048;
+constexpr int64_t kI8MinQueries = 1024;
+constexpr int64_t kI8MinRows = (int64_t)1 << 22;
+static bool i8_eligible(const kirag_index* h, int64_t nq, const FastParams& fp) {
+    if (!(h->shadow8 && h->s8_rows == h->ntotal && nq >= kI8MinQueries && h->ntotal >= kI8MinRows &&
+          fp.kprime <= kI8KPrime)) return false;
+    FastParams fpl = fp;
+    fpl.few_queries = 0;
+    const std::vector<int64_t> b = level_bounds((h->ntotal + kTileRows - 1) / kTileRows, pick_cap(fp, nq), fpl);
+    for (size_t i = 2; i < b.size(); ++i)
+        if (b[i] > b[i - 1] * (kWideCap / (2 * kI8KPrime))) return false;
+    return true;
+}
+static float i8_slack(const kirag_index* h) {
+    const double yn = (double)h->maxnorm, xn = (double)h->maxnorm_x, cn = (double)h->center_norm;
+    return (float)(((double)h->d * ldexp(1.0, -22) * xn + ldexp(1.0, -24) * yn + 64.0 * ldexp(1.0, -24) * cn) * 1.002);
+}
+
 static int fast_search(kirag_index* h, const float* qd, int64_t nq, int k, float* D, int64_t* I,
-                       int64_t id_offset, const FastParams& fp, int check_cert, int* levels_out,
+                       int64_t id_offset, const FastParams& fp, int check_cert, int* levels_out, bool i8,
                        cudaStream_t st) {
     const int d = h->d;
     const int64_t n = h->ntotal;
@@ -547,7 +580,9 @@
     const size_t qs_bytes = scan_tc_qshadow_bytes(nq, d, plan);
     if (h->qshadow.ensure(qs_bytes)) return 1;
     if (h->qnorm.ensure((size_t)nq * 12)) return 1;
-    const int cap = pick_cap(fp, nq);
+    const int cap_sched = pick_cap(fp, nq);
+    const int cap = i8 ? kWideCap : cap_sched;
+    const int m_scan = i8 ? kI8KPrime : fp.kprime;
     if (h->cand.ensure((size_t)nq * cap * sizeof(Cand))) return 1;
     if (h->cnt.ensure((size_t)nq * 4)) return 1;
     const int64_t nq_pad = round_up(nq, 256);
@@ -556,9 +591,23 @@
     if (h->flags.ensure((size_t)nq * 4)) return 1;
     if (h->rescored.ensure((size_t)nq * fp.kprime * 4)) return 1;
     if (h->tauk.ensure((size_t)nq * 4)) return 1;
-    const bool fuse_tail = cap == kWideCap && fp.kprime <= 2048;
+    const bool fuse_tail = !i8 && cap == kWideCap && fp.kprime <= 2048;
     if ((nq % plan.bq) != 0)
         KIRAG_CUDA_OK(cudaMemsetAsync(h->qshadow.p, 0, qs_bytes, st));
+    ScanTcPlan plan8 = plan;
+    plan8.i8 = 1;
+    ScanI8Args a8{};
+    if (i8) {
+        const size_t qs8_bytes = scan_tc_qshadow_bytes(nq, d, plan8);
+        const size_t meta_bytes = (size_t)(nq_pad * 3 + (nq_pad / 256) * 2) * 4;
+        if (h->qshadow8.ensure(qs8_bytes) || h->qmeta8.ensure(meta_bytes) || h->tau8.ensure((size_t)nq * 4)) return 1;
+        if ((nq % plan8.bq) != 0) KIRAG_CUDA_OK(cudaMemsetAsync(h->qshadow8.p, 0, qs8_bytes, st));
+        KIRAG_CUDA_OK(cudaMemsetAsync(h->qmeta8.p, 0, meta_bytes, st));
+        a8.rowmeta = h->meta8;
+        a8.qscale = h->qmeta8.as<float>();
+        a8.tile_ab = h->qmeta8.as<float>() + nq_pad * 3;
+        a8.slack = i8_slack(h);
+    }
     KIRAG_CUDA_OK(launch_chained(init_search_state_kernel, dim3((unsigned)((nq_pad + 255) / 256)), dim3(256), 0, st,
                                  h->tau.as<float>(), h->cnt.as<int>(), h->overflow.as<int>(), nq, nq_pad));
     KIRAG_LAUNCH_OK("init_search_state_kernel");
@@ -566,13 +615,15 @@
     float* const qcdot = h->qnorm.as<float>() + 2 * nq;
     if (launch_convert_rows(qd, nq, d, 0, h->qshadow.p, plan.bq / 2, nullptr, h->qnorm.as<float>(),
                             h->qnorm.as<float>() + nq, h->center, qcdot, st)) return 1;
+    if (i8 && launch_convert_rows_s8(qd, nq, d, 0, h->qshadow8.p, plan8.bq / 2, nullptr, h->qmeta8.as<float>(),
+                                     h->qmeta8.as<float>() + nq_pad * 3, nullptr, st)) return 1;
     prof_mark(1, st);
 
     const int64_t n_tiles = (n + kTileRows - 1) / kTileRows;
     const int64_t mult = pick_tile_mult(n_tiles);
     FastParams fpl = fp;
     fpl.few_queries = nq <= kFewQueries ? 1 : 0;
-    const std::vector<int64_t> bounds = level_bounds(n_tiles, cap, fpl);
+    const std::vector<int64_t> bounds = level_bounds(n_tiles, cap_sched, fpl);
     int64_t lo = 0;
     int levels = 0;
     for (const int64_t hi : bounds) {
@@ -582,9 +633,9 @@
             KIRAG_CUDA_OK(cudaEventCreate(&e1));
             KIRAG_CUDA_OK(cudaEventRecord(e0, st));
         }
-        if (launch_scan_tc(h->shadow, n, d, h->qshadow.p, nq, plan, lo, hi, n_tiles, mult,
-                           h->tau.as<float>(), h->cand.as<Cand>(), h->cnt.as<int>(), cap, h->num_sms,
-                           levels == 0 ? 1 : 0, st)) return 1;
+        if (launch_scan_tc(i8 ? h->shadow8 : h->shadow, n, d, i8 ? h->qshadow8.p : h->qshadow.p, nq, i8 ? plan8 : plan, lo,
+                           hi, n_tiles, mult, h->tau.as<float>(), h->cand.as<Cand>(), h->cnt.as<int>(), cap, h->num_sms,
+                           levels == 0 ? 1 : 0, st, i8 ? &a8 : nullptr)) return 1;
         if (g_prof.on) {
             KIRAG_CUDA_OK(cudaEventRecord(e1, st));
             g_prof.ev.emplace_back(e0, e1);
@@ -596,14 +647,24 @@
         prof_mark(10 + levels, st);
         const bool last = (hi == bounds.back());
         if (last && fuse_tail) break;
-        if (launch_compact_topm(h->cand.as<Cand>(), cap, h->cnt.as<int>(), cap, (int)nq, fp.kprime,
-                                h->tau.as<float>(), h->overflow.as<int>(), last ? h->tauk.as<float>() : nullptr,
+        if (launch_compact_topm(h->cand.as<Cand>(), cap, h->cnt.as<int>(), cap, (int)nq, m_scan,
+                                h->tau.as<float>(), h->overflow.as<int>(), (last && !i8) ? h->tauk.as<float>() : nullptr,
                                 k, st)) return 1;
         prof_mark(30 + levels, st);
         ++levels;
         lo = hi;
     }
     const CertEps ce = cert_eps(h);
+    if (i8) {
+        if (launch_bf16_rescore(h->shadow, d, qd, h->cand.as<Cand>(), h->cnt.as<int>(), cap, kI8KPrime, nq,
+                                h->tau.as<float>(), h->tau8.as<float>(), st)) return 1;
+        if (launch_compact_topm(h->cand.as<Cand>(), cap, h->cnt.as<int>(), cap, (int)nq, fp.kprime, h->tau.as<float>(),
+                                h->overflow.as<int>(), h->tauk.as<float>(), k, st)) return 1;
+        if (launch_tier2_threshold(h->tau.as<float>(), h->tau8.as<float>(), h->qnorm.as<float>(), h->qnorm.as<float>() + nq,
+                                   ce.a, ce.b, h->qmeta8.as<float>(), h->qmeta8.as<float>() + nq_pad * 3, h->emin8,
+                                   h->ymin8, nq, st)) return 1;
+        prof_mark(40, st);
+    }
     if (fuse_tail) {
         ++levels;
         if (launch_tail_fused(h->cand.as<Cand>(), cap, h->cnt.as<int>(), cap, (int)nq, fp.kprime, h->tau.as<float>(),
@@ -694,8 +755,9 @@
 }
 
 static int enqueue_chunk(kirag_index* h, const float* qd, int64_t cq, int k, float* Dd, int64_t* Id, int64_t id_offset,
-                         bool fast_ok, const FastParams& fp, SearchCounters* c, int* mode, cudaStream_t st) {
+                         bool fast_ok, const FastParams& fp, SearchCounters* c, int* mode, bool* i8, cudaStream_t st) {
     *mode = 0;
+    *i8 = false;
     if (h->ntotal == 0) return launch_fill_pad(Dd, Id, cq * k, st);
     if (!fast_ok) {
         if (exact_search(h, qd, cq, k, Dd, Id, 0, nullptr, id_offset, st)) return 1;
@@ -703,7 +765,8 @@
         return 0;
     }
     if (ensure_host_flags(h, cq)) return 1;
-    if (fast_search(h, qd, cq, k, Dd, Id, id_offset, fp, 1, &c->levels, st)) return 1;
+    *i8 = i8_eligible(h, cq, fp);
+    if (fast_search(h, qd, cq, k, Dd, Id, id_offset, fp, 1, &c->levels, *i8, st)) return 1;
     KIRAG_CUDA_OK(cudaMemcpyAsync(h->host_flags, h->flags.p, (size_t)cq * 4, cudaMemcpyDeviceToHost, st));
     *mode = 1;
     return 0;
@@ -748,7 +811,7 @@
         gentle.growth_override = 4;
         gentle.first_growth_override = 2;
         if (fast_search(h, h->qsel.as<float>(), nb, k, h->D_tmp.as<float>(), h->I_tmp.as<int64_t>(), id_offset, gentle, 1,
-                        nullptr, st)) return 1;
+                        nullptr, false, st)) return 1;
         std::vector<int> f2((size_t)nb);
         KIRAG_CUDA_OK(cudaMemcpyAsync(f2.data(), h->flags.p, (size_t)nb * 4, cudaMemcpyDeviceToHost, st));
         scatter_rows_kernel<<<(unsigned)nb, 128, 0, st>>>(h->D_tmp.as<float>(), h->I_tmp.as<int64_t>(), h->qmap.as<int>(), k,
@@ -797,6 +860,35 @@
     return 0;
 }
 
+static int resolve_i8_chunk(kirag_index* h, const float* qd, int64_t cq, int k, float* Dd, int64_t* Id, int64_t id_offset,
+                            int path, const FastParams& fp, SearchCounters* c, cudaStream_t st) {
+    const int d = h->d;
+    std::vector<int> fb;
+    for (int64_t i = 0; i < cq; ++i)
+        if (h->host_flags[(size_t)i]) fb.push_back((int)i);
+    const int64_t nb = (int64_t)fb.size();
+    c->n_i8 += cq - nb;
+    c->n_fast += cq - nb;
+    if (nb == 0) return 0;
+    if (h->qmapfb.ensure((size_t)nb * 4) || h->qfb.ensure((size_t)nb * d * 4)) return 1;
+    if (h->Dfb.ensure((size_t)nb * k * 4) || h->Ifb.ensure((size_t)nb * k * 8)) return 1;
+    KIRAG_CUDA_OK(cudaMemcpyAsync(h->qmapfb.p, fb.data(), (size_t)nb * 4, cudaMemcpyHostToDevice, st));
+    gather_rows_kernel<<<(unsigned)nb, 256, 0, st>>>(qd, h->qmapfb.as<int>(), d, h->qfb.as<float>());
+    KIRAG_LAUNCH_OK("gather_rows_kernel");
+    if (fast_search(h, h->qfb.as<float>(), nb, k, h->Dfb.as<float>(), h->Ifb.as<int64_t>(), id_offset, fp, 1, nullptr, false,
+                    st)) return 1;
+    KIRAG_CUDA_OK(cudaMemcpyAsync(h->host_flags, h->flags.p, (size_t)nb * 4, cudaMemcpyDeviceToHost, st));
+    KIRAG_CUDA_OK(cudaStreamSynchronize(st));
+    const int64_t changed0 = c->n_changed;
+    if (resolve_chunk(h, h->qfb.as<float>(), nb, k, h->Dfb.as<float>(), h->Ifb.as<int64_t>(), id_offset, path, fp, c, st))
+        return 1;
+    scatter_rows_kernel<<<(unsigned)nb, 128, 0, st>>>(h->Dfb.as<float>(), h->Ifb.as<int64_t>(), h->qmapfb.as<int>(), k, Dd, Id);
+    KIRAG_LAUNCH_OK("scatter_rows_kernel");
+    KIRAG_CUDA_OK(cudaStreamSynchronize(st));
+    c->n_changed = changed0 + nb;
+    return 0;
+}
+
 static void fill_stats(kirag_search_stats_t* stats, int64_t nq, const SearchCounters& c, bool fast_ok, int path,
                        long long launches0) {
     if (!stats) return;
@@ -807,6 +899,7 @@
     stats->n_overflow = c.n_overflow;
     stats->n_rescan = c.n_rescan;
     stats->n_retry = c.n_retry;
+    stats->n_i8 = c.n_i8;
     stats->levels = c.levels;
     stats->path = fast_ok ? path : KIRAG_PATH_EXACT;
     stats->kernel_launches = g_launches.load() - launches0;
@@ -831,7 +924,8 @@
     if (p.ev_recorded) KIRAG_CUDA_OK(cudaEventSynchronize(h->pending_ev));
     else KIRAG_CUDA_OK(cudaStreamSynchronize(p.st));
     SearchCounters c = p.counters;
-    if (p.mode == 1 && resolve_chunk(h, p.qd, p.nq, p.k, p.Dd, p.Id, p.id_offset, p.path, p.fp, &c, p.st)) return 1;
+    if (p.mode == 1 && (p.i8 ? resolve_i8_chunk(h, p.qd, p.nq, p.k, p.Dd, p.Id, p.id_offset, p.path, p.fp, &c, p.st)
+                              : resolve_chunk(h, p.qd, p.nq, p.k, p.Dd, p.Id, p.id_offset, p.path, p.fp, &c, p.st))) return 1;
     fill_stats(stats, p.nq, c, p.fast_ok, p.path, p.launches0);
     if (n_changed) *n_changed = c.n_changed;
     return 0;
@@ -872,7 +966,8 @@
             qd = h->q_dev.as<float>(); Dd = h->D_dev.as<float>(); Id = h->I_dev.as<int64_t>();
         }
         int mode = 0;
-        if (enqueue_chunk(h, qd, cq, k, Dd, Id, id_offset, fast_ok, fp, &c, &mode, st)) return 1;
+        bool i8 = false;
+        if (enqueue_chunk(h, qd, cq, k, Dd, Id, id_offset, fast_ok, fp, &c, &mode, &i8, st)) return 1;
         if (!ptrs_are_device) {
             KIRAG_CUDA_OK(cudaMemcpyAsync(D + q0 * k, Dd, (size_t)cq * k * 4, cudaMemcpyDeviceToHost, st));
             KIRAG_CUDA_OK(cudaMemcpyAsync(I + q0 * k, Id, (size_t)cq * k * 8, cudaMemcpyDeviceToHost, st));
@@ -880,7 +975,8 @@
         if (mode == 1 || !ptrs_are_device) KIRAG_CUDA_OK(cudaStreamSynchronize(st));
         if (mode == 1) {
             const int64_t changed0 = c.n_changed;
-            if (resolve_chunk(h, qd, cq, k, Dd, Id, id_offset, path, fp, &c, st)) return 1;
+            if (i8 ? resolve_i8_chunk(h, qd, cq, k, Dd, Id, id_offset, path, fp, &c, st)
+                   : resolve_chunk(h, qd, cq, k, Dd, Id, id_offset, path, fp, &c, st)) return 1;
             if (!ptrs_are_device && c.n_changed != changed0) {
                 KIRAG_CUDA_OK(cudaMemcpyAsync(D + q0 * k, Dd, (size_t)cq * k * 4, cudaMemcpyDeviceToHost, st));
                 KIRAG_CUDA_OK(cudaMemcpyAsync(I + q0 * k, Id, (size_t)cq * k * 8, cudaMemcpyDeviceToHost, st));
@@ -1180,6 +1276,36 @@
     return 0;
 }
 
+static int s8_storage(kirag_index* h, cudaStream_t st) {
+    const int64_t cap = h->capacity;
+    if (h->s8_cap >= cap && h->shadow8) return 0;
+    if (!h->min8_bits && cudaMalloc((void**)&h->min8_bits, 8) != cudaSuccess) { h->min8_bits = nullptr; cudaGetLastError(); return 1; }
+    if (h->use_vmm) {
+        if (h->shadow8 && h->vm_shadow8.ensure((size_t)cap * h->d) == 0 && h->vm_meta8.ensure((size_t)cap * 12) == 0) {
+            h->s8_cap = cap;
+            return 0;
+        }
+        h->s8_rows = 0;
+        return 1;
+    }
+    cudaStreamSynchronize(st);
+    if (h->shadow8) cudaFree(h->shadow8);
+    if (h->meta8) cudaFree(h->meta8);
+    h->shadow8 = nullptr;
+    h->meta8 = nullptr;
+    h->s8_cap = h->s8_rows = 0;
+    if (cudaMalloc((void**)&h->shadow8, (size_t)cap * h->d) != cudaSuccess ||
+        cudaMalloc((void**)&h->meta8, (size_t)cap * 12) != cudaSuccess) {
+        if (h->shadow8) cudaFree(h->shadow8);
+        h->shadow8 = nullptr;
+        h->meta8 = nullptr;
+        cudaGetLastError();
+        return 1;
+    }
+    h->s8_cap = cap;
+    return 0;
+}
+
 static int finalize_rows(kirag_index* h, int64_t r0, int64_t n, cudaStream_t st) {
     if (h->shadow && !h->center_decided && r0 + n >= kCenterMinRows) {
         if (decide_center(h, r0 + n, st)) return 1;
@@ -1192,6 +1318,18 @@
     }
     if (launch_convert_rows(h->master + r0 * (int64_t)h->d, n, h->d, r0, h->shadow, kTileRows, h->maxnorm2_bits, nullptr,
                             nullptr, h->center, nullptr, st)) return 1;
+    if (scan_tc_i8_supported(h->d) && r0 + n >= kI8MinRows && s8_storage(h, st) == 0 && h->s8_rows < r0 + n) {
+        const int64_t s0 = h->s8_rows;
+        if (s0 == 0) KIRAG_CUDA_OK(cudaMemsetAsync(h->min8_bits, 0xff, 8, st));
+        if (launch_convert_rows_s8(h->master + s0 * (int64_t)h->d, r0 + n - s0, h->d, s0, h->shadow8, kTileRows, h->center,
+                                   h->meta8, nullptr, h->min8_bits, st)) return 1;
+        unsigned mb[2];
+        KIRAG_CUDA_OK(cudaMemcpyAsync(mb, h->min8_bits, 8, cudaMemcpyDeviceToHost, st));
+        KIRAG_CUDA_OK(cudaStreamSynchronize(st));
+        memcpy(&h->emin8, &mb[0], 4);
+        memcpy(&h->ymin8, &mb[1], 4);
+        h->s8_rows = r0 + n;
+    }
     if (h->shadow && ((r0 + n) % kTileRows) != 0) {
         const int64_t end = r0 + n;
         const int64_t tile = end / kTileRows;
@@ -1326,16 +1464,21 @@
     if (h->use_vmm) {
         h->vm_master.release();
         h->vm_shadow.release();
+        h->vm_shadow8.release();
+        h->vm_meta8.release();
     } else {
         if (h->master) cudaFree(h->master);
         if (h->shadow) cudaFree(h->shadow);
+        if (h->shadow8) cudaFree(h->shadow8);
+        if (h->meta8) cudaFree(h->meta8);
     }
     if (h->maxnorm2_bits) cudaFree(h->maxnorm2_bits);
+    if (h->min8_bits) cudaFree(h->min8_bits);
     if (h->center) cudaFree(h->center);
     DevBuf* bufs[] = {&h->q_dev, &h->D_dev, &h->I_dev, &h->qshadow, &h->qnorm, &h->cand, &h->cnt, &h->tau, &h->tauk,
                       &h->overflow, &h->flags, &h->rescored, &h->dense, &h->stage_a, &h->stage_b, &h->qmap, &h->qsel, &h->qnorm2, &h->t_dev, &h->center_sums,
                       &h->D_tmp, &h->I_tmp, &h->ritems, &h->ritems2, &h->rcount, &h->rcursor, &h->roff, &h->rtab,
-                      &h->rD, &h->rI};
+                      &h->rD, &h->rI, &h->qshadow8, &h->qmeta8, &h->tau8, &h->qfb, &h->qmapfb, &h->Dfb, &h->Ifb};
     for (DevBuf* b : bufs) b->release();
     if (h->host_flags) cudaFreeHost(h->host_flags);
     if (h->pending_ev) cudaEventDestroy(h->pending_ev);
@@ -1413,7 +1556,7 @@
     p.launches0 = g_launches.load();
     p.fast_ok = h->ntotal > 0 && fast_eligible(h, k, &p.fp);
     p.path = KIRAG_PATH_AUTO;
-    if (enqueue_chunk(h, q, nq, k, D, I, id_offset, p.fast_ok, p.fp, &p.counters, &p.mode, st)) return 1;
+    if (enqueue_chunk(h, q, nq, k, D, I, id_offset, p.fast_ok, p.fp, &p.counters, &p.mode, &p.i8, st)) return 1;
     cudaStreamCaptureStatus cap = cudaStreamCaptureStatusNone;
     cudaStreamIsCapturing(st, &cap);
     if (cap == cudaStreamCaptureStatusNone) {
@@ -1452,12 +1595,21 @@
     mix((uint64_t)h->ntotal);
     mix((uint64_t)(uintptr_t)h->master);
     mix((uint64_t)(uintptr_t)h->shadow);
+    mix((uint64_t)(uintptr_t)h->shadow8);
+    mix((uint64_t)(uintptr_t)h->meta8);
+    mix((uint64_t)h->s8_rows);
+    {
+        uint32_t m8[2];
+        memcpy(&m8[0], &h->emin8, 4); memcpy(&m8[1], &h->ymin8, 4);
+        mix(((uint64_t)m8[0] << 32) | m8[1]);
+    }
     mix((uint64_t)(uintptr_t)h->center);
     uint32_t f[4];
     memcpy(&f[0], &h->maxnorm, 4); memcpy(&f[1], &h->maxerr, 4); memcpy(&f[2], &h->maxnorm_x, 4); memcpy(&f[3], &h->center_norm, 4);
     mix(((uint64_t)f[0] << 32) | f[1]);
     mix(((uint64_t)f[2] << 32) | f[3]);
-    const DevBuf* bufs[] = {&h->qshadow, &h->qnorm, &h->cand, &h->cnt, &h->tau, &h->tauk, &h->overflow, &h->flags, &h->rescored};
+    const DevBuf* bufs[] = {&h->qshadow, &h->qnorm, &h->cand, &h->cnt, &h->tau, &h->tauk, &h->overflow, &h->flags, &h->rescored,
+                            &h->qshadow8, &h->qmeta8, &h->tau8};
     for (const DevBuf* b : bufs) { mix((uint64_t)(uintptr_t)b->p); mix((uint64_t)b->bytes); }
     mix((uint64_t)(uintptr_t)h->host_flags);
     *token = x;
@@ -1502,20 +1654,35 @@
     if (scan_tc_pick(nq, d, &plan)) return 1;
     const char* force = getenv("KIRAG_DEBUG_BQ");
     if (force && *force) {
-        static const struct { const char* name; int bq, resident; } kVariants[] = {
-            {"64r", 64, 1}, {"64s", 64, 0}, {"128r", 128, 1}, {"128s", 128, 0}, {"256s", 256, 0}};
+        static const struct { const char* name; int bq, resident, i8; } kVariants[] = {
+            {"64r", 64, 1, 0}, {"64s", 64, 0, 0}, {"128r", 128, 1, 0}, {"128s", 128, 0, 0}, {"256s", 256, 0, 0},
+            {"256i", 256, 0, 1}};
         bool found = false;
         for (const auto& v : kVariants)
-            if (strcmp(force, v.name) == 0) { plan.bq = v.bq; plan.resident = v.resident; found = true; }
-        KIRAG_CHECK(found, "debug_scores: KIRAG_DEBUG_BQ=%s is not one of 64r, 64s, 128r, 128s, 256s", force);
-    }
-    const size_t qs_bytes = scan_tc_qshadow_bytes(nq, d, plan);
+            if (strcmp(force, v.name) == 0) { plan.bq = v.bq; plan.resident = v.resident; plan.i8 = v.i8; found = true; }
+        KIRAG_CHECK(found, "debug_scores: KIRAG_DEBUG_BQ=%s is not one of 64r, 64s, 128r, 128s, 256s, 256i", force);
+        KIRAG_CHECK(!plan.i8 || scan_tc_i8_supported(d), "debug_scores: no int8 scan at d=%d (needs d %% 128 == 0)", d);
+    }
+    ScanTcPlan plan16 = plan;
+    plan16.i8 = 0;
+    const size_t qs_bytes = scan_tc_qshadow_bytes(nq, d, plan16);
+    const size_t qs8_bytes = scan_tc_qshadow_bytes(nq, d, plan);
     const int64_t nq_pad = round_up(nq, 256);
-    DevBuf qd, qs, tau, cnt, dump, cdot;
+    const size_t meta_bytes = (size_t)(nq_pad * 3 + (nq_pad / 256) * 2) * 4;
+    const size_t xs8_bytes = plan.i8 ? (size_t)round_up(h->ntotal, kTileRows) * d : 0;
+    DevBuf qd, qs, tau, cnt, dump, cdot, qmeta, qs8, xs8, xmeta8;
     std::vector<float> cdot_host;
     int rc = 1;
     do {
-        if (cdot.ensure((size_t)nq_pad * 4)) break;
+        if (cdot.ensure((size_t)nq_pad * 4) || qmeta.ensure(meta_bytes) || qs8.ensure(qs8_bytes)) break;
+        if (cudaMemsetAsync(qmeta.p, 0, meta_bytes, st) != cudaSuccess) break;
+        if (cudaMemsetAsync(qs8.p, 0, qs8_bytes, st) != cudaSuccess) break;
+        if (plan.i8) {
+            if (xs8.ensure(xs8_bytes) || xmeta8.ensure((size_t)round_up(h->ntotal, kTileRows) * 12)) break;
+            if (cudaMemsetAsync(xs8.p, 0, xs8_bytes, st) != cudaSuccess) break;
+            if (launch_convert_rows_s8(h->master, h->ntotal, d, 0, xs8.p, kTileRows, h->center, xmeta8.as<float>(), nullptr,
+                                       nullptr, st)) break;
+        }
         if (qd.ensure((size_t)nq * d * 4) || qs.ensure(qs_bytes) || tau.ensure((size_t)nq_pad * 4) ||
             cnt.ensure((size_t)nq_pad * 4) || dump.ensure((size_t)h->ntotal * nq * 4)) break;
         if (cudaMemcpyAsync(qd.p, q_host, (size_t)nq * d * 4, cudaMemcpyHostToDevice, st) != cudaSuccess) break;
@@ -1525,8 +1692,11 @@
         if (fill_f32(tau.as<float>(), INFINITY, nq_pad, st)) break;
         if (launch_convert_rows(qd.as<float>(), nq, d, 0, qs.p, plan.bq / 2, nullptr, nullptr, nullptr, h->center,
                                 h->center ? cdot.as<float>() : nullptr, st)) break;
-        if (launch_scan_tc_dump(h->shadow, h->ntotal, d, qs.p, nq, plan, tau.as<float>(), cnt.as<int>(),
-                                dump.as<float>(), nq, h->num_sms, st)) break;
+        ScanI8Args a8{xmeta8.as<float>(), qmeta.as<float>(), qmeta.as<float>() + nq_pad * 3, i8_slack(h)};
+        if (plan.i8 && launch_convert_rows_s8(qd.as<float>(), nq, d, 0, qs8.p, plan.bq / 2, nullptr, qmeta.as<float>(),
+                                              qmeta.as<float>() + nq_pad * 3, nullptr, st)) break;
+        if (launch_scan_tc_dump(plan.i8 ? xs8.p : h->shadow, h->ntotal, d, plan.i8 ? qs8.p : qs.p, nq, plan, tau.as<float>(),
+                                cnt.as<int>(), dump.as<float>(), nq, h->num_sms, st, plan.i8 ? &a8 : nullptr)) break;
         if (h->center) {
             cdot_host.resize((size_t)nq);
             if (cudaMemcpyAsync(cdot_host.data(), cdot.p, (size_t)nq * 4, cudaMemcpyDeviceToHost, st) != cudaSuccess) break;
@@ -1541,7 +1711,7 @@
                 for (int64_t qi = 0; qi < nq; ++qi) out_host[r * nq + qi] += cdot_host[(size_t)qi];
         rc = 0;
     } while (0);
-    qd.release(); qs.release(); tau.release(); cnt.release(); dump.release(); cdot.release();
+    qd.release(); qs.release(); tau.release(); cnt.release(); dump.release(); cdot.release(); qmeta.release(); qs8.release(); xs8.release(); xmeta8.release();
     return rc;
 }
 
@@ -1810,6 +1980,7 @@
         return 0;
     }
     h->ntotal = 0;
+    h->s8_rows = 0;
     h->maxnorm = h->maxerr = h->maxnorm_x = h->center_norm = 0.f;
     h->center_decided = false;
     if (h->center) { cudaFree(h->center); h->center = nullptr; }
diff --git a/kirag_b200/csrc/common.cuh b/kirag_b200/csrc/common.cuh
--- a/kirag_b200/csrc/common.cuh
+++ b/kirag_b200/csrc/common.cuh
@@ -72,16 +72,17 @@
 constexpr int kKChunk = 64;
 constexpr int kChunkBytes = 16;
 
-__host__ __device__ __forceinline__ size_t shadow_offset(int64_t r, int c, int d, int rows_per_tile) {
+__host__ __device__ __forceinline__ size_t shadow_offset(int64_t r, int c, int d, int rows_per_tile, int elem_bytes = 2) {
     const int64_t tile = r / rows_per_tile;
     const int rr = (int)(r - tile * rows_per_tile);
-    const int kc = c >> 6;
-    const int cc = c & 63;
-    const int g = cc >> 3;
-    const size_t tile_bytes = (size_t)rows_per_tile * d * 2;
+    const int per_row = 128 / elem_bytes;
+    const int kc = c / per_row;
+    const int cb = (c - kc * per_row) * elem_bytes;
+    const int g = cb >> 4;
+    const size_t tile_bytes = (size_t)rows_per_tile * d * elem_bytes;
     const size_t block_bytes = (size_t)rows_per_tile * 128;
     return (size_t)tile * tile_bytes + (size_t)kc * block_bytes + (size_t)rr * 128 +
-           (size_t)((g ^ (rr & 7)) << 4) + (size_t)(cc & 7) * 2;
+           (size_t)((g ^ (rr & 7)) << 4) + (size_t)(cb & 15);
 }
 
 __host__ __device__ __forceinline__ uint32_t score_key(float f) {
@@ -167,6 +168,9 @@
 int launch_convert_rows(const float* src, int64_t n_rows, int d, int64_t dst_row0, void* shadow,
                         int rows_per_tile, unsigned* maxnorm2_bits, float* row_norms, float* row_errs,
                         const float* center, float* row_cdot, cudaStream_t st);
+int launch_convert_rows_s8(const float* src, int64_t n_rows, int d, int64_t dst_row0, void* shadow8,
+                           int rows_per_tile, const float* center, float* meta, float* tile_ab, unsigned* min_bits,
+                           cudaStream_t st);
 int launch_column_sums(const float* src, int64_t n_rows, int d, float* sums, cudaStream_t st);
 constexpr int kExactNQ = 8;
 int launch_scan_exact(const float* master, int64_t n, int d, const float* q, int nq_valid,
@@ -174,6 +178,10 @@
 int launch_rescore(const float* master, int d, const float* q, const Cand* cand, const int* cnt,
                    int cand_stride, int m, float* out_scores, int64_t nq, const float* tauk, const float* qnorm,
                    const float* qerr, float eps_a, float eps_b, cudaStream_t st);
+int launch_bf16_rescore(const void* shadow, int d, const float* q, Cand* cand, const int* cnt, int cand_stride, int m,
+                        int64_t nq, float* tau, float* tau8, cudaStream_t st);
+int launch_tier2_threshold(float* tau, const float* tau8, const float* qnorm, const float* qerr, float eps_a, float eps_b,
+                           const float* qmeta, const float* tile_ab, float emin, float ymin, int64_t nq, cudaStream_t st);
 constexpr int kSelectSeg = 8192;
 constexpr int kWideCap = 32768;
 int launch_select_dense(const float* scores, int64_t ld, int64_t n, int nq, int m, Cand* out,
@@ -197,17 +205,25 @@
 struct ScanTcPlan {
     int bq;
     int resident;
+    int i8;
+};
+struct ScanI8Args {
+    const float* rowmeta;
+    const float* qscale;
+    const float* tile_ab;
+    float slack;
 };
 int scan_tc_supported(int d);
+int scan_tc_i8_supported(int d);
 int scan_tc_pick(int64_t nq, int d, ScanTcPlan* plan);
 size_t scan_tc_qshadow_bytes(int64_t nq, int d, const ScanTcPlan& plan);
 int launch_scan_tc(const void* shadow, int64_t n_rows, int d, const void* qshadow, int64_t nq,
                    const ScanTcPlan& plan, int64_t tile_lo, int64_t tile_hi, int64_t n_tiles,
                    int64_t tile_mult, const float* tau, Cand* cand, int* cnt, int cap, int num_sms,
-                   int q_dep, cudaStream_t st);
+                   int q_dep, cudaStream_t st, const ScanI8Args* i8 = nullptr);
 int launch_scan_tc_dump(const void* shadow, int64_t n_rows, int d, const void* qshadow, int64_t nq,
                         const ScanTcPlan& plan, const float* tau_inf, int* cnt_scratch, float* dump,
-                        int64_t dump_ld, int num_sms, cudaStream_t st);
+                        int64_t dump_ld, int num_sms, cudaStream_t st, const ScanI8Args* i8 = nullptr);
 constexpr int kRangeRun = 8192;
 int launch_range_threshold(const int* qmap, const float* qnorm, const float* qerr, const float* qcdot, float radius,
                            float eps_a, float eps_b, int64_t nb, int64_t nb_pad, float* tau, int* cnt, cudaStream_t st);
diff --git a/kirag_b200/csrc/convert.cu b/kirag_b200/csrc/convert.cu
--- a/kirag_b200/csrc/convert.cu
+++ b/kirag_b200/csrc/convert.cu
@@ -81,6 +81,84 @@
 }
 
 __global__ void __launch_bounds__(256)
+convert_rows_s8_kernel(const float* __restrict__ src, int64_t n_rows, int d, int64_t dst_row0,
+                       uint8_t* __restrict__ shadow8, int rows_per_tile, const float* __restrict__ center,
+                       float* __restrict__ meta, unsigned* __restrict__ tile_ab, unsigned* __restrict__ min_bits) {
+    pdl_wait();
+    pdl_launch_dependents();
+    const int lane = threadIdx.x & 31;
+    const int64_t warp = ((int64_t)blockIdx.x * blockDim.x + threadIdx.x) >> 5;
+    const int64_t n_warps = ((int64_t)gridDim.x * blockDim.x) >> 5;
+    const int n_gran = d >> 4;
+    for (int64_t r = warp; r < n_rows; r += n_warps) {
+        const float* row = src + r * (int64_t)d;
+        float mx = 0.0f;
+        bool finite = true;
+        for (int c = lane * 4; c < d; c += 128) {
+            float4 a = *reinterpret_cast<const float4*>(row + c);
+            if (center) {
+                const float4 ca = __ldg(reinterpret_cast<const float4*>(center + c));
+                a.x = __fsub_rn(a.x, ca.x); a.y = __fsub_rn(a.y, ca.y); a.z = __fsub_rn(a.z, ca.z); a.w = __fsub_rn(a.w, ca.w);
+            }
+            finite = finite && isfinite(a.x) && isfinite(a.y) && isfinite(a.z) && isfinite(a.w);
+            mx = fmaxf(mx, fmaxf(fmaxf(fabsf(a.x), fabsf(a.y)), fmaxf(fabsf(a.z), fabsf(a.w))));
+        }
+#pragma unroll
+        for (int o = 16; o > 0; o >>= 1) mx = fmaxf(mx, __shfl_xor_sync(0xffffffffu, mx, o));
+        finite = __all_sync(0xffffffffu, finite);
+        const float s = finite ? mx / 127.0f : 0.0f;
+        const float inv = (s > 0.0f) ? 127.0f / mx : 0.0f;
+        double es = 0.0, ys = 0.0;
+        for (int g = lane; g < n_gran; g += 32) {
+            uint32_t packed[4];
+#pragma unroll
+            for (int j = 0; j < 4; ++j) {
+                float4 a = *reinterpret_cast<const float4*>(row + g * 16 + j * 4);
+                if (center) {
+                    const float4 ca = __ldg(reinterpret_cast<const float4*>(center + g * 16 + j * 4));
+                    a.x = __fsub_rn(a.x, ca.x); a.y = __fsub_rn(a.y, ca.y); a.z = __fsub_rn(a.z, ca.z); a.w = __fsub_rn(a.w, ca.w);
+                }
+                const float y[4] = {a.x, a.y, a.z, a.w};
+                uint32_t w = 0;
+#pragma unroll
+                for (int e = 0; e < 4; ++e) {
+                    const float qf = fminf(fmaxf(rintf(y[e] * inv), -127.0f), 127.0f);
+                    const double err = (double)y[e] - (double)s * (double)qf;
+                    es = fma(err, err, es);
+                    ys = fma((double)y[e], (double)y[e], ys);
+                    w |= ((uint32_t)(int)qf & 0xffu) << (8 * e);
+                }
+                packed[j] = w;
+            }
+            const size_t off = shadow_offset(dst_row0 + r, g * 16, d, rows_per_tile, 1);
+            *reinterpret_cast<uint4*>(shadow8 + off) = make_uint4(packed[0], packed[1], packed[2], packed[3]);
+        }
+#pragma unroll
+        for (int o = 16; o > 0; o >>= 1) {
+            es += __shfl_xor_sync(0xffffffffu, es, o);
+            ys += __shfl_xor_sync(0xffffffffu, ys, o);
+        }
+        if (lane == 0) {
+            const float E = finite ? __double2float_ru(sqrt(es) * (1.0 + 0x1p-40)) : INFINITY;
+            const float Y = finite ? __double2float_ru(sqrt(ys) * (1.0 + 0x1p-40)) : INFINITY;
+            float* m = meta + (dst_row0 + r) * 3;
+            m[0] = s;
+            m[1] = E;
+            m[2] = Y;
+            if (min_bits) {
+                atomicMin(min_bits, __float_as_uint(E));
+                atomicMin(min_bits + 1, __float_as_uint(Y));
+            }
+            if (tile_ab) {
+                const int64_t t = (dst_row0 + r) / 256;
+                atomicMax(tile_ab + 2 * t, __float_as_uint(__fadd_ru(Y, E)));
+                atomicMax(tile_ab + 2 * t + 1, __float_as_uint(E));
+            }
+        }
+    }
+}
+
+__global__ void __launch_bounds__(256)
 column_sums_kernel(const float* __restrict__ src, int64_t n_rows, int d, int rows_per_block, float* __restrict__ sums) {
     const int64_t r0 = (int64_t)blockIdx.x * rows_per_block;
     int64_t r1 = r0 + rows_per_block;
@@ -133,6 +211,19 @@
     column_sums_kernel<<<(unsigned)((n_rows + rows_per_block - 1) / rows_per_block), 256, 0, st>>>(src, n_rows, d,
                                                                                                     rows_per_block, sums);
     KIRAG_LAUNCH_OK("column_sums_kernel");
+    return 0;
+}
+
+int launch_convert_rows_s8(const float* src, int64_t n_rows, int d, int64_t dst_row0, void* shadow8,
+                           int rows_per_tile, const float* center, float* meta, float* tile_ab, unsigned* min_bits,
+                           cudaStream_t st) {
+    if (n_rows <= 0) return 0;
+    KIRAG_CHECK(d % 128 == 0, "convert_s8: d=%d is not a multiple of 128", d);
+    int64_t blocks = (n_rows * 32 + 255) / 256;
+    if (blocks > 148 * 16) blocks = 148 * 16;
+    KIRAG_CUDA_OK(launch_chained(convert_rows_s8_kernel, dim3((unsigned)blocks), dim3(256), 0, st, src, n_rows, d, dst_row0,
+                                 (uint8_t*)shadow8, rows_per_tile, center, meta, (unsigned*)tile_ab, min_bits));
+    KIRAG_LAUNCH_OK("convert_rows_s8_kernel");
     return 0;
 }
 
diff --git a/kirag_b200/csrc/rescore.cu b/kirag_b200/csrc/rescore.cu
--- a/kirag_b200/csrc/rescore.cu
+++ b/kirag_b200/csrc/rescore.cu
@@ -31,6 +31,81 @@
     if (lane == 0) out[qi * (int64_t)m + j] = result;
 }
 
+__global__ void __launch_bounds__(256)
+bf16_rescore_kernel(const uint8_t* __restrict__ shadow, int d, const float* __restrict__ q, Cand* __restrict__ cand,
+                    const int* __restrict__ cnt, int cand_stride, int m, int64_t nq, float* __restrict__ tau,
+                    float* __restrict__ tau8) {
+    pdl_wait();
+    pdl_launch_dependents();
+    const int lane = threadIdx.x & 31;
+    const int64_t warp = ((int64_t)blockIdx.x * blockDim.x + threadIdx.x) >> 5;
+    if (warp >= nq * m) return;
+    const int64_t qi = warp / m;
+    const int j = (int)(warp - qi * m);
+    if (j == 0 && lane == 0) {
+        tau8[qi] = tau[qi];
+        tau[qi] = -INFINITY;
+    }
+    int count = cnt[qi];
+    if (count > m) count = m;
+    if (j >= count) return;
+    Cand* cd = cand + qi * (int64_t)cand_stride + j;
+    const int32_t row = cd->id;
+    const float* qr = q + qi * (int64_t)d;
+    float acc = 0.0f;
+    for (int c = lane * 8; c < d; c += 256) {
+        const uint4 raw = *reinterpret_cast<const uint4*>(shadow + shadow_offset(row, c, d, kTileRows));
+        const float4 qa = *reinterpret_cast<const float4*>(qr + c);
+        const float4 qb = *reinterpret_cast<const float4*>(qr + c + 4);
+        const float qv[8] = {qa.x, qa.y, qa.z, qa.w, qb.x, qb.y, qb.z, qb.w};
+        const uint32_t w[4] = {raw.x, raw.y, raw.z, raw.w};
+#pragma unroll
+        for (int e = 0; e < 8; ++e) {
+            const float y = __uint_as_float((e & 1) ? (w[e >> 1] & 0xffff0000u) : (w[e >> 1] << 16));
+            acc = fmaf(__bfloat162float(__float2bfloat16_rn(qv[e])), y, acc);
+        }
+    }
+    acc = warp_butterfly_sum(acc);
+    if (lane == 0) cd->s = acc;
+}
+
+__global__ void tier2_threshold_kernel(float* __restrict__ tau, const float* __restrict__ tau8, const float* __restrict__ qnorm,
+                                       const float* __restrict__ qerr, float eps_a, float eps_b,
+                                       const float* __restrict__ qmeta, const float* __restrict__ tile_ab, float emin,
+                                       float ymin, int64_t nq) {
+    pdl_wait();
+    pdl_launch_dependents();
+    const int64_t i = (int64_t)blockIdx.x * blockDim.x + threadIdx.x;
+    if (i >= nq) return;
+    const float eq = qmeta[3 * i + 1], aq = __fadd_ru(qmeta[3 * i + 2], eq);
+    const float at = tile_ab[2 * (i / 256)], bt = tile_ab[2 * (i / 256) + 1];
+    float delta = __fadd_rd(__fmul_rd(emin, __fsub_rd(at, aq)), __fmul_rd(ymin, __fsub_rd(bt, eq))) * (1.0f - 0x1p-10f);
+    if (!(delta >= 0.0f)) delta = 0.0f;
+    const float t8 = tau8[i] - delta - (eps_a * qnorm[i] + eps_b * qerr[i]);
+    if (t8 > tau[i] || !(t8 == t8)) tau[i] = (t8 == t8) ? t8 : INFINITY;
+}
+
+int launch_bf16_rescore(const void* shadow, int d, const float* q, Cand* cand, const int* cnt, int cand_stride, int m,
+                        int64_t nq, float* tau, float* tau8, cudaStream_t st) {
+    if (nq <= 0 || m <= 0) return 0;
+    KIRAG_CHECK(d % 64 == 0 && (reinterpret_cast<uintptr_t>(q) & 15) == 0, "bf16_rescore: d=%d or query alignment", d);
+    const int64_t blocks = (nq * m + 7) / 8;
+    KIRAG_CHECK(blocks < 0x7fffffffLL, "bf16_rescore: too many candidates");
+    KIRAG_CUDA_OK(launch_chained(bf16_rescore_kernel, dim3((unsigned)blocks), dim3(256), 0, st, (const uint8_t*)shadow, d, q,
+                                 cand, cnt, cand_stride, m, nq, tau, tau8));
+    KIRAG_LAUNCH_OK("bf16_rescore_kernel");
+    return 0;
+}
+
+int launch_tier2_threshold(float* tau, const float* tau8, const float* qnorm, const float* qerr, float eps_a, float eps_b,
+                           const float* qmeta, const float* tile_ab, float emin, float ymin, int64_t nq, cudaStream_t st) {
+    if (nq <= 0) return 0;
+    KIRAG_CUDA_OK(launch_chained(tier2_threshold_kernel, dim3((unsigned)((nq + 255) / 256)), dim3(256), 0, st, tau, tau8,
+                                 qnorm, qerr, eps_a, eps_b, qmeta, tile_ab, emin, ymin, nq));
+    KIRAG_LAUNCH_OK("tier2_threshold_kernel");
+    return 0;
+}
+
 int launch_rescore(const float* master, int d, const float* q, const Cand* cand, const int* cnt,
                    int cand_stride, int m, float* out_scores, int64_t nq, const float* tauk, const float* qnorm,
                    const float* qerr, float eps_a, float eps_b, cudaStream_t st) {
diff --git a/kirag_b200/csrc/scan_tc.cu b/kirag_b200/csrc/scan_tc.cu
--- a/kirag_b200/csrc/scan_tc.cu
+++ b/kirag_b200/csrc/scan_tc.cu
@@ -100,14 +100,23 @@
 __device__ __forceinline__ void tmem_dealloc2(uint32_t taddr, uint32_t ncols) {
     asm volatile("tcgen05.dealloc.cta_group::2.sync.aligned.b32 %0, %1;" ::"r"(taddr), "r"(ncols) : "memory");
 }
-__device__ __forceinline__ void umma_bf16_2cta(uint32_t tmem_d, uint64_t desc_a, uint64_t desc_b, uint32_t idesc,
-                                               uint32_t accumulate) {
-    asm volatile(
-        "{\n\t.reg .pred p;\n\t"
-        "setp.ne.b32 p, %4, 0;\n\t"
-        "tcgen05.mma.cta_group::2.kind::f16 [%0], %1, %2, %3, p;\n\t}"
-        ::"r"(tmem_d), "l"(desc_a), "l"(desc_b), "r"(idesc), "r"(accumulate)
-        : "memory");
+template <bool I8>
+__device__ __forceinline__ void umma_2cta(uint32_t tmem_d, uint64_t desc_a, uint64_t desc_b, uint32_t idesc,
+                                          uint32_t accumulate) {
+    if (I8)
+        asm volatile(
+            "{\n\t.reg .pred p;\n\t"
+            "setp.ne.b32 p, %4, 0;\n\t"
+            "tcgen05.mma.cta_group::2.kind::i8 [%0], %1, %2, %3, p;\n\t}"
+            ::"r"(tmem_d), "l"(desc_a), "l"(desc_b), "r"(idesc), "r"(accumulate)
+            : "memory");
+    else
+        asm volatile(
+            "{\n\t.reg .pred p;\n\t"
+            "setp.ne.b32 p, %4, 0;\n\t"
+            "tcgen05.mma.cta_group::2.kind::f16 [%0], %1, %2, %3, p;\n\t}"
+            ::"r"(tmem_d), "l"(desc_a), "l"(desc_b), "r"(idesc), "r"(accumulate)
+            : "memory");
 }
 __device__ __forceinline__ void umma_commit_2cta(uint64_t* bar, uint16_t mask) {
     asm volatile(
@@ -145,6 +154,9 @@
 }
 __host__ __device__ constexpr uint32_t make_idesc_bf16(int M, int N) {
     return (1u << 4) | (1u << 7) | (1u << 10) | ((uint32_t)(N >> 3) << 17) | ((uint32_t)(M >> 4) << 24);
+}
+__host__ __device__ constexpr uint32_t make_idesc_s8(int M, int N) {
+    return (2u << 4) | (1u << 7) | (1u << 10) | ((uint32_t)(N >> 3) << 17) | ((uint32_t)(M >> 4) << 24);
 }
 
 struct ScanArgs {
@@ -162,14 +174,23 @@
     int q_dep;
     float* dump;
     int64_t dump_ld;
+    const float* rowmeta;
+    const float* qscale;
+    const float* tile_ab;
+    float slack;
 };
 
-__device__ __forceinline__ uint32_t pass_mask(const ScanArgs& a, const uint32_t (&v)[32], int64_t q0, int64_t row,
-                                              bool row_ok, float mytau) {
+template <bool I8>
+__device__ __forceinline__ uint32_t pass_mask(const ScanArgs& a, uint32_t (&v)[32], int64_t q0, int64_t row,
+                                              bool row_ok, float mytau, float mysq, float sj, float mj) {
     uint32_t pass = 0;
 #pragma unroll
     for (int c = 0; c < 32; ++c) {
         const float t = __shfl_sync(0xffffffffu, mytau, c);
+        if (I8) {
+            const float sq = __shfl_sync(0xffffffffu, mysq, c);
+            v[c] = __float_as_uint(fmaf(sq, __int2float_rn((int)v[c]) * sj, mj));
+        }
         pass |= (__uint_as_float(v[c]) >= t ? 1u : 0u) << c;
     }
     if (!row_ok) pass = 0;
@@ -298,9 +319,10 @@
     }
 }
 
-template <int NG, typename Release>
+template <int NG, bool I8, typename Release>
 __device__ __forceinline__ void filter_item(const ScanArgs& a, uint32_t taddr, int64_t q0, int64_t row, bool row_ok,
-                                            int lane, Stash& st, const float (&mytau)[NG], Release release) {
+                                            int lane, Stash& st, const float (&mytau)[NG], const float (&mysq)[NG],
+                                            float sj, float mj, Release release) {
     stash_clear(st);
     st.q0 = q0;
     st.row = (int32_t)row;
@@ -309,7 +331,7 @@
         uint32_t v[32];
         tmem_ld32(taddr + g * 32, v);
         tmem_ld_wait();
-        const uint32_t pass = pass_mask(a, v, q0 + g * 32, row, row_ok, mytau[g]);
+        const uint32_t pass = pass_mask<I8>(a, v, q0 + g * 32, row, row_ok, mytau[g], mysq[g], sj, mj);
         if (__any_sync(0xffffffffu, pass != 0))
             handle_survivors(a, v, pass, q0 + g * 32, g * 32, (int32_t)row, lane, st);
     }
@@ -328,7 +350,7 @@
     static constexpr int kStageBytes = kBlockBytes + (RES ? 0 : kQHalfBytes);
 };
 
-template <int PQ, bool RES>
+template <int PQ, bool RES, bool I8>
 __global__ void __cluster_dims__(2, 1, 1) __launch_bounds__(EpiCfg<PQ>::kThreads, 1)
 scan_tc_pair_kernel(const ScanArgs a) {
     constexpr int kHalfQ = PairCfg<PQ, RES>::kHalfQ;
@@ -337,7 +359,8 @@
     constexpr uint16_t kPairMask = 0x3;
     extern __shared__ uint8_t smem_raw[];
     uint8_t* smem = reinterpret_cast<uint8_t*>((reinterpret_cast<uintptr_t>(smem_raw) + 1023) & ~(uintptr_t)1023);
-    const int KC = a.d >> 6;
+    constexpr int kElemBytes = I8 ? 1 : 2;
+    const int KC = I8 ? (a.d >> 7) : (a.d >> 6);
     const int NS = a.n_stages;
     uint8_t* stage_base = smem;
     uint8_t* q_res = smem + (size_t)NS * kStageBytes;
@@ -380,7 +403,7 @@
             if (a.q_dep) pdl_wait();
             if (RES && elect_one()) {
                 mbar_expect_tx(q_bar, (uint32_t)(KC * kQHalfBytes));
-                bulk_g2s(q_res, a.qshadow + (size_t)rank * ((size_t)a.d * kHalfQ * 2), (uint32_t)(KC * kQHalfBytes),
+                bulk_g2s(q_res, a.qshadow + (size_t)rank * ((size_t)a.d * kHalfQ * kElemBytes), (uint32_t)(KC * kQHalfBytes),
                          q_bar, pol_q);
             }
             __syncwarp();
@@ -392,8 +415,8 @@
                 int64_t ti = a.tile_lo + 2 * p + rank;
                 if (ti >= a.tile_hi) ti = a.tile_hi - 1;
                 const int64_t tile = (ti * a.tile_mult) % a.n_tiles;
-                const uint8_t* xsrc = a.shadow + (size_t)tile * ((size_t)a.d * kTileRows * 2);
-                const uint8_t* qsrc = a.qshadow + (size_t)(2 * qt + rank) * ((size_t)a.d * kHalfQ * 2);
+                const uint8_t* xsrc = a.shadow + (size_t)tile * ((size_t)a.d * kTileRows * kElemBytes);
+                const uint8_t* qsrc = a.qshadow + (size_t)(2 * qt + rank) * ((size_t)a.d * kHalfQ * kElemBytes);
                 const uint64_t pol_xw = (n_qt > 1 && qt == n_qt - 1) ? pol_x_last : pol_x;
                 for (int kc = 0; kc < KC; ++kc) {
                     mbar_wait_warp(&empty_bar[s], ph ^ 1u, 100 + s, lane);
@@ -428,7 +451,7 @@
                     }
                 }
             } else {
-                constexpr uint32_t idesc = make_idesc_bf16(2 * kTileRows, PQ);
+                constexpr uint32_t idesc = I8 ? make_idesc_s8(2 * kTileRows, PQ) : make_idesc_bf16(2 * kTileRows, PQ);
                 if (RES) mbar_wait_warp(q_bar, 0, 200, lane);
                 uint32_t it = 0;
                 for (int64_t w = w_lo; w < w_hi; ++w, ++it) {
@@ -446,7 +469,7 @@
                         if (elect_one()) {
 #pragma unroll
                             for (int k4 = 0; k4 < 4; ++k4)
-                                umma_bf16_2cta(d_tmem, da + (uint64_t)(k4 * 2), db + (uint64_t)(k4 * 2), idesc,
+                                umma_2cta<I8>(d_tmem, da + (uint64_t)(k4 * 2), db + (uint64_t)(k4 * 2), idesc,
                                                (kc | k4) ? 1u : 0u);
                             umma_commit_2cta(&empty_bar[s], kPairMask);
                             if (kc == KC - 1) umma_commit_2cta(&tmem_full[as], kPairMask);
@@ -470,11 +493,27 @@
         stash_clear(pend);
         pdl_wait();
         float mytau[NG], nxtau[NG];
+        float mysq[NG], nxsq[NG];
+        float rm[3] = {0.f, 0.f, 0.f}, ab[2] = {0.f, 0.f};
+        auto item_row = [&](int64_t w) {
+            const int64_t ti = a.tile_lo + 2 * (w / n_qt) + rank;
+            const int64_t tile = ((ti < a.tile_hi ? ti : a.tile_hi - 1) * a.tile_mult) % a.n_tiles;
+            return tile * kTileRows + quad * 32 + lane;
+        };
         {
             const int qt0 = RES ? 0 : (int)(w_lo % n_qt);
 #pragma unroll
-            for (int g = 0; g < NG; ++g)
+            for (int g = 0; g < NG; ++g) {
                 mytau[g] = (w_lo < w_hi) ? __ldcg(a.tau + (int64_t)qt0 * PQ + col0 + g * 32 + lane) : 0.f;
+                mysq[g] = (I8 && w_lo < w_hi) ? __ldcg(a.qscale + 3 * ((int64_t)qt0 * PQ + col0 + g * 32 + lane)) : 0.f;
+            }
+            if (I8 && w_lo < w_hi) {
+                const int64_t r0 = item_row(w_lo);
+#pragma unroll
+                for (int i = 0; i < 3; ++i) rm[i] = __ldg(a.rowmeta + r0 * 3 + i);
+                ab[0] = __ldcg(a.tile_ab + 2 * qt0);
+                ab[1] = __ldcg(a.tile_ab + 2 * qt0 + 1);
+            }
         }
         for (int64_t w = w_lo; w < w_hi; ++w, ++it) {
             const int64_t p = w / n_qt;
@@ -489,19 +528,38 @@
             const int qt_next = (qt + 1 == n_qt) ? 0 : qt + 1;
             const bool fetch = !RES && n_qt > 1 && w + 1 < w_hi;
 #pragma unroll
-            for (int g = 0; g < NG; ++g)
+            for (int g = 0; g < NG; ++g) {
                 nxtau[g] = fetch ? __ldcg(a.tau + (int64_t)qt_next * PQ + col0 + g * 32 + lane) : mytau[g];
+                if (I8) nxsq[g] = fetch ? __ldcg(a.qscale + 3 * ((int64_t)qt_next * PQ + col0 + g * 32 + lane)) : mysq[g];
+            }
+            float sj = 0.f, mj = 0.f, nxrm[3], nxab[2];
+            if (I8) {
+                const float A = ab[0], B = ab[1];
+                sj = rm[0];
+                mj = fmaf(fmaf(rm[1], A, fmaf(rm[2], B, A * a.slack)), 1.0f + 0x1p-13f, 0x1p-20f * A * (rm[1] + rm[2]));
+                const int64_t rn = item_row(w + 1 < w_hi ? w + 1 : w);
+#pragma unroll
+                for (int i = 0; i < 3; ++i) nxrm[i] = __ldg(a.rowmeta + rn * 3 + i);
+                nxab[0] = fetch ? __ldcg(a.tile_ab + 2 * qt_next) : ab[0];
+                nxab[1] = fetch ? __ldcg(a.tile_ab + 2 * qt_next + 1) : ab[1];
+            }
             mbar_wait(&tmem_full[as], aph, 500 + as);
             tc_fence_after();
             const uint32_t ebar = leader_empty[as];
-            filter_item<NG>(a, tmem_base + lane_base + as * PQ + col0, (int64_t)qt * PQ + col0, row, row_ok,
-                            lane, cur, mytau, [=]() {
+            filter_item<NG, I8>(a, tmem_base + lane_base + as * PQ + col0, (int64_t)qt * PQ + col0, row, row_ok,
+                            lane, cur, mytau, mysq, sj, mj, [=]() {
                                 tc_fence_before();
                                 __syncwarp();
                                 if (lane == 0) mbar_arrive_cluster(ebar);
                             });
 #pragma unroll
-            for (int g = 0; g < NG; ++g) mytau[g] = nxtau[g];
+            for (int g = 0; g < NG; ++g) { mytau[g] = nxtau[g]; if (I8) mysq[g] = nxsq[g]; }
+            if (I8) {
+#pragma unroll
+                for (int i = 0; i < 3; ++i) rm[i] = nxrm[i];
+                ab[0] = nxab[0];
+                ab[1] = nxab[1];
+            }
             stash_store(a, pend);
             stash_reserve(a, cur);
             pend = cur;
@@ -518,6 +576,7 @@
 }
 
 int scan_tc_supported(int d) { return (d % 64 == 0 && d >= 64 && d <= 4096) ? 1 : 0; }
+int scan_tc_i8_supported(int d) { return (scan_tc_supported(d) && d % 128 == 0) ? 1 : 0; }
 
 template <int PQ, bool RES>
 static size_t pair_fixed_bytes(int d) {
@@ -532,6 +591,7 @@
 
 int scan_tc_pick(int64_t nq, int d, ScanTcPlan* plan) {
     KIRAG_CHECK(scan_tc_supported(d), "scan_tc: dimension %d is not supported (need a multiple of 64, <= 4096)", d);
+    plan->i8 = 0;
     if (nq <= 64) { plan->bq = 64; plan->resident = pair_stages<64, true>(d) >= 6; }
     else if (nq <= 128) { plan->bq = 128; plan->resident = pair_stages<128, true>(d) >= 4; }
     else { plan->bq = 256; plan->resident = 0; }
@@ -540,10 +600,10 @@
 
 size_t scan_tc_qshadow_bytes(int64_t nq, int d, const ScanTcPlan& plan) {
     const int64_t tiles = (nq + plan.bq - 1) / plan.bq;
-    return (size_t)tiles * plan.bq * d * 2;
-}
-
-template <int PQ, bool RES>
+    return (size_t)tiles * plan.bq * d * (plan.i8 ? 1 : 2);
+}
+
+template <int PQ, bool RES, bool I8 = false>
 static int launch_scan_pair(const ScanArgs& args_in, int num_sms, cudaStream_t st) {
     ScanArgs args = args_in;
     const int ns = pair_stages<PQ, RES>(args.d);
@@ -551,16 +611,28 @@
     KIRAG_CHECK(!RES || args.nq <= PQ, "scan_tc pair: the resident variant takes a single query tile");
     args.n_stages = ns;
     const size_t smem = pair_fixed_bytes<PQ, RES>(args.d) + (size_t)ns * PairCfg<PQ, RES>::kStageBytes;
-    if (ensure_dynamic_smem(scan_tc_pair_kernel<PQ, RES>, kSmemLimit)) return 1;
+    if (ensure_dynamic_smem(scan_tc_pair_kernel<PQ, RES, I8>, kSmemLimit)) return 1;
     int64_t pairs = ((args.tile_hi - args.tile_lo + 1) / 2) * ((args.nq + PQ - 1) / PQ);
     if (pairs > num_sms / 2) pairs = num_sms / 2;
     if (pairs <= 0) return 0;
-    KIRAG_CUDA_OK(launch_chained(scan_tc_pair_kernel<PQ, RES>, dim3((unsigned)(2 * pairs)), dim3(EpiCfg<PQ>::kThreads), smem, st, args));
+    KIRAG_CUDA_OK(launch_chained(scan_tc_pair_kernel<PQ, RES, I8>, dim3((unsigned)(2 * pairs)), dim3(EpiCfg<PQ>::kThreads), smem, st, args));
     KIRAG_LAUNCH_OK("scan_tc_pair_kernel");
     return 0;
 }
 
-static int launch_scan_args(const ScanArgs& args, const ScanTcPlan& plan, int num_sms, cudaStream_t st) {
+static int launch_scan_args(const ScanArgs& args, const ScanTcPlan& plan, const ScanI8Args* i8, int num_sms,
+                            cudaStream_t st) {
+    KIRAG_CHECK(!plan.i8 == !i8, "scan_tc: the int8 plan needs the int8 arguments and only it takes them");
+    if (plan.i8) {
+        KIRAG_CHECK(plan.bq == 256 && !plan.resident && args.d % 128 == 0, "scan_tc: no int8 kernel for bq=%d d=%d",
+                    plan.bq, args.d);
+        ScanArgs a8 = args;
+        a8.rowmeta = i8->rowmeta;
+        a8.qscale = i8->qscale;
+        a8.tile_ab = i8->tile_ab;
+        a8.slack = i8->slack;
+        return launch_scan_pair<256, false, true>(a8, num_sms, st);
+    }
     if (plan.bq == 64 && plan.resident) return launch_scan_pair<64, true>(args, num_sms, st);
     if (plan.bq == 64 && !plan.resident) return launch_scan_pair<64, false>(args, num_sms, st);
     if (plan.bq == 128 && plan.resident) return launch_scan_pair<128, true>(args, num_sms, st);
@@ -573,7 +645,7 @@
 int launch_scan_tc(const void* shadow, int64_t n_rows, int d, const void* qshadow, int64_t nq,
                    const ScanTcPlan& plan, int64_t tile_lo, int64_t tile_hi, int64_t n_tiles,
                    int64_t tile_mult, const float* tau, Cand* cand, int* cnt, int cap, int num_sms,
-                   int q_dep, cudaStream_t st) {
+                   int q_dep, cudaStream_t st, const ScanI8Args* i8) {
     ScanArgs args{};
     args.q_dep = q_dep;
     args.shadow = (const uint8_t*)shadow;
@@ -591,12 +663,12 @@
     args.cap = cap;
     args.dump = nullptr;
     args.dump_ld = 0;
-    return launch_scan_args(args, plan, num_sms, st);
+    return launch_scan_args(args, plan, i8, num_sms, st);
 }
 
 int launch_scan_tc_dump(const void* shadow, int64_t n_rows, int d, const void* qshadow, int64_t nq,
                         const ScanTcPlan& plan, const float* tau_inf, int* cnt_scratch, float* dump,
-                        int64_t dump_ld, int num_sms, cudaStream_t st) {
+                        int64_t dump_ld, int num_sms, cudaStream_t st, const ScanI8Args* i8) {
     ScanArgs args{};
     args.shadow = (const uint8_t*)shadow;
     args.qshadow = (const uint8_t*)qshadow;
@@ -614,7 +686,7 @@
     args.dump = dump;
     args.dump_ld = dump_ld;
     args.q_dep = 1;
-    return launch_scan_args(args, plan, num_sms, st);
-}
-
-}
+    return launch_scan_args(args, plan, i8, num_sms, st);
+}
+
+}
```

Measured after the change: 44550, median of 6. +40.9%, better.
